# Nobita421/signature-Gan

Measured on AMD Instinct MI355X. Metric: signature images/sec (G+D train step, bs64 64x64 z=100), higher is better.
Workload: dtype f32; 1 GPU; configs[1]: reference conv G/D 64x64x1, z=100, batch 64 per GPU, f32, n_critic=1; global_batch=64, parallelism=dp1

## Files before the change

### signature-gan_amd/csrc/act.h

```cpp
#pragma once
#include <hip/hip_runtime.h>
#include <hip/hip_ext.h>
#include <stdint.h>

#define SIGGAN_LAUNCH_EV(ev, kernel, grid, block, shmem, stream, ...)                                            \
    do {                                                                                                         \
        if (ev) hipExtLaunchKernelGGL(kernel, grid, block, shmem, stream, nullptr, ev, 0, __VA_ARGS__);          \
        else hipLaunchKernelGGL(kernel, grid, block, shmem, stream, __VA_ARGS__);                                \
    } while (0)


namespace siggan {

typedef __bf16 bf16_t;
typedef _Float16 f16_t;
enum DType : int { DT_F32 = 0, DT_BF16 = 1, DT_F16 = 2 };
static inline size_t dt_size(int dt) { return dt == DT_F32 ? 4 : 2; }

typedef float f32x4 __attribute__((ext_vector_type(4)));
typedef float f32x16 __attribute__((ext_vector_type(16)));
typedef short s16x4 __attribute__((ext_vector_type(4)));
typedef short s16x8 __attribute__((ext_vector_type(8)));
typedef bf16_t bf16x4 __attribute__((ext_vector_type(4)));
typedef bf16_t bf16x8 __attribute__((ext_vector_type(8)));
typedef f16_t f16x4 __attribute__((ext_vector_type(4)));
typedef f16_t f16x8 __attribute__((ext_vector_type(8)));

template <class T> __device__ __forceinline__ f32x4 ld4(const T* p);
template <> __device__ __forceinline__ f32x4 ld4<float>(const float* p) { return *reinterpret_cast<const f32x4*>(p); }
template <> __device__ __forceinline__ f32x4 ld4<bf16_t>(const bf16_t* p) {
    const bf16x4 v = *reinterpret_cast<const bf16x4*>(p);
    return f32x4{(float)v[0], (float)v[1], (float)v[2], (float)v[3]};
}
template <> __device__ __forceinline__ f32x4 ld4<f16_t>(const f16_t* p) {
    const f16x4 v = *reinterpret_cast<const f16x4*>(p);
    return f32x4{(float)v[0], (float)v[1], (float)v[2], (float)v[3]};
}
template <class T> __device__ __forceinline__ void st4(T* p, f32x4 v);
template <> __device__ __forceinline__ void st4<float>(float* p, f32x4 v) { *reinterpret_cast<f32x4*>(p) = v; }
template <> __device__ __forceinline__ void st4<bf16_t>(bf16_t* p, f32x4 v) {
    *reinterpret_cast<bf16x4*>(p) = bf16x4{(bf16_t)v[0], (bf16_t)v[1], (bf16_t)v[2], (bf16_t)v[3]};
}
template <> __device__ __forceinline__ void st4<f16_t>(f16_t* p, f32x4 v) {
    *reinterpret_cast<f16x4*>(p) = f16x4{(f16_t)v[0], (f16_t)v[1], (f16_t)v[2], (f16_t)v[3]};
}
template <class T> __device__ __forceinline__ float ld1(const T* p) { return (float)*p; }
template <class T> __device__ __forceinline__ void st1(T* p, float v) { *p = (T)v; }

template <bool LK> __device__ __forceinline__ float g_act(float x, float gs) { return LK ? (x > 0.f ? x : x * gs) : fmaxf(x, 0.f); }
template <bool LK> __device__ __forceinline__ float g_dact(float x, float g, float gs) { return x > 0.f ? g : (LK ? g * gs : 0.f); }

#define SIGGAN_GS_SWITCH(GS, LK, ...)                                                   \
    do {                                                                         \
        if ((GS) != 0.f) { constexpr bool LK = true; __VA_ARGS__; }              \
        else { constexpr bool LK = false; __VA_ARGS__; }                         \
    } while (0)

#define SIGGAN_DT_SWITCH(DT, T, ...)                                     \
    do {                                                                 \
        if ((DT) == DT_F32) { using T = float; __VA_ARGS__; }            \
        else if ((DT) == DT_BF16) { using T = bf16_t; __VA_ARGS__; }     \
        else { using T = f16_t; __VA_ARGS__; }                           \
    } while (0)

}
```

### signature-gan_amd/csrc/gconv.h

```cpp
#pragma once
#include <hip/hip_runtime.h>
#include <stdint.h>
#include <vector>

#include "act.h"

namespace siggan {

enum Epilogue : int {
    EPI_RAW = 0,
    EPI_BIAS_LRELU_DROP,
    EPI_AFFINE_RELU,
    EPI_LRELU_BWD,
    EPI_BN_BWD_STATS,
};

struct GConvArgs {
    int dt;
    const void* in;
    const void* wp;
    void* out;
    int B, Hi, Wi, Ci, Co;
    int lgHr, lgWr;
    int Ho, Wo;
    int form;
    int M;
    int epi;
    const float* bias;
    const float* noise;
    const float* scale;
    const float* shift;
    const void* aref;
    const float* bnp;
    float* stat0;
    float* stat1;
    int64_t stat_cap;
    const float* cls_w;
    float* cls_part;
    float slope;
    float gslope;
    float* slab;
    int64_t slab_floats;
    size_t slab_stride;
    const float* zeros;
};

struct BnBwdParams { f32x4 sc, sf, mu, rs; };
__device__ __forceinline__ BnBwdParams bn_bwd_params(const float* __restrict__ bnp, int Co, int co) {
    BnBwdParams q;
    q.sc = *reinterpret_cast<const f32x4*>(bnp + co); q.sf = *reinterpret_cast<const f32x4*>(bnp + Co + co);
    q.mu = *reinterpret_cast<const f32x4*>(bnp + 2 * Co + co); q.rs = *reinterpret_cast<const f32x4*>(bnp + 3 * Co + co);
    return q;
}
template <class T, bool LK>
__device__ __forceinline__ void bn_bwd_stat_terms(const f32x4 v, const f32x4 y, const BnBwdParams& q, float gs, f32x4& s0, f32x4& s1) {
#pragma unroll
    for (int e = 0; e < 4; ++e) {
        const float vq = (float)(T)v[e];
        const float d = g_dact<LK>(fmaf(y[e], q.sc[e], q.sf[e]), vq, gs);
        s0[e] += d;
        s1[e] = fmaf(d, (y[e] - q.mu[e]) * q.rs[e], s1[e]);
    }
}
__host__ __device__ inline bool gen_lk(const GConvArgs& a) {
    return a.gslope != 0.f && (a.epi == EPI_AFFINE_RELU || a.epi == EPI_BN_BWD_STATS);
}

struct WgradArgs {
    int dt;
    const void* S;
    const void* L;
    float* slab;
    float* dw;
    float* db;
    int B, Cs, Cl;
    int lgHs, lgWs, lgCl;
    int K;
    int kchunk;
    const float* zeros;
};

struct Prof {
    struct Rec { int id; double flops, bytes; hipEvent_t e0, e1; };
    static constexpr int NID = 8;
    std::vector<Rec> recs;
    static const char* name(int id);
    void begin(int id, double flops, double bytes, hipStream_t st);
    void clear();
};
extern Prof* g_prof;

int launch_gconv(const GConvArgs& a, hipStream_t st);
void launch_gconv16(int cfg, const GConvArgs& a, dim3 grid, hipStream_t st, hipEvent_t e0, hipEvent_t e1, int kq = 1);
void launch_wgrad16(bool small, const WgradArgs& a, dim3 grid, hipStream_t st, hipEvent_t e0, hipEvent_t e1);
int launch_wgrad(WgradArgs a, int max_splits, hipStream_t st);

}
```

### signature-gan_amd/csrc/gconv.hip

```cpp
#include "gconv.h"
#include <hip/hip_ext.h>

namespace siggan {


static constexpr int BK = 32;
static constexpr int PAD = 4;

__device__ __forceinline__ int xcd_remap(int bid, int nwg) {
    const int q = nwg >> 3, r = nwg & 7, xcd = bid & 7, idx = bid >> 3;
    return (xcd < r ? xcd * (q + 1) : r * (q + 1) + (xcd - r) * q) + idx;
}

template <int BM, int BN, int WM, int WN, int BK = 32, int DEEP = 0, int KQ = 1, bool LK = false>
__global__ __launch_bounds__(256 * KQ) void k_gconv(const GConvArgs a) {
    constexpr int TM = BM / (32 * WM), TN = BN / (32 * WN);
    constexpr int PA = BM / 32, PB = BN / 32;
    constexpr int KC = BK / 32;
    constexpr int LD = BK + 4;
    __shared__ __attribute__((aligned(16))) float smem[KQ * 2 * LD * (BM + BN)];
    const int quad = KQ > 1 ? (int)(threadIdx.x >> 8) : 0;
    float* const sA = smem + quad * (2 * LD * (BM + BN));
    float* const sB = sA + 2 * LD * BM;

    const int tid = threadIdx.x & 255, lane = tid & 63, wave = tid >> 6;
    const int li = lane & 31, lh = lane >> 5;
    const int wm = wave / WN, wn = wave % WN;
    const float* const a_in = static_cast<const float*>(a.in);
    const float* const a_wp = static_cast<const float*>(a.wp);

    const int tiles_n = a.Co / BN;
    const int bid = xcd_remap(blockIdx.x, gridDim.x);
    const int m0 = (bid / tiles_n) * BM, n0 = (bid % tiles_n) * BN;
    const int cls = blockIdx.z, ph = cls >> 1, pw = cls & 1;
    const int Hr = 1 << a.lgHr, Wr = 1 << a.lgWr;
    const int ntaps = a.form == 0 ? 16 : 4;
    const int Ktot = ntaps * a.Ci;
    const int lgcpt = 31 - __builtin_clz(a.Ci / BK);
    const int nk_all = ntaps << lgcpt;
    const int kper = (nk_all + gridDim.y * KQ - 1) / (gridDim.y * KQ);
    const int k_lo = (blockIdx.y * KQ + quad) * kper;
    const int k_hi = min(nk_all, k_lo + kper);
    const int nk = k_hi - k_lo;

    const int kc = tid & 7, rloc = tid >> 3;
    const float* a_base[PA];
    int a_ih0[PA], a_iw0[PA];
#pragma unroll
    for (int p = 0; p < PA; ++p) {
        const int m = m0 + rloc + 32 * p;
        if (m < a.M) {
            const int n = m >> (a.lgHr + a.lgWr);
            const int rh = (m >> a.lgWr) & (Hr - 1), rw = m & (Wr - 1);
            a_base[p] = a_in + (size_t)n * a.Hi * a.Wi * a.Ci + kc * 4;
            if (a.form == 0) { a_ih0[p] = 2 * rh - 1; a_iw0[p] = 2 * rw - 1; }
            else             { a_ih0[p] = rh + ph;    a_iw0[p] = rw + pw; }
        } else {
            a_base[p] = a_in; a_ih0[p] = -(1 << 20); a_iw0[p] = -(1 << 20);
        }
    }
    const float* wcur = a_wp + ((size_t)cls * a.Co + n0 + rloc) * Ktot + kc * 4 + (size_t)k_lo * BK;

    const float* a_cur[PA];
    int a_step[PA];
    int l_tap = k_lo >> lgcpt, l_cc = k_lo & ((1 << lgcpt) - 1);
    auto set_tap = [&]() __attribute__((always_inline)) {
        int dh, dw;
        if (a.form == 0) { dh = l_tap >> 2; dw = l_tap & 3; } else { dh = -(l_tap >> 1); dw = -(l_tap & 1); }
#pragma unroll
        for (int p = 0; p < PA; ++p) {
            const int ih = a_ih0[p] + dh, iw = a_iw0[p] + dw;
            const bool ok = (unsigned)ih < (unsigned)a.Hi && (unsigned)iw < (unsigned)a.Wi;
            a_cur[p] = ok ? a_base[p] + ((size_t)(ih * a.Wi + iw) * a.Ci + l_cc * BK) : a.zeros;
            a_step[p] = ok ? BK : 0;
        }
    };
    constexpr int NSET = DEEP ? 2 : 1;
    f32x4 ra[NSET][PA][KC], rb[NSET][PB][KC];
    auto load_tile = [&](int set = 0) __attribute__((always_inline)) {
#pragma unroll
        for (int p = 0; p < PA; ++p) {
#pragma unroll
            for (int q = 0; q < KC; ++q) ra[set][p][q] = *reinterpret_cast<const f32x4*>(a_cur[p] + 32 * q);
            a_cur[p] += a_step[p];
        }
#pragma unroll
        for (int p = 0; p < PB; ++p)
#pragma unroll
            for (int q = 0; q < KC; ++q) rb[set][p][q] = *reinterpret_cast<const f32x4*>(wcur + (size_t)(32 * p) * Ktot + 32 * q);
        wcur += BK;
        if (++l_cc == (1 << lgcpt)) { l_cc = 0; ++l_tap; set_tap(); }
    };
    auto store_tile = [&](int buf, int set = 0) __attribute__((always_inline)) {
        float* dA = sA + buf * LD * BM + rloc * LD + kc * 4;
        float* dB = sB + buf * LD * BN + rloc * LD + kc * 4;
#pragma unroll
        for (int p = 0; p < PA; ++p)
#pragma unroll
            for (int q = 0; q < KC; ++q) *reinterpret_cast<f32x4*>(dA + 32 * p * LD + 32 * q) = ra[set][p][q];
#pragma unroll
        for (int p = 0; p < PB; ++p)
#pragma unroll
            for (int q = 0; q < KC; ++q) *reinterpret_cast<f32x4*>(dB + 32 * p * LD + 32 * q) = rb[set][p][q];
    };

    f32x16 acc[TM][TN];
#pragma unroll
    for (int i = 0; i < TM; ++i)
#pragma unroll
        for (int j = 0; j < TN; ++j)
#pragma unroll
            for (int r = 0; r < 16; ++r) acc[i][j][r] = 0.f;

    if (DEEP && nk >= 5) {
        auto tile = [&](const int h, const int kt, const bool st, const bool ld) __attribute__((always_inline)) {
            const float* pA = sA + h * LD * BM + (wm * (32 * TM) + li) * LD + 4 * lh;
            const float* pB = sB + h * LD * BN + (wn * (32 * TN) + li) * LD + 4 * lh;
            f32x4 fa[2][TM], fb[2][TN];
#pragma unroll
            for (int i = 0; i < TM; ++i) fa[0][i] = *reinterpret_cast<const f32x4*>(pA + 32 * i * LD);
#pragma unroll
            for (int j = 0; j < TN; ++j) fb[0][j] = *reinterpret_cast<const f32x4*>(pB + 32 * j * LD);
#pragma unroll
            for (int c = 0; c < BK / 8; ++c) {
                const int cur = c & 1, nxt = cur ^ 1;
                if (c + 1 < BK / 8) {
#pragma unroll
                    for (int i = 0; i < TM; ++i) fa[nxt][i] = *reinterpret_cast<const f32x4*>(pA + 32 * i * LD + 8 * (c + 1));
#pragma unroll
                    for (int j = 0; j < TN; ++j) fb[nxt][j] = *reinterpret_cast<const f32x4*>(pB + 32 * j * LD + 8 * (c + 1));
                }
                __builtin_amdgcn_sched_barrier(0);
#pragma unroll
                for (int t = 0; t < 4; ++t)
#pragma unroll
                    for (int i = 0; i < TM; ++i)
#pragma unroll
                        for (int j = 0; j < TN; ++j)
                            acc[i][j] = __builtin_amdgcn_mfma_f32_32x32x2f32(fa[cur][i][t], fb[cur][j][t], acc[i][j], 0, 0, 0);
                if (c == 0 && st) store_tile(h ^ 1, h ^ 1);
                if (c == 1 && ld) load_tile(h ^ 1);
            }
            __syncthreads();
        };
        set_tap();
        load_tile(0);
        load_tile(1);
        store_tile(0, 0);
        load_tile(0);
        __syncthreads();
        int kt = 0;
        for (; kt + 4 < nk; kt += 2) {
            tile(0, kt, true, true);
            tile(1, kt + 1, true, true);
        }
        for (; kt < nk; kt += 2) {
            tile(0, kt, kt + 1 < nk, kt + 3 < nk);
            if (kt + 1 < nk) tile(1, kt + 1, kt + 2 < nk, kt + 4 < nk);
        }
    } else {
    if (nk > 0) {
        set_tap();
        load_tile();
        store_tile(0);
        if (nk > 1) load_tile();
    }
    __syncthreads();

    for (int kt = 0; kt < nk; ++kt) {
        const int buf = kt & 1;
        const float* pA = sA + buf * LD * BM + (wm * (32 * TM) + li) * LD + 4 * lh;
        const float* pB = sB + buf * LD * BN + (wn * (32 * TN) + li) * LD + 4 * lh;
        f32x4 fa[2][TM], fb[2][TN];
#pragma unroll
        for (int i = 0; i < TM; ++i) fa[0][i] = *reinterpret_cast<const f32x4*>(pA + 32 * i * LD);
#pragma unroll
        for (int j = 0; j < TN; ++j) fb[0][j] = *reinterpret_cast<const f32x4*>(pB + 32 * j * LD);
#pragma unroll
        for (int c = 0; c < BK / 8; ++c) {
            const int cur = c & 1, nxt = cur ^ 1;
            if (c + 1 < BK / 8) {
#pragma unroll
                for (int i = 0; i < TM; ++i) fa[nxt][i] = *reinterpret_cast<const f32x4*>(pA + 32 * i * LD + 8 * (c + 1));
#pragma unroll
                for (int j = 0; j < TN; ++j) fb[nxt][j] = *reinterpret_cast<const f32x4*>(pB + 32 * j * LD + 8 * (c + 1));
            }
            __builtin_amdgcn_sched_barrier(0);
#pragma unroll
            for (int t = 0; t < 4; ++t)
#pragma unroll
                for (int i = 0; i < TM; ++i)
#pragma unroll
                    for (int j = 0; j < TN; ++j)
                        acc[i][j] = __builtin_amdgcn_mfma_f32_32x32x2f32(fa[cur][i][t], fb[cur][j][t], acc[i][j], 0, 0, 0);
            if (c == 0 && kt + 1 < nk) store_tile(buf ^ 1);
            if (c == 1 && kt + 2 < nk) load_tile();
        }
        __syncthreads();
    }
    }

    float* const outp = gridDim.y > 1 ? a.slab + (size_t)blockIdx.y * a.slab_stride : static_cast<float*>(a.out);
    const int epi = gridDim.y > 1 ? (int)EPI_RAW : a.epi;
    constexpr int LDT = BN + 4;
    static_assert(BM * LDT <= 2 * LD * (BM + BN), "output tile must fit the staging buffers");
    float* const sT = smem;
    if (KQ > 1) {
        float* const red = smem + 2 * LD * (BM + BN);
        if (quad == 1) {
#pragma unroll
            for (int i = 0; i < TM; ++i)
#pragma unroll
                for (int j = 0; j < TN; ++j)
#pragma unroll
                    for (int r = 0; r < 16; ++r) red[(((wave * TM + i) * TN + j) * 16 + r) * 64 + lane] = acc[i][j][r];
        }
        __syncthreads();
        if (quad == 0) {
#pragma unroll
            for (int i = 0; i < TM; ++i)
#pragma unroll
                for (int j = 0; j < TN; ++j)
#pragma unroll
                    for (int r = 0; r < 16; ++r) acc[i][j][r] += red[(((wave * TM + i) * TN + j) * 16 + r) * 64 + lane];
        }
    }
    if (quad == 0) {
#pragma unroll
        for (int i = 0; i < TM; ++i)
#pragma unroll
            for (int j = 0; j < TN; ++j)
#pragma unroll
                for (int r = 0; r < 16; ++r)
                    sT[(wm * (32 * TM) + 32 * i + (r & 3) + 8 * (r >> 2) + 4 * lh) * LDT + wn * (32 * TN) + 32 * j + li] = acc[i][j][r];
    }
    __syncthreads();
    if (quad != 0 && epi != EPI_BN_BWD_STATS) return;
    constexpr int C4 = BN / 4, RPP = 256 / C4;
    const int c4 = tid % C4, r0 = tid / C4;
    const int co = n0 + c4 * 4;
    BnBwdParams bq;
    f32x4 st0 = {0.f, 0.f, 0.f, 0.f}, st1 = st0;
    if (epi == EPI_BN_BWD_STATS) bq = bn_bwd_params(a.bnp, a.Co, co);
    const f32x4 bias4 = epi == EPI_BIAS_LRELU_DROP ? *reinterpret_cast<const f32x4*>(a.bias + co) : f32x4{0.f, 0.f, 0.f, 0.f};
    f32x4 sc4 = {1.f, 1.f, 1.f, 1.f}, sh4 = {0.f, 0.f, 0.f, 0.f};
    if (epi == EPI_AFFINE_RELU) { sc4 = *reinterpret_cast<const f32x4*>(a.scale + co); sh4 = *reinterpret_cast<const f32x4*>(a.shift + co); }
    const bool use_noise = (epi == EPI_BIAS_LRELU_DROP || epi == EPI_LRELU_BWD) && a.noise != nullptr;
#pragma unroll
    for (int p = 0; p < BM / RPP; ++p) {
        const int row = r0 + RPP * p, m = m0 + row;
        if (m >= a.M || quad != 0) continue;
        const int n = m >> (a.lgHr + a.lgWr);
        size_t opix;
        if (a.form == 0) {
            opix = (size_t)m;
        } else {
            const int rh = (m >> a.lgWr) & (Hr - 1), rw = m & (Wr - 1);
            opix = ((size_t)n * a.Ho + 2 * rh + ph) * a.Wo + 2 * rw + pw;
        }
        const size_t o = opix * a.Co + co;
        f32x4 v = *reinterpret_cast<const f32x4*>(sT + row * LDT + c4 * 4);
        if (epi == EPI_BN_BWD_STATS) {
            bn_bwd_stat_terms<float, LK>(v, *reinterpret_cast<const f32x4*>(static_cast<const float*>(a.aref) + o), bq, a.gslope, st0, st1);
        } else if (epi == EPI_BIAS_LRELU_DROP) {
#pragma unroll
            for (int e = 0; e < 4; ++e) { float t = v[e] + bias4[e]; v[e] = t > 0.f ? t : t * a.slope; }
            if (use_noise) {
                const f32x4 nz = *reinterpret_cast<const f32x4*>(a.noise + (size_t)n * a.Co + co);
#pragma unroll
                for (int e = 0; e < 4; ++e) v[e] *= nz[e];
            }
        } else if (epi == EPI_AFFINE_RELU) {
#pragma unroll
            for (int e = 0; e < 4; ++e) v[e] = g_act<LK>(fmaf(v[e], sc4[e], sh4[e]), a.gslope);
        } else if (epi == EPI_LRELU_BWD) {
            const f32x4 ar = *reinterpret_cast<const f32x4*>(static_cast<const float*>(a.aref) + o);
#pragma unroll
            for (int e = 0; e < 4; ++e) v[e] *= ar[e] > 0.f ? 1.f : a.slope;
            if (use_noise) {
                const f32x4 nz = *reinterpret_cast<const f32x4*>(a.noise + (size_t)n * a.Co + co);
#pragma unroll
                for (int e = 0; e < 4; ++e) v[e] *= nz[e];
            }
        }
        *reinterpret_cast<f32x4*>(outp + o) = v;
    }
    if (epi == EPI_BN_BWD_STATS) {
        __syncthreads();
        if (quad == 0) {
            *reinterpret_cast<f32x4*>(sT + (size_t)tid * 8) = st0;
            *reinterpret_cast<f32x4*>(sT + (size_t)tid * 8 + 4) = st1;
        }
        __syncthreads();
        if (quad == 0 && r0 == 0) {
#pragma unroll 4
            for (int k = 1; k < RPP; ++k) {
                st0 += *reinterpret_cast<const f32x4*>(sT + (size_t)(k * C4 + c4) * 8);
                st1 += *reinterpret_cast<const f32x4*>(sT + (size_t)(k * C4 + c4) * 8 + 4);
            }
            const size_t prow = (size_t)cls * (gridDim.x / tiles_n) + bid / tiles_n;
            *reinterpret_cast<f32x4*>(a.stat0 + prow * a.Co + co) = st0;
            *reinterpret_cast<f32x4*>(a.stat1 + prow * a.Co + co) = st1;
        }
    }
}

template <int CI, bool LK>
__global__ __launch_bounds__(256) void k_gconv_up4(const GConvArgs a) {
    constexpr int BM = 128, BN = 32, LD = BK + 4, LP = CI + 4, NCC = CI / BK;
    constexpr int PATCH_PIX = 264;
    constexpr int SMEM = (PATCH_PIX * LP + 2 * 4 * BN * LD) > (BM * 4 * BN) ? (PATCH_PIX * LP + 2 * 4 * BN * LD) : (BM * 4 * BN);
    __shared__ __attribute__((aligned(16))) float smem[SMEM];
    float* const sP = smem;
    float* const sB = smem + PATCH_PIX * LP;
    const int tid = threadIdx.x, lane = tid & 63, wave = tid >> 6;
    const int li = lane & 31, lh = lane >> 5;
    const int m0 = xcd_remap(blockIdx.x, gridDim.x) * BM;
    const int Hr = 1 << a.lgHr, Wr = 1 << a.lgWr, Wp = Wr + 2;
    const int Ktot = 4 * CI;
    const int n_img = m0 >> (a.lgHr + a.lgWr), rh0 = (m0 >> a.lgWr) & (Hr - 1), rows = BM >> a.lgWr;

    {
        const float* const img = static_cast<const float*>(a.in) + (size_t)n_img * a.Hi * a.Wi * CI;
        const int nchunk = (rows + 2) * Wp * (CI / 4);
        constexpr int NI = (PATCH_PIX * (CI / 4) + 255) / 256;
        f32x4 v[NI];
#pragma unroll
        for (int q = 0; q < NI; ++q) {
            const int i = tid + 256 * q;
            const int pix = i / (CI / 4), ch = i - pix * (CI / 4);
            const int pr = pix / Wp, pc = pix - pr * Wp;
            const int ih = rh0 - 1 + pr, iw = pc - 1;
            const bool ok = i < nchunk && (unsigned)ih < (unsigned)a.Hi && (unsigned)iw < (unsigned)a.Wi;
            const float* src = ok ? img + ((size_t)ih * a.Wi + iw) * CI + ch * 4 : a.zeros;
            v[q] = *reinterpret_cast<const f32x4*>(src);
        }
#pragma unroll
        for (int q = 0; q < NI; ++q) {
            const int i = tid + 256 * q;
            if (i < nchunk) {
                const int pix = i / (CI / 4), ch = i - pix * (CI / 4);
                *reinterpret_cast<f32x4*>(sP + pix * LP + ch * 4) = v[q];
            }
        }
    }
    const int kc = tid & 7, rloc = tid >> 3;
    const float* const w_row = static_cast<const float*>(a.wp) + (size_t)rloc * Ktot + kc * 4;
    f32x4 rb[4];
    int l_k = 0;
    auto load_tile = [&]() __attribute__((always_inline)) {
        const int cls = l_k / NCC, cc = l_k - cls * NCC;
#pragma unroll
        for (int t = 0; t < 4; ++t)
            rb[t] = *reinterpret_cast<const f32x4*>(w_row + (size_t)cls * a.Co * Ktot + t * CI + cc * BK);
        ++l_k;
    };
    auto store_tile = [&](int buf) __attribute__((always_inline)) {
#pragma unroll
        for (int t = 0; t < 4; ++t)
            *reinterpret_cast<f32x4*>(sB + ((buf * 4 + t) * BN + rloc) * LD + kc * 4) = rb[t];
    };

    f32x16 acc[4];
#pragma unroll
    for (int cls = 0; cls < 4; ++cls)
#pragma unroll
        for (int r = 0; r < 16; ++r) acc[cls][r] = 0.f;

    load_tile();
    store_tile(0);
    load_tile();
    __syncthreads();

    const int ml = wave * 32 + li;
    const float* const pP = sP + (((ml >> a.lgWr) + 1) * Wp + (ml & (Wr - 1)) + 1) * LP + 4 * lh;

#pragma unroll
    for (int cls = 0; cls < 4; ++cls) {
        const int ph = cls >> 1, pw = cls & 1;
        for (int cc = 0; cc < NCC; ++cc) {
            const int kt = cls * NCC + cc, buf = kt & 1;
            const float* pA[4];
#pragma unroll
            for (int t = 0; t < 4; ++t) pA[t] = pP + ((ph - (t >> 1)) * Wp + (pw - (t & 1))) * LP + cc * BK;
            const float* pB = sB + (buf * 4 * BN + li) * LD + 4 * lh;
            f32x4 fa[2][4], fb[2][4];
#pragma unroll
            for (int t = 0; t < 4; ++t) {
                fa[0][t] = *reinterpret_cast<const f32x4*>(pA[t]);
                fb[0][t] = *reinterpret_cast<const f32x4*>(pB + t * BN * LD);
            }
#pragma unroll
            for (int c = 0; c < BK / 8; ++c) {
                const int cur = c & 1, nxt = cur ^ 1;
                if (c + 1 < BK / 8) {
#pragma unroll
                    for (int t = 0; t < 4; ++t) {
                        fa[nxt][t] = *reinterpret_cast<const f32x4*>(pA[t] + 8 * (c + 1));
                        fb[nxt][t] = *reinterpret_cast<const f32x4*>(pB + t * BN * LD + 8 * (c + 1));
                    }
                }
                __builtin_amdgcn_sched_barrier(0);
#pragma unroll
                for (int t = 0; t < 4; ++t)
#pragma unroll
                    for (int u = 0; u < 4; ++u)
                        acc[cls] = __builtin_amdgcn_mfma_f32_32x32x2f32(fa[cur][t][u], fb[cur][t][u], acc[cls], 0, 0, 0);
                if (c == 0 && kt + 1 < 4 * NCC) store_tile(buf ^ 1);
                if (c == 1 && kt + 2 < 4 * NCC) load_tile();
            }
            __syncthreads();
        }
    }

    const float sc = a.epi == EPI_AFFINE_RELU ? a.scale[li] : 1.f, sf = a.epi == EPI_AFFINE_RELU ? a.shift[li] : 0.f;
    const int Wo = 2 * Wr;
    float* const so = smem;
#pragma unroll
    for (int r = 0; r < 16; ++r) {
        const int mr = wave * 32 + (r & 3) + 8 * (r >> 2) + 4 * lh;
        const int rl = mr >> a.lgWr, rw = mr & (Wr - 1);
#pragma unroll
        for (int cls = 0; cls < 4; ++cls) {
            float v = acc[cls][r];
            if (a.epi == EPI_AFFINE_RELU) v = g_act<LK>(fmaf(v, sc, sf), a.gslope);
            so[(((2 * rl + (cls >> 1)) * Wo) + 2 * rw + (cls & 1)) * BN + li] = v;
        }
    }
    __syncthreads();
    f32x4* const dst = reinterpret_cast<f32x4*>(static_cast<float*>(a.out) + ((size_t)n_img * a.Ho + 2 * rh0) * a.Wo * BN);
    const f32x4* const src = reinterpret_cast<const f32x4*>(so);
#pragma unroll
    for (int q = 0; q < (BM * 4 * BN / 4) / 256; ++q) dst[q * 256 + tid] = src[q * 256 + tid];
}

template <class T, bool LK>
__global__ __launch_bounds__(256) void k_splitk_epilogue(const GConvArgs a, int nsplit, int64_t total4) {
    const int64_t i = (int64_t)blockIdx.x * 256 + threadIdx.x;
    if (a.epi == EPI_BN_BWD_STATS) {
        __shared__ __attribute__((aligned(16))) float sh[256 * 8];
        const int C4 = a.Co / 4, c4 = threadIdx.x & (C4 - 1);
        f32x4 s0 = {0.f, 0.f, 0.f, 0.f}, s1 = s0;
        if (i < total4) {
            const f32x4* sl = reinterpret_cast<const f32x4*>(a.slab);
            const size_t stride4 = a.slab_stride / 4;
            f32x4 v = sl[i];
            for (int z = 1; z < nsplit; ++z) v += sl[(size_t)z * stride4 + i];
            bn_bwd_stat_terms<T, LK>(v, ld4<T>(static_cast<const T*>(a.aref) + i * 4), bn_bwd_params(a.bnp, a.Co, c4 * 4), a.gslope, s0, s1);
            st4<T>(static_cast<T*>(a.out) + i * 4, v);
        }
        *reinterpret_cast<f32x4*>(sh + threadIdx.x * 8) = s0;
        *reinterpret_cast<f32x4*>(sh + threadIdx.x * 8 + 4) = s1;
        __syncthreads();
        if ((int)threadIdx.x < C4) {
            for (int k = 1; k < 256 / C4; ++k) {
                s0 += *reinterpret_cast<const f32x4*>(sh + (k * C4 + c4) * 8);
                s1 += *reinterpret_cast<const f32x4*>(sh + (k * C4 + c4) * 8 + 4);
            }
            *reinterpret_cast<f32x4*>(a.stat0 + (size_t)blockIdx.x * a.Co + c4 * 4) = s0;
            *reinterpret_cast<f32x4*>(a.stat1 + (size_t)blockIdx.x * a.Co + c4 * 4) = s1;
        }
        return;
    }
    if (i >= total4) return;
    const float4* sl = reinterpret_cast<const float4*>(a.slab);
    const size_t stride4 = a.slab_stride / 4;
    float4 v = sl[i];
    for (int z = 1; z < nsplit; ++z) {
        const float4 w = sl[(size_t)z * stride4 + i];
        v.x += w.x; v.y += w.y; v.z += w.z; v.w += w.w;
    }
    const int C4 = a.Co / 4;
    const int64_t per_img = (int64_t)C4 * a.Ho * a.Wo;
    const bool p2 = (C4 & (C4 - 1)) == 0 && (per_img & (per_img - 1)) == 0;
    const int c = (p2 ? (int)(i & (C4 - 1)) : (int)(i % C4)) * 4;
    const int64_t n = p2 ? i >> (63 - __builtin_clzll(per_img)) : i / per_img;
    float* e = reinterpret_cast<float*>(&v);
    if (a.epi == EPI_BIAS_LRELU_DROP) {
#pragma unroll
        for (int k = 0; k < 4; ++k) {
            float x = e[k] + a.bias[c + k];
            x = x > 0.f ? x : x * a.slope;
            if (a.noise) x *= a.noise[n * a.Co + c + k];
            e[k] = x;
        }
    } else if (a.epi == EPI_AFFINE_RELU) {
#pragma unroll
        for (int k = 0; k < 4; ++k) e[k] = g_act<LK>(fmaf(e[k], a.scale[c + k], a.shift[c + k]), a.gslope);
    } else if (a.epi == EPI_LRELU_BWD) {
        const f32x4 ar = ld4<T>(static_cast<const T*>(a.aref) + i * 4);
        const float* r = reinterpret_cast<const float*>(&ar);
#pragma unroll
        for (int k = 0; k < 4; ++k) {
            float x = e[k] * (r[k] > 0.f ? 1.f : a.slope);
            if (a.noise) x *= a.noise[n * a.Co + c + k];
            e[k] = x;
        }
    }
    st4<T>(static_cast<T*>(a.out) + i * 4, f32x4{v.x, v.y, v.z, v.w});
    if (a.cls_w) {
        __shared__ float shc[4];
        const f32x4 w4 = *reinterpret_cast<const f32x4*>(a.cls_w + (size_t)(p2 ? (i & (per_img - 1)) : (i % per_img)) * 4);
        float d = (float)(T)v.x * w4[0];
        d = fmaf((float)(T)v.y, w4[1], d); d = fmaf((float)(T)v.z, w4[2], d); d = fmaf((float)(T)v.w, w4[3], d);
#pragma unroll
        for (int o = 32; o > 0; o >>= 1) d += __shfl_down(d, o, 64);
        if ((threadIdx.x & 63) == 0) shc[threadIdx.x >> 6] = d;
        __syncthreads();
        if (threadIdx.x == 0) a.cls_part[blockIdx.x] = ((shc[0] + shc[1]) + shc[2]) + shc[3];
    }
}

Prof* g_prof = nullptr;

const char* Prof::name(int id) {
    static const char* n[NID] = {"k_gconv<128,128>", "k_gconv<128,64>", "k_gconv<64,64>", "k_gconv<128,32>",
                                 "k_wgrad<64,64>", "k_gconv_up4", "k_wgrad<32,128>", "?"};
    return n[id < 0 || id >= NID ? NID - 1 : id];
}
void Prof::begin(int id, double flops, double bytes, hipStream_t) {
    Rec r; r.id = id; r.flops = flops; r.bytes = bytes;
    (void)hipEventCreate(&r.e0); (void)hipEventCreate(&r.e1);
    recs.push_back(r);
}
void Prof::clear() {
    for (auto& r : recs) { (void)hipEventDestroy(r.e0); (void)hipEventDestroy(r.e1); }
    recs.clear();
}

static double gconv_bytes(const GConvArgs& a) {
    const double es = (double)dt_size(a.dt);
    const double in = (double)a.B * a.Hi * a.Wi * a.Ci, out = (double)a.B * a.Ho * a.Wo * a.Co, w = 16.0 * a.Ci * a.Co;
    return es * (in + w + out * (a.epi == EPI_LRELU_BWD ? 2.0 : 1.0));
}
static double wgrad_bytes(const WgradArgs& a) {
    const double es = (double)dt_size(a.dt);
    return es * ((double)a.K * a.Cs + 4.0 * a.K * a.Cl) + 4.0 * 16.0 * a.Cs * a.Cl;
}

template <int BM, int BN, int WM, int WN, int BKT = 32, int DEEP = 0, int KQ = 1>
static int launch_cfg(const GConvArgs& a_in, hipStream_t st, int id, int nsplit) {
    GConvArgs a = a_in;
    const int tiles = ((a.M + BM - 1) / BM) * (a.Co / BN);
    const int ncls = a.form == 0 ? 1 : 4;
    const int64_t total4 = (int64_t)a.B * a.Ho * a.Wo * a.Co / 4;
    int rows = 0;
    if (a.epi == EPI_BN_BWD_STATS) {
        if (nsplit > 1 && (256 % (a.Co / 4)) != 0) nsplit = 1;
        rows = nsplit > 1 ? (int)((total4 + 255) / 256) : ((a.M + BM - 1) / BM) * ncls;
        if ((int64_t)2 * rows * a.Co > a.stat_cap) { a.epi = EPI_RAW; rows = 0; }
        else a.stat1 = a.stat0 + (size_t)rows * a.Co;
    }
    if (a.cls_w) {
        const int64_t per_img4 = (int64_t)a.Ho * a.Wo * a.Co / 4;
        if (nsplit > 1 && a.epi != EPI_BN_BWD_STATS && total4 % 256 == 0 && per_img4 % 256 == 0) rows = (int)(per_img4 / 256);
        else a.cls_w = nullptr;
    }
    dim3 grid(tiles, nsplit, ncls);
    if (g_prof) g_prof->begin(id, 2.0 * a.M * a.Co * (double)((a.form == 0 ? 16 : 4) * a.Ci) * ncls, gconv_bytes(a), st);
    hipEvent_t e0 = g_prof ? g_prof->recs.back().e0 : nullptr, e1 = g_prof ? g_prof->recs.back().e1 : nullptr;
    if (a.dt != DT_F32) {
        launch_gconv16(id, a, grid, st, e0, e1, KQ);
    } else if (gen_lk(a)) {
        hipExtLaunchKernelGGL((k_gconv<BM, BN, WM, WN, BKT, DEEP, KQ, true>), grid, dim3(256 * KQ), 0, st, e0, e1, 0, a);
    } else if (g_prof) {
        hipExtLaunchKernelGGL((k_gconv<BM, BN, WM, WN, BKT, DEEP, KQ>), grid, dim3(256 * KQ), 0, st, e0, e1, 0, a);
    } else {
        hipLaunchKernelGGL((k_gconv<BM, BN, WM, WN, BKT, DEEP, KQ>), grid, dim3(256 * KQ), 0, st, a);
    }
    if (nsplit > 1)
        SIGGAN_GS_SWITCH(gen_lk(a) ? 1.f : 0.f, LK, SIGGAN_DT_SWITCH(a.dt, T, hipLaunchKernelGGL((k_splitk_epilogue<T, LK>),
            dim3((unsigned)((total4 + 255) / 256)), dim3(256), 0, st, a, nsplit, total4)));
    return rows;
}

int launch_gconv(const GConvArgs& a_in, hipStream_t st) {
    GConvArgs a = a_in;
    const int ncls = a.form == 0 ? 1 : 4;
    auto blocks = [&](int bm, int bn) { return ((a.M + bm - 1) / bm) * (a.Co / bn) * ncls; };
    const int nk = (a.form == 0 ? 16 : 4) * (a.Ci / BK);
    auto splits = [&](int nblk) {
        int ns = 1;
        if (a.slab && nblk < 384) {
            ns = (512 + nblk - 1) / nblk;
            if (ns > nk / 4) ns = nk / 4;
            if (ns > 8) ns = 8;
            const int64_t out_floats = (int64_t)a.B * a.Ho * a.Wo * a.Co;
            if (ns > 1 && (int64_t)ns * out_floats > a.slab_floats) ns = (int)(a.slab_floats / out_floats);
            if (ns < 1) ns = 1;
        }
        a.slab_stride = (size_t)a.B * a.Ho * a.Wo * a.Co;
        return ns;
    };
    if (a.Co >= 64) {
        if (a.Co >= 128 && blocks(128, 128) >= 512) return launch_cfg<128, 128, 2, 2, 32, 1>(a, st, 0, 1);
        const int ns = splits(blocks(64, 64));
        if (ns == 2 && (nk & 1) == 0) return launch_cfg<64, 64, 2, 2, 32, 1, 2>(a, st, 2, 1);
        if (ns == 4 && !a.cls_w && a.dt != DT_F32 && (nk & 1) == 0) return launch_cfg<64, 64, 2, 2, 32, 1, 2>(a, st, 2, 1);
        return launch_cfg<64, 64, 2, 2, 32, 1>(a, st, 2, ns);
    }
    if (a.dt == DT_F32 && a.form == 1 && a.Co == 32 && (a.epi == EPI_RAW || a.epi == EPI_AFFINE_RELU) && (a.Ci == 32 || a.Ci == 64) &&
        a.M / 128 >= (a.Ci == 32 ? 384 : 768) && a.M % 128 == 0 &&
        ((1 << (a.lgHr + a.lgWr)) % 128) == 0 && a.lgWr >= 4 && a.lgWr <= 6) {
        dim3 grid(a.M / 128);
        if (g_prof) g_prof->begin(5, 2.0 * a.M * a.Co * (double)(4 * a.Ci) * 4, gconv_bytes(a), st);
        hipEvent_t e0 = g_prof ? g_prof->recs.back().e0 : nullptr, e1 = g_prof ? g_prof->recs.back().e1 : nullptr;
        if (gen_lk(a)) {
            if (a.Ci == 32) hipExtLaunchKernelGGL((k_gconv_up4<32, true>), grid, dim3(256), 0, st, e0, e1, 0, a);
            else hipExtLaunchKernelGGL((k_gconv_up4<64, true>), grid, dim3(256), 0, st, e0, e1, 0, a);
        } else {
            if (a.Ci == 32) hipExtLaunchKernelGGL((k_gconv_up4<32, false>), grid, dim3(256), 0, st, e0, e1, 0, a);
            else hipExtLaunchKernelGGL((k_gconv_up4<64, false>), grid, dim3(256), 0, st, e0, e1, 0, a);
        }
        return 0;
    }
    const int ns = splits(blocks(128, 32));
    return launch_cfg<128, 32, 4, 1, 32, 1>(a, st, 3, ns);
}

template <int BM, int BN, int WM, int WN>
__global__ __launch_bounds__(256) void k_wgrad(const WgradArgs a) {
    constexpr int TM = BM / (32 * WM), TN = BN / (32 * WN);
    constexpr int LDA = BM + PAD, LDB = BN + PAD;
    constexpr int CA = BM / 4, RA = 256 / CA, PA = BK / RA;
    constexpr int CB = BN / 4, RB = 256 / CB, PB = BK / RB;
    __shared__ __attribute__((aligned(16))) float smem[2 * BK * (LDA + LDB)];
    float* const sA = smem;
    float* const sB = smem + 2 * BK * LDA;

    const int tid = threadIdx.x, lane = tid & 63, wave = tid >> 6;
    const int li = lane & 31, lh = lane >> 5;
    const int wm = wave / WN, wn = wave % WN;
    const int N = 16 << a.lgCl;
    const int tiles_n = N / BN;
    const int lin = blockIdx.z * gridDim.x + blockIdx.x;
    const int lid = xcd_remap(lin, gridDim.x * gridDim.z);
    const int bx = lid % gridDim.x, bz = lid / gridDim.x;
    const int i0 = (bx / tiles_n) * BM, j0 = (bx % tiles_n) * BN;
    const int kbeg = bz * a.kchunk;
    const int kend = min(a.K, kbeg + a.kchunk);
    const int nk = (kend - kbeg + BK - 1) / BK;
    const int Hs = 1 << a.lgHs, Ws = 1 << a.lgWs, Hl = 2 * Hs, Wl = 2 * Ws, Cl = 1 << a.lgCl;

    const int ca = tid % CA, ka = tid / CA;
    const int cb = tid % CB, kb = tid / CB;
    const float* const a_S = static_cast<const float*>(a.S);
    const float* const a_L = static_cast<const float*>(a.L);
    const int jj = j0 + cb * 4, tap = jj >> a.lgCl, lch = jj & (Cl - 1);
    const int kh = tap >> 2, kw = tap & 3;

    f32x4 ra[2][PA], rb[2][PB];
    size_t a_off[PA];
    int a_pix[PA], b_pix[PB];
#pragma unroll
    for (int p = 0; p < PA; ++p) { a_pix[p] = kbeg + ka + RA * p; a_off[p] = (size_t)a_pix[p] * a.Cs + i0 + ca * 4; }
#pragma unroll
    for (int p = 0; p < PB; ++p) b_pix[p] = kbeg + kb + RB * p;
    const int a_adv = BK * a.Cs;
    const int lgWl = a.lgWs + 1;
#define WG_LOAD_TILE(KT, SET)                                                                         \
    {                                                                                                 \
        _Pragma("unroll") for (int p = 0; p < PA; ++p) {                                              \
            const float* src = a_pix[p] < kend ? a_S + a_off[p] : a.zeros;                            \
            ra[SET][p] = *reinterpret_cast<const f32x4*>(src);                                       \
            a_off[p] += a_adv; a_pix[p] += BK;                                                        \
        }                                                                                             \
        _Pragma("unroll") for (int p = 0; p < PB; ++p) {                                              \
            const int pix = b_pix[p];                                                                 \
            const int y = pix >> a.lgWs;                                              \
            const int ih = 2 * (y & (Hs - 1)) - 1 + kh, iw = 2 * (pix & (Ws - 1)) - 1 + kw;           \
            const bool ok = pix < kend && (unsigned)ih < (unsigned)Hl && (unsigned)iw < (unsigned)Wl; \
                          \
            const unsigned off = (((unsigned)(2 * y - 1 + kh) << lgWl) + (unsigned)iw) << a.lgCl;     \
            const float* src = ok ? a_L + ((size_t)off + lch) : a.zeros;                              \
            rb[SET][p] = *reinterpret_cast<const f32x4*>(src);                                       \
            b_pix[p] += BK;                                                                           \
        }                                                                                             \
    }
#define WG_STORE_TILE(BUF, SET)                                                                       \
    {                                                                                                 \
        _Pragma("unroll") for (int p = 0; p < PA; ++p)                                                \
            *reinterpret_cast<f32x4*>(sA + (BUF) * BK * LDA + (ka + RA * p) * LDA + ca * 4) = ra[SET][p]; \
        _Pragma("unroll") for (int p = 0; p < PB; ++p)                                                \
            *reinterpret_cast<f32x4*>(sB + (BUF) * BK * LDB + (kb + RB * p) * LDB + cb * 4) = rb[SET][p]; \
    }

    f32x16 acc[TM][TN];
#pragma unroll
    for (int i = 0; i < TM; ++i)
#pragma unroll
        for (int j = 0; j < TN; ++j)
#pragma unroll
            for (int r = 0; r < 16; ++r) acc[i][j][r] = 0.f;

    constexpr int NQ = 256 / BM, KQ = BK / NQ;
    const bool bias_blk = a.db != nullptr && j0 == 0;
    const int bcol = tid % BM, kq = tid / BM;
    float bsum = 0.f;
#define WG_TILE(BUF, ST, LD)                                                                          \
    {                                                                                                 \
        if (bias_blk) {                                                                               \
            const float* col = sA + (BUF) * BK * LDA + kq * KQ * LDA + bcol;                          \
            _Pragma("unroll") for (int k = 0; k < KQ; ++k) bsum += col[k * LDA];                      \
        }                                                                                             \
        const float* pA = sA + (BUF) * BK * LDA + lh * LDA + wm * (32 * TM) + li;                     \
        const float* pB = sB + (BUF) * BK * LDB + lh * LDB + wn * (32 * TN) + li;                     \
                          \
        float fa[2][4][TM], fb[2][4][TN];                                                             \
        _Pragma("unroll") for (int q = 0; q < 4; ++q) {                                               \
            _Pragma("unroll") for (int i = 0; i < TM; ++i) fa[0][q][i] = pA[(2 * q) * LDA + 32 * i];  \
            _Pragma("unroll") for (int j = 0; j < TN; ++j) fb[0][q][j] = pB[(2 * q) * LDB + 32 * j];  \
        }                                                                                             \
        _Pragma("unroll") for (int c = 0; c < BK / 8; ++c) {                                          \
            const int cur = c & 1, nxt = cur ^ 1;                                                     \
            if (c + 1 < BK / 8) {                                                                     \
                _Pragma("unroll") for (int q = 0; q < 4; ++q) {                                       \
                    _Pragma("unroll") for (int i = 0; i < TM; ++i) fa[nxt][q][i] = pA[(8 * c + 8 + 2 * q) * LDA + 32 * i]; \
                    _Pragma("unroll") for (int j = 0; j < TN; ++j) fb[nxt][q][j] = pB[(8 * c + 8 + 2 * q) * LDB + 32 * j]; \
                }                                                                                     \
            }                                                                                         \
            __builtin_amdgcn_sched_barrier(0);                                                        \
            _Pragma("unroll") for (int q = 0; q < 4; ++q)                                             \
                _Pragma("unroll") for (int i = 0; i < TM; ++i)                                        \
                    _Pragma("unroll") for (int j = 0; j < TN; ++j)                                    \
                        acc[i][j] = __builtin_amdgcn_mfma_f32_32x32x2f32(fa[cur][q][i], fb[cur][q][j], acc[i][j], 0, 0, 0); \
            if (c == 0) { ST }                                                                        \
            if (c == 1) { LD }                                                                        \
        }                                                                                             \
        __syncthreads();                                                                              \
    }
    if (nk >= 5) {
        WG_LOAD_TILE(0, 0)
        WG_LOAD_TILE(1, 1)
        WG_STORE_TILE(0, 0)
        WG_LOAD_TILE(2, 0)
        __syncthreads();
        int kt = 0;
        for (; kt + 4 < nk; kt += 2) {
            WG_TILE(0, WG_STORE_TILE(1, 1), WG_LOAD_TILE(kt + 3, 1))
            WG_TILE(1, WG_STORE_TILE(0, 0), WG_LOAD_TILE(kt + 4, 0))
        }
        for (; kt < nk; kt += 2) {
            WG_TILE(0, if (kt + 1 < nk) WG_STORE_TILE(1, 1), if (kt + 3 < nk) WG_LOAD_TILE(kt + 3, 1))
            if (kt + 1 < nk) WG_TILE(1, if (kt + 2 < nk) WG_STORE_TILE(0, 0), if (kt + 4 < nk) WG_LOAD_TILE(kt + 4, 0))
        }
    } else {
        if (nk > 0) {
            WG_LOAD_TILE(0, 0)
            WG_STORE_TILE(0, 0)
            if (nk > 1) WG_LOAD_TILE(1, 0)
        }
        __syncthreads();
        for (int kt = 0; kt < nk; ++kt) {
            if (kt & 1) WG_TILE(1, if (kt + 1 < nk) WG_STORE_TILE(0, 0), if (kt + 2 < nk) WG_LOAD_TILE(kt + 2, 0))
            else WG_TILE(0, if (kt + 1 < nk) WG_STORE_TILE(1, 0), if (kt + 2 < nk) WG_LOAD_TILE(kt + 2, 0))
        }
    }
#undef WG_TILE

#undef WG_LOAD_TILE
#undef WG_STORE_TILE
    if (bias_blk) {
        smem[kq * BM + bcol] = bsum;
        __syncthreads();
        if (tid < BM) {
            float t = smem[tid];
#pragma unroll
            for (int q = 1; q < NQ; ++q) t += smem[q * BM + tid];
            if (gridDim.z == 1) a.db[i0 + tid] = t;
            else a.slab[(size_t)gridDim.z * a.Cs * N + (size_t)bz * a.Cs + i0 + tid] = t;
        }
    }
    if (gridDim.z == 1 && a.dw) {
#pragma unroll
        for (int i = 0; i < TM; ++i)
#pragma unroll
            for (int r = 0; r < 16; ++r) {
                const int row = i0 + wm * (32 * TM) + 32 * i + (r & 3) + 8 * (r >> 2) + 4 * lh;
#pragma unroll
                for (int j = 0; j < TN; ++j) {
                    const int col = j0 + wn * (32 * TN) + 32 * j + li;
                    a.dw[((size_t)row * Cl + (col & (Cl - 1))) * 16 + (col >> a.lgCl)] = acc[i][j][r];
                }
            }
        return;
    }
    float* const out = a.slab + (size_t)bz * a.Cs * N;
#pragma unroll
    for (int i = 0; i < TM; ++i)
#pragma unroll
        for (int r = 0; r < 16; ++r) {
            const int row = i0 + wm * (32 * TM) + 32 * i + (r & 3) + 8 * (r >> 2) + 4 * lh;
#pragma unroll
            for (int j = 0; j < TN; ++j)
                out[(size_t)row * N + j0 + wn * (32 * TN) + 32 * j + li] = acc[i][j][r];
        }
}

static void launch_wgrad_reduce(const float* slab, float* dw, float* db, int nsplit, int Cs, int Cl, hipStream_t st);

int launch_wgrad(WgradArgs a, int max_splits, hipStream_t st) {
    const int N = 16 << a.lgCl;
    const bool small = a.Cs < 64;
    const int tiles = small ? (N / 128) : (a.Cs / 64) * (N / 64);
    int ktiles = (a.K + BK - 1) / BK;
    int nsplit = (512 + tiles - 1) / tiles;
    if (nsplit > ktiles / 4) nsplit = ktiles / 4;
    if (nsplit > max_splits) nsplit = max_splits;
    if (nsplit < 1) nsplit = 1;
    int per = (ktiles + nsplit - 1) / nsplit;
    a.kchunk = per * BK;
    nsplit = (ktiles + per - 1) / per;
    dim3 grid(tiles, 1, nsplit);
    if (g_prof) g_prof->begin(small ? 6 : 4, 2.0 * a.Cs * (double)N * a.K, wgrad_bytes(a), st);
    hipEvent_t e0 = g_prof ? g_prof->recs.back().e0 : nullptr, e1 = g_prof ? g_prof->recs.back().e1 : nullptr;
    if (a.dt != DT_F32) {
        launch_wgrad16(small, a, grid, st, e0, e1);
    } else if (g_prof) {
        if (small) hipExtLaunchKernelGGL((k_wgrad<32, 128, 1, 4>), grid, dim3(256), 0, st, e0, e1, 0, a);
        else hipExtLaunchKernelGGL((k_wgrad<64, 64, 2, 2>), grid, dim3(256), 0, st, e0, e1, 0, a);
    } else if (small) {
        hipLaunchKernelGGL((k_wgrad<32, 128, 1, 4>), grid, dim3(256), 0, st, a);
    } else {
        hipLaunchKernelGGL((k_wgrad<64, 64, 2, 2>), grid, dim3(256), 0, st, a);
    }
    if (nsplit > 1) launch_wgrad_reduce(a.slab, a.dw, a.db, nsplit, a.Cs, 1 << a.lgCl, st);
    return nsplit;
}

__global__ __launch_bounds__(1024) void k_wgrad_reduce(const float* __restrict__ slab, float* __restrict__ dw, float* __restrict__ db,
                                                       int nsplit, int Cs, int lgCl) {
    __shared__ float sh[16][64];
    const int N = 16 << lgCl, Cl = 1 << lgCl;
    const size_t total = (size_t)Cs * N;
    const int cl = threadIdx.x & 63, zl = threadIdx.x >> 6, SL = blockDim.x >> 6;
    const size_t wblocks = total / 64;
    const bool bias = blockIdx.x >= wblocks;
    const size_t idx = bias ? (size_t)(blockIdx.x - wblocks) * 64 + cl : (size_t)blockIdx.x * 64 + cl;
    const float* src = bias ? slab + (size_t)nsplit * total : slab;
    const size_t zstride = bias ? (size_t)Cs : total;
    const bool live = !bias || idx < (size_t)Cs;
    float acc = 0.f;
    if (live) {
#pragma unroll 8
        for (int z = zl; z < nsplit; z += SL) acc += src[(size_t)z * zstride + idx];
    }
    if (SL > 1) {
        sh[zl][cl] = acc;
        __syncthreads();
        if (zl != 0) return;
        for (int k = 1; k < SL; ++k) acc += sh[k][cl];
    }
    if (!live) return;
    if (bias) { db[idx] = acc; return; }
    const int j = (int)(idx & (size_t)(N - 1)), s_ = (int)(idx >> (4 + lgCl));
    const int tap = j >> lgCl, l = j & (Cl - 1);
    dw[((size_t)s_ * Cl + l) * 16 + tap] = acc;
}

static int ilog2(int v) { int l = 0; while ((1 << l) < v) ++l; return l; }

static void launch_wgrad_reduce(const float* slab, float* dw, float* db, int nsplit, int Cs, int Cl, hipStream_t st) {
    const size_t total = (size_t)Cs * 16 * Cl;
    int SL = 1;
    while (SL < 16 && SL < nsplit) SL *= 2;
    const unsigned blocks = (unsigned)(total / 64) + (db ? (unsigned)((Cs + 63) / 64) : 0u);
    hipLaunchKernelGGL(k_wgrad_reduce, dim3(blocks), dim3(64 * SL), 0, st, slab, dw, db, nsplit, Cs, ilog2(Cl));
}

}
```

### signature-gan_amd/csrc/ops.h

```cpp
#pragma once
#include <hip/hip_runtime.h>
#include <stdint.h>

#include "act.h"

namespace siggan {

struct DevState {
    unsigned long long seed;
    unsigned long long rng_ctr;
    float step_size;
    float bc2_sqrt;
    float grad_mul;
    float grad_norm;
    float sumsq;
    int skip;
    float pad[2];
};

void launch_randn(float* out, int64_t n, const DevState* st, uint32_t stream_id, hipStream_t s);
void launch_dropnoise_multi(int nt, float* const* out, const int64_t* n, const int64_t* elem0, const uint32_t* sid, float keep,
                            const DevState* st, hipStream_t s, uint32_t ctr_add = 0);
void launch_mask_to_noise(const float* mask, float* out, int64_t n, float keep, hipStream_t s);
void launch_tick(DevState* st, hipStream_t s);

enum PrepType : int { PREP_PACK_DOWN = 0, PREP_PACK_UP, PREP_FC_T, PREP_CLS, PREP_BN_EVAL, PREP_SCALE, PREP_TAPS };
struct PrepJob {
    int type, O, I, perm;
    int dt;
    const float* mul;
    const float* src;
    const float* src2;
    const float* src3;
    const float* src4;
    float* dst;
};
struct PrepTable {
    static constexpr int MAXJ = 32;
    int njobs;
    int overflow;
    long long prefix[MAXJ + 1];
    PrepJob job[MAXJ];
};
void prep_add(PrepTable& t, const PrepJob& j, long long count);
bool launch_prepare(const PrepTable& t, float bn_eps, hipStream_t s);
bool launch_prepare_conv1(const PrepTable& t, float bn_eps, int dt, const float* x, const float* W, const float* b, float slope,
                          void* out, int B, int S, hipStream_t s);

void launch_fc_fwd(int dt, const float* z, const float* Wt, const float* b, void* y, int B, int K, int C0, float gslope,
                   hipStream_t s, const float* bn_affine_relu = nullptr, const DevState* st = nullptr, uint32_t stream_id = 0,
                   float* z_out = nullptr);
bool launch_fc_fwd_fused(int dt, const float* z, const float* W, const float* bias, void* y, void* a, const float* gamma,
                         const float* beta, float* rmean, float* rvar, int64_t* batches, float* bn, const float* bne,
                         float* z_out, const DevState* st, uint32_t sid, int B, int K, int C0, float momentum, float eps,
                         float gslope, hipStream_t s);
bool launch_fc_bwd_fused(int dt, const void* da, const void* y, const float* z, float* bn, float* dW, float* db, float* dgamma,
                         float* dbeta, int B, int K, int C0, float gslope, hipStream_t s);
void launch_fc_wgrad(int dt, const void* dy, const float* z, float* dW, float* db, int B, int K, int C0, hipStream_t s);

void launch_bn_train_stats(int dt, const void* y, int64_t R, int C, const float* gamma, const float* beta,
                           float* rmean, float* rvar, int64_t* batches, float* bn, float* partial,
                           int perm_c0, float momentum, float eps, hipStream_t s);
void launch_bn_relu(int dt, const void* y, void* a, int64_t R, int C, const float* bn, float gslope, hipStream_t s);
void launch_bn_bwd(int dt, void* da, const void* y, int64_t R, int C, float* bn, float* partial,
                   float* dgamma, float* dbeta, int perm_c0, float gslope, hipStream_t s, int pre_rows = 0, hipEvent_t done = nullptr);

void launch_final_fwd(int dt, const void* act, const float* Wt, const float* b, float* img, int B, int S, int C, float gslope,
                      hipStream_t s, const float* bn = nullptr, hipEvent_t done = nullptr);
void launch_final_bwd_reduce(int dt, const float* dpre, const float* Wt, const void* y, int B, int S, int C, const float* bn,
                             float* partial, float* partial_w, float gslope, hipStream_t s);
void launch_final_bn_bwd_apply(int dt, const float* dpre, const float* Wt, const void* y, void* dy, int B, int S, int C, float* bn,
                               const float* partial, const float* partial_w, float* dW, float* db, float* dgamma, float* dbeta,
                               float gslope, hipStream_t s, hipEvent_t done = nullptr);

void launch_conv1_fwd(int dt, const float* x0, int n0, const float* x1, const float* W, const float* b,
                      const float* noise, float slope, void* out, int B, int S, int C, hipStream_t s);
void launch_conv1_wgrad(int dt, const void* dv, const float* x0, int n0, const float* x1, float* dW, float* db,
                        float* partial, int B, int S, int C, hipStream_t s);
void launch_conv1_dgrad_tanh(int dt, const void* dv, const float* Wt, const float* img, float* dpre, int B, int S,
                             int C, hipStream_t s);
void launch_cls_fwd(int dt, const void* act, const float* wcp, const float* bc, float* logits, int B, int F, hipStream_t s);
void launch_cls_features(int dt, const void* act, float* feat, int B, int C, hipStream_t s);
void launch_bce(const float* logits, int B, int n0, float y0, float y1, float* probs, float* dlogit,
                float* metrics, int is_g_step, hipStream_t s, float gscale = 1.0f, const float* parts = nullptr, int P = 0,
                const float* bc = nullptr);
void launch_cls_bwd(int dt, const float* logits, int n0, float y0, float y1, const float* wcp, const void* act, const float* noise,
                    float slope, void* dv, int B, int C, hipStream_t s, float gscale = 1.0f, float* bce_probs = nullptr,
                    float* bce_dlogit = nullptr, float* bce_metrics = nullptr, int bce_is_g = 0, bool with_bce = false,
                    const float* parts = nullptr, int P = 0, const float* bc = nullptr);
void launch_cls_wgrad(int dt, const float* dlogit, const void* act, float* dWc, float* dbc, int B, int C, hipStream_t s);
void launch_to_f32(int dt, const void* src, float* dst, int64_t n, hipStream_t s);

struct SnLayer {
    const float* W;
    int rows, K;
    int u_off, v_off;
    int64_t w_off;
};
struct SnTable {
    static constexpr int MAXS = 8;
    int n;
    SnLayer layer[MAXS];
    int pre_k[MAXS + 1], pre_r[MAXS + 1];
    float *u, *v;
    float *tbuf, *wbuf;
    float* sig;
    float *u_saved, *v_saved;
    float* dots;
    int u_total, v_total;
    int slot[2];
};
void launch_sn_sigma(const SnTable& t, int training, int slot, float eps, hipStream_t s);
void launch_sn_combine(const SnTable& t, const float* g0, const float* g1, float* out, int64_t total, int npass, hipStream_t s);

void launch_grad_sumsq(const float* g, int64_t n, DevState* st, float* partial, hipStream_t s);
void launch_adam_prepare(DevState* st, float* steps, int ntensors, double lr, double beta1, double beta2,
                         float grad_scale, float clip_max_norm, float* metric_norm, hipStream_t s,
                         int check_finite = 0, float* metric_skipped = nullptr, const float* sumsq_partial = nullptr);
__host__ __device__ inline double pow_step(double b, double t) {
    unsigned long long n = (unsigned long long)t;
    double r = 1.0;
    while (n) { if (n & 1) r *= b; b *= b; n >>= 1; }
    return r;
}
void launch_adam_fused(float* p, float* g, float* m, float* v, int64_t n, DevState* st, float* steps, int ntensors, double t,
                       double lr, double beta1, double beta2, double eps, float grad_scale, float clip_max_norm,
                       float* metric_norm, const float* sumsq_partial, hipStream_t s, float* metric_skipped = nullptr);
void launch_adam(float* p, float* g, float* m, float* v, int64_t n, const DevState* st, double beta1,
                 double beta2, double eps, int write_back_grad, hipStream_t s);

enum ApType : int { AP_FLAT = 0, AP_CONV, AP_T16, AP_TAPS, AP_BN };
struct ApJob {
    int type;
    int A, Bc;
    int dt;
    long long off, n;
    long long off2, n2;
    float* dst;
    float* dst2;
    const float* rmean;
    const float* rvar;
    int wait;
};
struct ApTable {
    static constexpr int MAXJ = 24;
    int njobs, overflow;
    long long prefix[MAXJ + 1];
    ApJob job[MAXJ];
};
void ap_add(ApTable& t, const ApJob& j);
struct ApRide { const float* x; void* out; int B, S, dt; float slope; long long w_off, b_off; unsigned* counter; unsigned* late; };
bool launch_adam_pack(const ApTable& t, float* p, float* g, float* m, float* v, DevState* st, float* steps, int ntensors,
                      double tstep, double lr, double beta1, double beta2, double eps, float grad_scale, float clip_max_norm,
                      float* metric_norm, const float* sumsq_partial, float* metric_skipped, float bn_eps,
                      const ApRide* ride, hipStream_t s);

void launch_augment(const uint8_t* cache, int64_t n_images, const int32_t* index, const int32_t* prm, const int16_t* tabs,
                    const float* lut, float* out, int B, int S, int augment, int fill, hipStream_t s);

}
```

### signature-gan_amd/csrc/ops.hip

```cpp
#include "ops.h"
#include "rng.h"

namespace siggan {

static inline int cdiv(int64_t a, int64_t b) { return (int)((a + b - 1) / b); }

__device__ __forceinline__ uint4 draw(const DevState* st, uint64_t idx, uint32_t stream_id, uint32_t ctr_add = 0) {
    return draw_raw(st->seed, st->rng_ctr + ctr_add, idx, stream_id);
}

__global__ void k_randn(float* __restrict__ out, int64_t n, const DevState* __restrict__ st, uint32_t sid) {
    const int64_t t = (int64_t)blockIdx.x * blockDim.x + threadIdx.x;
    if (t * 4 >= n) return;
    const f32x4 v = normal4(draw(st, (uint64_t)t, sid));
    for (int j = 0; j < 4 && t * 4 + j < n; ++j) out[t * 4 + j] = v[j];
}
__global__ void k_mask_to_noise(const float* __restrict__ m, float* __restrict__ out, int64_t n, float inv) {
    const int64_t i = (int64_t)blockIdx.x * blockDim.x + threadIdx.x;
    if (i < n) out[i] = m[i] * inv;
}
__global__ void k_tick(DevState* st) { st->rng_ctr += 1; }

void launch_randn(float* out, int64_t n, const DevState* st, uint32_t sid, hipStream_t s) {
    hipLaunchKernelGGL(k_randn, dim3(cdiv((n + 3) / 4, 256)), dim3(256), 0, s, out, n, st, sid);
}
struct NoiseTable { float* out[8]; int64_t n[8]; int64_t elem0[8]; uint32_t sid[8]; int64_t pre[9]; int nt; };
__global__ void k_dropnoise_multi(const NoiseTable tb, float keep, float inv, const DevState* __restrict__ st, uint32_t ctr_add) {
    const int64_t g = (int64_t)blockIdx.x * blockDim.x + threadIdx.x;
    if (g >= tb.pre[tb.nt]) return;
    int t = 0;
    while (g >= tb.pre[t + 1]) ++t;
    const int64_t q = g - tb.pre[t];
    const uint4 r = draw(st, (uint64_t)(tb.elem0[t] / 4 + q), tb.sid[t], ctr_add);
    const uint32_t x[4] = {r.x, r.y, r.z, r.w};
    float* o = tb.out[t];
    for (int j = 0; j < 4 && q * 4 + j < tb.n[t]; ++j) o[q * 4 + j] = u01(x[j]) < keep ? inv : 0.f;
}
void launch_dropnoise_multi(int nt, float* const* out, const int64_t* n, const int64_t* elem0, const uint32_t* sid, float keep,
                            const DevState* st, hipStream_t s, uint32_t ctr_add) {
    NoiseTable tb; tb.nt = nt; tb.pre[0] = 0;
    for (int t = 0; t < nt; ++t) { tb.out[t] = out[t]; tb.n[t] = n[t]; tb.elem0[t] = elem0[t]; tb.sid[t] = sid[t]; tb.pre[t + 1] = tb.pre[t] + (n[t] + 3) / 4; }
    hipLaunchKernelGGL(k_dropnoise_multi, dim3(cdiv(tb.pre[nt], 256)), dim3(256), 0, s, tb, keep, 1.0f / keep, st, ctr_add);
}
void launch_mask_to_noise(const float* mask, float* out, int64_t n, float keep, hipStream_t s) {
    hipLaunchKernelGGL(k_mask_to_noise, dim3(cdiv(n, 256)), dim3(256), 0, s, mask, out, n, 1.0f / keep);
}
void launch_tick(DevState* st, hipStream_t s) { hipLaunchKernelGGL(k_tick, dim3(1), dim3(1), 0, s, st); }

__device__ __forceinline__ int perm16(int c, int perm_c0) { return perm_c0 > 0 ? (c % perm_c0) * 16 + c / perm_c0 : c; }

struct AdamK { float mul, ss, bc2, w1, beta2, w2, eps; };
__device__ __forceinline__ void adam_upd(const AdamK& k, float& pp, float& gg, float& mm, float& vv) {
    const float gr = gg * k.mul;
    gg = gr;
    mm = k.w1 < 0.5f ? mm + k.w1 * (gr - mm) : gr - (gr - mm) * (1.0f - k.w1);
    vv = vv * k.beta2 + k.w2 * gr * gr;
    const float denom = sqrtf(vv) / k.bc2 + k.eps;
    pp = pp + (k.ss * mm) / denom;
}

static long long prep_units(const PrepJob& j) {
    switch (j.type) {
        case PREP_PACK_DOWN: case PREP_CLS: return j.type == PREP_CLS ? 1 : j.O;
        case PREP_PACK_UP: return j.O;
        case PREP_FC_T: return (long long)(j.I * 16 / 64) * ((j.O + 127) / 128);
        case PREP_SCALE: return (j.O + 1023) / 1024;
        case PREP_TAPS: return (j.O * j.I + 255) / 256;
        default: return (j.O + 255) / 256;
    }
}
void prep_add(PrepTable& t, const PrepJob& j, long long ) {
    if (t.njobs >= PrepTable::MAXJ) { t.overflow = 1; return; }
    if (t.njobs == 0) t.prefix[0] = 0;
    t.job[t.njobs] = j;
    t.prefix[t.njobs + 1] = t.prefix[t.njobs] + prep_units(j);
    ++t.njobs;
}
__device__ __forceinline__ void put_w(const PrepJob& q, size_t idx, float v) {
    if (q.mul) v *= q.mul[0];
    if (q.dt == DT_F32) q.dst[idx] = v;
    else if (q.dt == DT_BF16) reinterpret_cast<bf16_t*>(q.dst)[idx] = (bf16_t)v;
    else reinterpret_cast<f16_t*>(q.dst)[idx] = (f16_t)v;
}
__device__ __forceinline__ void prepare_unit(const PrepTable& t, float eps, unsigned bid) {
    extern __shared__ float tile[];
    int j = 0;
    while ((long long)bid >= t.prefix[j + 1]) ++j;
    const PrepJob& q = t.job[j];
    const int u = (int)(bid - t.prefix[j]);
    const int tid = threadIdx.x;
    if (q.type == PREP_PACK_DOWN || q.type == PREP_CLS) {
        const int I = q.type == PREP_CLS ? q.O : q.I;
        const float* src = q.src + (size_t)u * I * 16;
#pragma unroll 4
        for (int e = tid; e < I * 16; e += 256) tile[(e >> 4) * 17 + (e & 15)] = src[e];
        __syncthreads();
        const size_t d0 = (size_t)u * I * 16;
        if ((I & (I - 1)) == 0) {
            const int lgI = 31 - __builtin_clz(I);
#pragma unroll 4
            for (int e = tid; e < I * 16; e += 256) { const int tap = e >> lgI, i = e & (I - 1); put_w(q, d0 + e, tile[i * 17 + tap]); }
        } else {
            for (int e = tid; e < I * 16; e += 256) { const int tap = e / I, i = e - tap * I; put_w(q, d0 + e, tile[i * 17 + tap]); }
        }
    } else if (q.type == PREP_PACK_UP) {
        const int I = q.I, O = q.O;
#pragma unroll 4
        for (int e = tid; e < I * 16; e += 256) tile[(e >> 4) * 17 + (e & 15)] = q.src[((size_t)(e >> 4) * O + u) * 16 + (e & 15)];
        __syncthreads();
        if ((I & (I - 1)) == 0) {
            const int lgI = 31 - __builtin_clz(I);
#pragma unroll 4
            for (int e = tid; e < I * 16; e += 256) {
                const int i = e & (I - 1), tt = (e >> lgI) & 3, cls = e >> (lgI + 2);
                const int kh = 1 - (cls >> 1) + 2 * (tt >> 1), kw = 1 - (cls & 1) + 2 * (tt & 1);
                put_w(q, ((size_t)cls * O + u) * 4 * I + tt * I + i, tile[i * 17 + kh * 4 + kw]);
            }
        } else {
            for (int e = tid; e < I * 16; e += 256) {
                const int i = e % I, tt = (e / I) & 3, cls = e / (4 * I);
                const int kh = 1 - (cls >> 1) + 2 * (tt >> 1), kw = 1 - (cls & 1) + 2 * (tt & 1);
                put_w(q, ((size_t)cls * O + u) * 4 * I + tt * I + i, tile[i * 17 + kh * 4 + kw]);
            }
        }
    } else if (q.type == PREP_FC_T) {
        const int K = q.O, C0 = q.I, F = C0 * 16, kchunks = (K + 127) / 128;
        const int f0 = (u / kchunks) * 64, k0 = (u % kchunks) * 128, kn = min(128, K - k0);
        for (int e = tid; e < 64 * kn; e += 256) {
            const int r = e / kn, k = e - r * kn, fp = f0 + r;
            tile[r * 129 + k] = q.src[(size_t)((fp % C0) * 16 + fp / C0) * K + k0 + k];
        }
        __syncthreads();
        for (int e = tid; e < 64 * kn; e += 256) { const int k = e >> 6, r = e & 63; q.dst[(size_t)(k0 + k) * F + f0 + r] = tile[r * 129 + k]; }
    } else if (q.type == PREP_TAPS) {
        const int e = u * 256 + tid;
        if (e < q.O * q.I) q.dst[(e % q.I) * q.O + e / q.I] = q.mul ? q.src[e] * q.mul[0] : q.src[e];
    } else if (q.type == PREP_SCALE) {
        const float m = q.mul ? q.mul[0] : 1.0f;
        for (int e = u * 1024 + tid; e < min(q.O, (u + 1) * 1024); e += 256) q.dst[e] = q.src[e] * m;
    } else {
        const int C = q.O, c = u * 256 + tid;
        if (c < C) {
            const int tix = perm16(c, q.perm);
            const float rstd = 1.0f / sqrtf(q.src4[tix] + eps);
            const float sc = q.src[tix] * rstd;
            q.dst[c] = sc; q.dst[C + c] = q.src2[tix] - q.src3[tix] * sc; q.dst[2 * C + c] = q.src3[tix]; q.dst[3 * C + c] = rstd;
        }
    }
}
__global__ __launch_bounds__(256) void k_prepare(const PrepTable t, float eps) { prepare_unit(t, eps, blockIdx.x); }
bool launch_prepare(const PrepTable& t, float bn_eps, hipStream_t s) {
    if (t.overflow) return false;
    if (t.njobs == 0) return true;
    hipLaunchKernelGGL(k_prepare, dim3((unsigned)t.prefix[t.njobs]), dim3(256), 512 * 17 * sizeof(float), s, t, bn_eps);
    return true;
}

struct ColPlan { int cg, cbx, nch, rows; };
static ColPlan col_plan(int64_t R, int C) {
    const int C4 = C / 4;
    ColPlan p;
    p.cg = C4 < 64 ? C4 : 64;
    p.cbx = cdiv(C4, p.cg);
    const int rl = 256 / p.cg;
    int nch = 1024 / p.cbx;
    if (nch > 256) nch = 256;
    const int64_t max_ch = (R + 2 * rl - 1) / (2 * rl);
    if (nch > max_ch) nch = (int)max_ch;
    if (nch < 1) nch = 1;
    int rows = (int)((R + nch - 1) / nch);
    rows = ((rows + rl - 1) / rl) * rl;
    p.nch = (int)((R + rows - 1) / rows);
    p.rows = rows;
    return p;
}

__device__ __forceinline__ void add4(float4& a, const float4 b) { a.x += b.x; a.y += b.y; a.z += b.z; a.w += b.w; }

template <class F>
__global__ __launch_bounds__(256) void k_colreduce(F f, int64_t R, int C, int cg, int rows, float* __restrict__ p0,
                                                   float* __restrict__ p1) {
    __shared__ float4 sh[2][256];
    const int C4 = C / 4, rl = 256 / cg;
    const int cl = threadIdx.x % cg, lane = threadIdx.x / cg;
    const int c4 = blockIdx.x * cg + cl;
    const int64_t r0 = (int64_t)blockIdx.y * rows;
    const int64_t r1 = r0 + rows < R ? r0 + rows : R;
    float4 s0 = make_float4(0.f, 0.f, 0.f, 0.f), s1 = s0;
    if (c4 < C4) {
#pragma unroll 8
        for (int64_t r = r0 + lane; r < r1; r += rl) f(r, c4, C4, s0, s1);
    }
    sh[0][threadIdx.x] = s0; sh[1][threadIdx.x] = s1;
    __syncthreads();
    if (lane == 0 && c4 < C4) {
        for (int k = 1; k < rl; ++k) { add4(s0, sh[0][k * cg + cl]); add4(s1, sh[1][k * cg + cl]); }
        reinterpret_cast<float4*>(p0 + (size_t)blockIdx.y * C)[c4] = s0;
        reinterpret_cast<float4*>(p1 + (size_t)blockIdx.y * C)[c4] = s1;
    }
}

template <int W = 64>
__device__ __forceinline__ void gather2(const float* __restrict__ p0, const float* __restrict__ p1, int nch, int C,
                                        float& s, float& q, float (*sh)[16][64], int bx = -1) {
    const int cl = threadIdx.x & (W - 1), rl = threadIdx.x / W, nl = blockDim.x / W;
    const int c = (bx < 0 ? (int)blockIdx.x : bx) * W + cl;
    float* const s0 = &sh[0][0][0];
    float* const s1 = &sh[1][0][0];
    float a = 0.f, b = 0.f;
    if (c < C) {
        if (p1) {
#pragma unroll 8
            for (int k = rl; k < nch; k += nl) { a += p0[(size_t)k * C + c]; b += p1[(size_t)k * C + c]; }
        } else {
#pragma unroll 8
            for (int k = rl; k < nch; k += nl) a += p0[(size_t)k * C + c];
        }
    }
    s0[rl * W + cl] = a; s1[rl * W + cl] = b;
    __syncthreads();
    s = 0.f; q = 0.f;
    for (int k = 0; k < nl; ++k) { s += s0[k * W + cl]; q += s1[k * W + cl]; }
}

__device__ __forceinline__ float4 f4(const f32x4 v) { return make_float4(v[0], v[1], v[2], v[3]); }
template <class T>
struct FStats {
    const T* y;
    __device__ void operator()(int64_t r, int c4, int C4, float4& s0, float4& s1) const {
        const float4 v = f4(ld4<T>(y + (r * C4 + c4) * 4)), p = f4(ld4<T>(y + c4 * 4));
        const float4 d = make_float4(v.x - p.x, v.y - p.y, v.z - p.z, v.w - p.w);
        add4(s0, d);
        s1.x = fmaf(d.x, d.x, s1.x); s1.y = fmaf(d.y, d.y, s1.y); s1.z = fmaf(d.z, d.z, s1.z); s1.w = fmaf(d.w, d.w, s1.w);
    }
};
template <class T, bool LK>
struct FBnBwd {
    const T* da; const T* y; const float4* bn; float gs;
    __device__ void operator()(int64_t r, int c4, int C4, float4& s0, float4& s1) const {
        const size_t i = (size_t)r * C4 + c4;
        const float4 g = f4(ld4<T>(da + i * 4)), yy = f4(ld4<T>(y + i * 4)), sc = bn[c4], sf = bn[C4 + c4], mu = bn[2 * C4 + c4], rs = bn[3 * C4 + c4];
        const float4 d = make_float4(g_dact<LK>(fmaf(yy.x, sc.x, sf.x), g.x, gs), g_dact<LK>(fmaf(yy.y, sc.y, sf.y), g.y, gs),
                                     g_dact<LK>(fmaf(yy.z, sc.z, sf.z), g.z, gs), g_dact<LK>(fmaf(yy.w, sc.w, sf.w), g.w, gs));
        add4(s0, d);
        s1.x = fmaf(d.x, (yy.x - mu.x) * rs.x, s1.x); s1.y = fmaf(d.y, (yy.y - mu.y) * rs.y, s1.y);
        s1.z = fmaf(d.z, (yy.z - mu.z) * rs.z, s1.z); s1.w = fmaf(d.w, (yy.w - mu.w) * rs.w, s1.w);
    }
};


template <int W, class T>
__global__ __launch_bounds__(1024) void k_bn_train_fin(const float* __restrict__ p0, const float* __restrict__ p1, int nch, int64_t R, int C,
                               const T* __restrict__ y, const float* __restrict__ gamma,
                               const float* __restrict__ beta, float* __restrict__ rmean, float* __restrict__ rvar,
                               int64_t* __restrict__ batches, float* __restrict__ bn, int perm_c0, float momentum,
                               float eps) {
    __shared__ float sh[2][16][64];
    float s, q;
    gather2<W>(p0, p1, nch, C, s, q, sh);
    const int c = blockIdx.x * W + (threadIdx.x & (W - 1));
    if (blockIdx.x == 0 && threadIdx.x == 0 && batches) batches[0] += 1;
    if (threadIdx.x >= W || c >= C) return;
    const float invR = 1.0f / (float)R;
    const float d = s * invR;
    const float mean = ld1<T>(y + c) + d;
    float var = q * invR - d * d;
    var = var > 0.f ? var : 0.f;
    const float rstd = 1.0f / sqrtf(var + eps);
    const int t = perm16(c, perm_c0);
    const float sc = gamma[t] * rstd;
    bn[c] = sc; bn[C + c] = beta[t] - mean * sc; bn[2 * C + c] = mean; bn[3 * C + c] = rstd;
    const float unb = R > 1 ? var * ((float)R / (float)(R - 1)) : var;
    rmean[t] = momentum * mean + (1.0f - momentum) * rmean[t];
    rvar[t] = momentum * unb + (1.0f - momentum) * rvar[t];
}
void launch_bn_train_stats(int dt, const void* yv, int64_t R, int C, const float* gamma, const float* beta, float* rmean,
                           float* rvar, int64_t* batches, float* bn, float* partial, int perm_c0, float momentum,
                           float eps, hipStream_t s) {
    const ColPlan pl = col_plan(R, C);
    float* p0 = partial; float* p1 = partial + (size_t)pl.nch * C;
    SIGGAN_DT_SWITCH(dt, T, {
        const T* y = (const T*)yv;
        hipLaunchKernelGGL((k_colreduce<FStats<T>>), dim3(pl.cbx, pl.nch), dim3(256), 0, s, FStats<T>{y}, R, C, pl.cg, pl.rows, p0, p1);
        if (C <= 32)
            hipLaunchKernelGGL((k_bn_train_fin<32, T>), dim3(cdiv(C, 32)), dim3(1024), 0, s, p0, p1, pl.nch, R, C, y, gamma, beta, rmean,
                               rvar, batches, bn, perm_c0, momentum, eps);
        else
            hipLaunchKernelGGL((k_bn_train_fin<64, T>), dim3(cdiv(C, 64)), dim3(1024), 0, s, p0, p1, pl.nch, R, C, y, gamma, beta, rmean,
                               rvar, batches, bn, perm_c0, momentum, eps);
    });
}

template <class T, bool LK>
__global__ void k_bn_relu(const T* __restrict__ y, T* __restrict__ a, int64_t n4, int C4,
                          const float4* __restrict__ bn, float gs) {
    const int64_t i = (int64_t)blockIdx.x * blockDim.x + threadIdx.x;
    if (i >= n4) return;
    const int c = (C4 & (C4 - 1)) == 0 ? (int)(i & (C4 - 1)) : (int)(i % C4);
    const float4 v = f4(ld4<T>(y + i * 4)), sc = bn[c], sh = bn[C4 + c];
    st4<T>(a + i * 4, f32x4{g_act<LK>(fmaf(v.x, sc.x, sh.x), gs), g_act<LK>(fmaf(v.y, sc.y, sh.y), gs),
                            g_act<LK>(fmaf(v.z, sc.z, sh.z), gs), g_act<LK>(fmaf(v.w, sc.w, sh.w), gs)});
}
void launch_bn_relu(int dt, const void* y, void* a, int64_t R, int C, const float* bn, float gslope, hipStream_t s) {
    const int64_t n4 = R * C / 4;
    SIGGAN_DT_SWITCH(dt, T, {
        if (gslope != 0.f) hipLaunchKernelGGL((k_bn_relu<T, true>), dim3(cdiv(n4, 256)), dim3(256), 0, s, (const T*)y, (T*)a, n4, C / 4,
                                               (const float4*)bn, gslope);
        else hipLaunchKernelGGL((k_bn_relu<T, false>), dim3(cdiv(n4, 256)), dim3(256), 0, s, (const T*)y, (T*)a, n4, C / 4,
                                (const float4*)bn, gslope);
    });
}

template <int W>
__global__ __launch_bounds__(1024) void k_bn_bwd_fin(const float* __restrict__ p0, const float* __restrict__ p1, int nch, int64_t R, int C,
                             float* __restrict__ bn, float* __restrict__ dgamma, float* __restrict__ dbeta, int perm_c0) {
    __shared__ float sh[2][16][64];
    float s, q;
    gather2<W>(p0, p1, nch, C, s, q, sh);
    const int c = blockIdx.x * W + (threadIdx.x & (W - 1));
    if (threadIdx.x >= W || c >= C) return;
    const int t = perm16(c, perm_c0);
    dbeta[t] = s; dgamma[t] = q;
    const float invR = 1.0f / (float)R;
    bn[4 * C + c] = s * invR; bn[5 * C + c] = q * invR;
}
static void launch_bn_bwd_fin(const float* p0, const float* p1, int nch, int64_t R, int C, float* bn, float* dgamma,
                              float* dbeta, int perm_c0, hipStream_t s) {
    if (C <= 32) hipLaunchKernelGGL(k_bn_bwd_fin<32>, dim3(cdiv(C, 32)), dim3(1024), 0, s, p0, p1, nch, R, C, bn, dgamma, dbeta, perm_c0);
    else hipLaunchKernelGGL(k_bn_bwd_fin<64>, dim3(cdiv(C, 64)), dim3(1024), 0, s, p0, p1, nch, R, C, bn, dgamma, dbeta, perm_c0);
}
template <class T, bool LK>
__global__ void k_bn_bwd_apply(T* __restrict__ da, const T* __restrict__ y, int64_t n4, int C4,
                               const float4* __restrict__ bn, float gs) {
    const int64_t i = (int64_t)blockIdx.x * blockDim.x + threadIdx.x;
    if (i >= n4) return;
    const int c = (C4 & (C4 - 1)) == 0 ? (int)(i & (C4 - 1)) : (int)(i % C4);
    const float4 g = f4(ld4<T>(da + i * 4)), yy = f4(ld4<T>(y + i * 4));
    const float4 sc = bn[c], sf = bn[C4 + c], mu = bn[2 * C4 + c], rs = bn[3 * C4 + c], c1 = bn[4 * C4 + c], c2 = bn[5 * C4 + c];
    float4 o;
    o.x = sc.x * (g_dact<LK>(fmaf(yy.x, sc.x, sf.x), g.x, gs) - c1.x - (yy.x - mu.x) * rs.x * c2.x);
    o.y = sc.y * (g_dact<LK>(fmaf(yy.y, sc.y, sf.y), g.y, gs) - c1.y - (yy.y - mu.y) * rs.y * c2.y);
    o.z = sc.z * (g_dact<LK>(fmaf(yy.z, sc.z, sf.z), g.z, gs) - c1.z - (yy.z - mu.z) * rs.z * c2.z);
    o.w = sc.w * (g_dact<LK>(fmaf(yy.w, sc.w, sf.w), g.w, gs) - c1.w - (yy.w - mu.w) * rs.w * c2.w);
    st4<T>(da + i * 4, f32x4{o.x, o.y, o.z, o.w});
}
template <class T, bool LK>
__global__ __launch_bounds__(256) void k_bn_bwd_fin_apply(T* __restrict__ da, const T* __restrict__ y, int64_t R, int C, float* __restrict__ bn,
                                                          const float* __restrict__ p0, const float* __restrict__ p1, int nrows,
                                                          float* __restrict__ dgamma, float* __restrict__ dbeta, int rows_per_chunk,
                                                          float gs) {
    __shared__ f32x4 sh[2][32][8];
    const int c4 = threadIdx.x & 7, rl = threadIdx.x >> 3;
    const int ch = blockIdx.x * 32 + c4 * 4;
    f32x4 s = {0.f, 0.f, 0.f, 0.f}, q = s;
#pragma unroll 4
    for (int k = rl; k < nrows; k += 32) {
        s += *reinterpret_cast<const f32x4*>(p0 + (size_t)k * C + ch);
        q += *reinterpret_cast<const f32x4*>(p1 + (size_t)k * C + ch);
    }
    sh[0][rl][c4] = s; sh[1][rl][c4] = q;
    __syncthreads();
    s = sh[0][0][c4]; q = sh[1][0][c4];
#pragma unroll
    for (int k = 1; k < 32; ++k) { s += sh[0][k][c4]; q += sh[1][k][c4]; }
    const float invR = 1.0f / (float)R;
    const f32x4 c1 = s * invR, c2 = q * invR;
    if (blockIdx.y == 0 && rl == 0) {
        *reinterpret_cast<f32x4*>(dbeta + ch) = s; *reinterpret_cast<f32x4*>(dgamma + ch) = q;
        *reinterpret_cast<f32x4*>(bn + 4 * C + ch) = c1; *reinterpret_cast<f32x4*>(bn + 5 * C + ch) = c2;
    }
    const f32x4 sc = *reinterpret_cast<const f32x4*>(bn + ch), sf = *reinterpret_cast<const f32x4*>(bn + C + ch);
    const f32x4 mu = *reinterpret_cast<const f32x4*>(bn + 2 * C + ch), rs = *reinterpret_cast<const f32x4*>(bn + 3 * C + ch);
    const int64_t r0 = (int64_t)blockIdx.y * rows_per_chunk, r1 = r0 + rows_per_chunk < R ? r0 + rows_per_chunk : R;
#pragma unroll 4
    for (int64_t r = r0 + rl; r < r1; r += 32) {
        const size_t i = (size_t)r * C + ch;
        const f32x4 g = ld4<T>(da + i), yy = ld4<T>(y + i);
        f32x4 o;
#pragma unroll
        for (int e = 0; e < 4; ++e)
            o[e] = sc[e] * (g_dact<LK>(fmaf(yy[e], sc[e], sf[e]), g[e], gs) - c1[e] - (yy[e] - mu[e]) * rs[e] * c2[e]);
        st4<T>(da + i, o);
    }
}
void launch_bn_bwd(int dt, void* dav, const void* yv, int64_t R, int C, float* bn, float* partial,
                   float* dgamma, float* dbeta, int perm_c0, float gslope, hipStream_t s, int pre_rows, hipEvent_t done) {
    const ColPlan pl = col_plan(R, C);
    const int nch = pre_rows > 0 ? pre_rows : pl.nch;
    float* p0 = partial; float* p1 = partial + (size_t)nch * C;
    const int64_t n4 = R * C / 4;
    if (pre_rows > 0 && perm_c0 == 0 && (C % 32) == 0) {
        const int slices = C / 32;
        int64_t chunks = 256 / slices; if (chunks < 1) chunks = 1;
        if (chunks > (R + 63) / 64) chunks = (R + 63) / 64;
        int rpc = (int)((R + chunks - 1) / chunks); rpc = ((rpc + 31) / 32) * 32;
        chunks = (R + rpc - 1) / rpc;
        SIGGAN_GS_SWITCH(gslope, LK, SIGGAN_DT_SWITCH(dt, T, SIGGAN_LAUNCH_EV(done, (k_bn_bwd_fin_apply<T, LK>), dim3(slices, (unsigned)chunks),
                                                                      dim3(256), 0, s, (T*)dav, (const T*)yv, R, C, bn, p0, p1, nch,
                                                                      dgamma, dbeta, rpc, gslope)));
        return;
    }
    SIGGAN_GS_SWITCH(gslope, LK, SIGGAN_DT_SWITCH(dt, T, {
        T* da = (T*)dav; const T* y = (const T*)yv;
        if (pre_rows <= 0)
            hipLaunchKernelGGL((k_colreduce<FBnBwd<T, LK>>), dim3(pl.cbx, pl.nch), dim3(256), 0, s,
                               FBnBwd<T, LK>{da, y, (const float4*)bn, gslope}, R, C, pl.cg, pl.rows, p0, p1);
        launch_bn_bwd_fin(p0, p1, nch, R, C, bn, dgamma, dbeta, perm_c0, s);
        SIGGAN_LAUNCH_EV(done, (k_bn_bwd_apply<T, LK>), dim3(cdiv(n4, 256)), dim3(256), 0, s, da, y, n4, C / 4, (const float4*)bn, gslope);
    }));
}

template <class T, bool LK>
__global__ __launch_bounds__(256) void k_fc_fwd(const float* __restrict__ z, const float* __restrict__ Wt,
                                                const float* __restrict__ b, T* __restrict__ y, int B, int K, int C0,
                                                const float* __restrict__ bn, const DevState* __restrict__ st, uint32_t sid,
                                                float* __restrict__ z_out, float gs) {
    extern __shared__ float sz[];
    const int F = C0 * 16;
    const int fp = blockIdx.x * 256 + threadIdx.x, nb = blockIdx.y * 8;
    if (z) {
        for (int i = threadIdx.x; i < 8 * K; i += 256) {
            const int n = nb + i / K;
            sz[i] = n < B ? z[(size_t)n * K + i % K] : 0.f;
        }
    } else {
        const int64_t e0 = (int64_t)nb * K;
        const int rows = B - nb < 8 ? B - nb : 8, cnt = rows * K;
        for (int i = threadIdx.x; i < 2 * K; i += 256) {
            const int q = i * 4;
            float v[4] = {0.f, 0.f, 0.f, 0.f};
            if (q < cnt) {
                const f32x4 nv = normal4(draw(st, (uint64_t)(e0 / 4 + i), sid));
                v[0] = nv[0]; v[1] = nv[1]; v[2] = nv[2]; v[3] = nv[3];
            }
#pragma unroll
            for (int j = 0; j < 4; ++j) {
                const bool in = q + j < cnt;
                sz[q + j] = in ? v[j] : 0.f;
                if (in && z_out && blockIdx.x == 0) z_out[e0 + q + j] = v[j];
            }
        }
    }
    __syncthreads();
    if (fp >= F) return;
    float acc[8];
#pragma unroll
    for (int j = 0; j < 8; ++j) acc[j] = 0.f;
    const float* wp = Wt + fp;
    int k = 0;
    for (; k + 50 <= K; k += 50) {
        float w[50];
#pragma unroll
        for (int u = 0; u < 50; ++u) w[u] = wp[(size_t)(k + u) * F];
#pragma unroll
        for (int u = 0; u < 50; ++u)
#pragma unroll
            for (int j = 0; j < 8; ++j) acc[j] = fmaf(sz[j * K + k + u], w[u], acc[j]);
    }
    for (; k + 14 <= K; k += 14) {
        float w[14];
#pragma unroll
        for (int u = 0; u < 14; ++u) w[u] = wp[(size_t)(k + u) * F];
#pragma unroll
        for (int u = 0; u < 14; ++u)
#pragma unroll
            for (int j = 0; j < 8; ++j) acc[j] = fmaf(sz[j * K + k + u], w[u], acc[j]);
    }
    for (; k < K; ++k) {
        const float w = wp[(size_t)k * F];
#pragma unroll
        for (int j = 0; j < 8; ++j) acc[j] = fmaf(sz[j * K + k], w, acc[j]);
    }
    const float bias = b[(fp % C0) * 16 + fp / C0];
    if (bn) {
        const float sc = bn[fp], sf = bn[F + fp];
#pragma unroll
        for (int j = 0; j < 8; ++j)
            if (nb + j < B) st1<T>(y + (size_t)(nb + j) * F + fp, g_act<LK>(fmaf(acc[j] + bias, sc, sf), gs));
        return;
    }
#pragma unroll
    for (int j = 0; j < 8; ++j)
        if (nb + j < B) st1<T>(y + (size_t)(nb + j) * F + fp, acc[j] + bias);
}
void launch_fc_fwd(int dt, const float* z, const float* Wt, const float* b, void* y, int B, int K, int C0, float gslope,
                   hipStream_t s, const float* bn_affine_relu, const DevState* st, uint32_t stream_id, float* z_out) {
    SIGGAN_GS_SWITCH(gslope, LK, SIGGAN_DT_SWITCH(dt, T, hipLaunchKernelGGL((k_fc_fwd<T, LK>), dim3(cdiv(C0 * 16, 256), cdiv(B, 8)), dim3(256),
                                                                     8 * K * sizeof(float), s, z, Wt, b, (T*)y, B, K, C0, bn_affine_relu,
                                                                     st, stream_id, z_out, gslope)));
}
static constexpr int FK = 8;
template <class T>
__global__ __launch_bounds__(256) void k_fc_wgrad(const T* __restrict__ dy, const float* __restrict__ z, float* __restrict__ dW,
                           float* __restrict__ db, int B, int K, int C0) {
    __shared__ float sz[64][FK];
    const int F = C0 * 16;
    const int fp = blockIdx.x * 256 + threadIdx.x, k0 = blockIdx.y * FK;
    float acc[FK], sb = 0.f;
#pragma unroll
    for (int u = 0; u < FK; ++u) acc[u] = 0.f;
    for (int n0 = 0; n0 < B; n0 += 64) {
        __syncthreads();
        for (int i = threadIdx.x; i < 64 * FK; i += 256) {
            const int n = n0 + i / FK, k = k0 + i % FK;
            sz[i / FK][i % FK] = (n < B && k < K) ? z[(size_t)n * K + k] : 0.f;
        }
        __syncthreads();
        if (fp < F) {
            const int nn = B - n0 < 64 ? B - n0 : 64;
            int n = 0;
            for (; n + 8 <= nn; n += 8) {
                float g[8];
#pragma unroll
                for (int v = 0; v < 8; ++v) g[v] = ld1<T>(dy + (size_t)(n0 + n + v) * F + fp);
#pragma unroll
                for (int v = 0; v < 8; ++v) {
                    sb += g[v];
#pragma unroll
                    for (int u = 0; u < FK; ++u) acc[u] = fmaf(g[v], sz[n + v][u], acc[u]);
                }
            }
            for (; n < nn; ++n) {
                const float g = ld1<T>(dy + (size_t)(n0 + n) * F + fp);
                sb += g;
#pragma unroll
                for (int u = 0; u < FK; ++u) acc[u] = fmaf(g, sz[n][u], acc[u]);
            }
        }
    }
    if (fp >= F) return;
    const int f = (fp % C0) * 16 + fp / C0;
#pragma unroll
    for (int u = 0; u < FK; ++u)
        if (k0 + u < K) dW[(size_t)f * K + k0 + u] = acc[u];
    if (blockIdx.y == 0) db[f] = sb;
}
void launch_fc_wgrad(int dt, const void* dy, const float* z, float* dW, float* db, int B, int K, int C0, hipStream_t s) {
    SIGGAN_DT_SWITCH(dt, T, hipLaunchKernelGGL(k_fc_wgrad<T>, dim3(cdiv(C0 * 16, 256), cdiv(K, FK)), dim3(256), 0, s, (const T*)dy, z, dW, db,
                                                B, K, C0));
}

typedef f32x4 f4v;
__device__ __forceinline__ f4v ldg4(const float* p) { return *reinterpret_cast<const f4v*>(p); }
__device__ __forceinline__ int clampi(int v, int hi) { return v < 0 ? 0 : (v > hi ? hi : v); }

struct StripId { int n, y0, x; };
template <int RY>
__device__ __forceinline__ StripId strip_of(int sid, int S, int xi) {
    const int nbx = S >> 5, nby = S / RY;
    StripId r;
    r.x = (sid % nbx) * 32 + xi; sid /= nbx;
    r.y0 = (sid % nby) * RY; r.n = sid / nby;
    return r;
}

template <class T, bool BN, bool LK>
__global__ __launch_bounds__(256) void k_final_fwd(const T* __restrict__ act, const float* __restrict__ Wt,
                                                   const float* __restrict__ b, float* __restrict__ img, int S,
                                                   const float* __restrict__ bn, float gs) {
    constexpr int RY = 4, C = 32;
    const int c4 = threadIdx.x & 7;
    const StripId t = strip_of<RY>(blockIdx.x, S, threadIdx.x >> 3);
    f4v w[9];
#pragma unroll
    for (int k = 0; k < 9; ++k) w[k] = ldg4(Wt + k * 32 + c4 * 4);
    const float bias = b[0];
    f4v sc = {1.f, 1.f, 1.f, 1.f}, sf = {0.f, 0.f, 0.f, 0.f};
    if (BN) { sc = ldg4(bn + c4 * 4); sf = ldg4(bn + C + c4 * 4); }
    const T* base = act + (size_t)t.n * S * S * C + c4 * 4;
    f4v v[RY + 2][3];
#pragma unroll
    for (int r = 0; r < RY + 2; ++r) {
        const int yy = t.y0 + r - 1, yc = clampi(yy, S - 1);
#pragma unroll
        for (int d = 0; d < 3; ++d) {
            const int xx = t.x + d - 1, xc = clampi(xx, S - 1);
            f4v q = ld4<T>(base + ((size_t)yc * S + xc) * C);
            if (BN) q = f4v{g_act<LK>(fmaf(q.x, sc.x, sf.x), gs), g_act<LK>(fmaf(q.y, sc.y, sf.y), gs),
                            g_act<LK>(fmaf(q.z, sc.z, sf.z), gs), g_act<LK>(fmaf(q.w, sc.w, sf.w), gs)};
            v[r][d] = (yy == yc && xx == xc) ? q : f4v{0.f, 0.f, 0.f, 0.f};
        }
    }
#pragma unroll
    for (int r = 0; r < RY; ++r) {
        float acc = 0.f;
#pragma unroll
        for (int kh = 0; kh < 3; ++kh)
#pragma unroll
            for (int kw = 0; kw < 3; ++kw) {
                const f4v a = v[r + kh][kw], ww = w[kh * 3 + kw];
                acc = fmaf(a.x, ww.x, acc); acc = fmaf(a.y, ww.y, acc); acc = fmaf(a.z, ww.z, acc); acc = fmaf(a.w, ww.w, acc);
            }
        acc += __shfl_xor(acc, 4, 8); acc += __shfl_xor(acc, 2, 8); acc += __shfl_xor(acc, 1, 8);
        if (c4 == 0) img[((size_t)t.n * S + t.y0 + r) * S + t.x] = tanhf(acc + bias);
    }
}
void launch_final_fwd(int dt, const void* act, const float* Wt, const float* b, float* img, int B, int S, int C, float gslope,
                      hipStream_t s, const float* bn, hipEvent_t done) {
    (void)C;
    const dim3 grid(B * (S / 4) * (S / 32));
    SIGGAN_DT_SWITCH(dt, T, {
        if (bn && gslope != 0.f) SIGGAN_LAUNCH_EV(done, (k_final_fwd<T, true, true>), grid, dim3(256), 0, s, (const T*)act, Wt, b, img, S, bn, gslope);
        else if (bn) SIGGAN_LAUNCH_EV(done, (k_final_fwd<T, true, false>), grid, dim3(256), 0, s, (const T*)act, Wt, b, img, S, bn, gslope);
        else SIGGAN_LAUNCH_EV(done, (k_final_fwd<T, false, false>), grid, dim3(256), 0, s, (const T*)act, Wt, b, img, S, bn, gslope);
    });
}

template <int RY>
__device__ __forceinline__ float dpre_patch_elem(const float* __restrict__ dpre, int n, int y0, int xb, int S, int idx) {
    constexpr int PW = 34;
    const int r = idx / PW, k = idx - r * PW;
    const int yy = y0 + r - 1, xx = xb + k - 1, yc = clampi(yy, S - 1), xc = clampi(xx, S - 1);
    const float q = dpre[((size_t)n * S + yc) * S + xc];
    return (yy == yc && xx == xc && idx < (RY + 2) * PW) ? q : 0.f;
}
template <int RY>
__device__ __forceinline__ void read_dpre_patch(const float* sp, int xi, float (&d)[RY + 2][3]) {
#pragma unroll
    for (int r = 0; r < RY + 2; ++r)
#pragma unroll
        for (int k = 0; k < 3; ++k) d[r][k] = sp[r * 34 + xi + k];
}
template <int RY>
__device__ __forceinline__ f4v final_dact(const float (&d)[RY + 2][3], const f4v (&w)[9], int r) {
    f4v acc = {0.f, 0.f, 0.f, 0.f};
#pragma unroll
    for (int kh = 0; kh < 3; ++kh)
#pragma unroll
        for (int kw = 0; kw < 3; ++kw) {
            const float g = d[r + 2 - kh][2 - kw];
            const f4v ww = w[kh * 3 + kw];
            acc.x = fmaf(g, ww.x, acc.x); acc.y = fmaf(g, ww.y, acc.y); acc.z = fmaf(g, ww.z, acc.z); acc.w = fmaf(g, ww.w, acc.w);
        }
    return acc;
}

template <class T, int RY, bool LK>
__global__ __launch_bounds__(256) void k_final_bwd_reduce(const float* __restrict__ dpre, const float* __restrict__ Wt,
                                                          const T* __restrict__ y, const float* __restrict__ bn,
                                                          float* __restrict__ p0, float* __restrict__ p1,
                                                          float* __restrict__ pw, int S, int nstrips, float gs) {
    constexpr int C = 32;
    __shared__ f4v sh[2][4][8];
    __shared__ float shw[4][8][37];
    const int c4 = threadIdx.x & 7, wave = threadIdx.x >> 6;
    f4v w[9];
#pragma unroll
    for (int k = 0; k < 9; ++k) w[k] = ldg4(Wt + k * 32 + c4 * 4);
    const f4v sc = ldg4(bn + c4 * 4), sf = ldg4(bn + C + c4 * 4), mu = ldg4(bn + 2 * C + c4 * 4), rs = ldg4(bn + 3 * C + c4 * 4);
    f4v s0 = {0.f, 0.f, 0.f, 0.f}, s1 = s0;
    f4v acc[9];
#pragma unroll
    for (int k = 0; k < 9; ++k) acc[k] = f4v{0.f, 0.f, 0.f, 0.f};
    float sdb = 0.f;
    __shared__ float sp[2][(RY + 2) * 34];
    const int xi = threadIdx.x >> 3;
    f4v yn[RY];
    float pn;
    {
        const StripId t0 = strip_of<RY>(blockIdx.x < (unsigned)nstrips ? blockIdx.x : 0, S, xi);
        const T* yb = y + (((size_t)t0.n * S + t0.y0) * S + t0.x) * C + c4 * 4;
#pragma unroll
        for (int r = 0; r < RY; ++r) yn[r] = ld4<T>(yb + (size_t)r * S * C);
        pn = dpre_patch_elem<RY>(dpre, t0.n, t0.y0, t0.x - xi, S, threadIdx.x);
    }
    int it = 0;
    for (int sid = blockIdx.x; sid < nstrips; sid += gridDim.x, it ^= 1) {
        if (threadIdx.x < (RY + 2) * 34) sp[it][threadIdx.x] = pn;
        __syncthreads();
        f4v yv[RY];
#pragma unroll
        for (int r = 0; r < RY; ++r) yv[r] = yn[r];
        {
            const int nx = sid + gridDim.x < nstrips ? sid + gridDim.x : sid;
            const StripId tn = strip_of<RY>(nx, S, xi);
            const T* yb = y + (((size_t)tn.n * S + tn.y0) * S + tn.x) * C + c4 * 4;
#pragma unroll
            for (int r = 0; r < RY; ++r) yn[r] = ld4<T>(yb + (size_t)r * S * C);
            pn = dpre_patch_elem<RY>(dpre, tn.n, tn.y0, tn.x - xi, S, threadIdx.x);
        }
        float d[RY + 2][3];
        read_dpre_patch<RY>(sp[it], xi, d);
#pragma unroll
        for (int r = 0; r < RY; ++r) {
            const f4v g = final_dact<RY>(d, w, r);
            const f4v v = yv[r];
            const f4v pre = {fmaf(v.x, sc.x, sf.x), fmaf(v.y, sc.y, sf.y), fmaf(v.z, sc.z, sf.z), fmaf(v.w, sc.w, sf.w)};
            const f4v m = {g_dact<LK>(pre.x, g.x, gs), g_dact<LK>(pre.y, g.y, gs), g_dact<LK>(pre.z, g.z, gs), g_dact<LK>(pre.w, g.w, gs)};
            s0 += m;
            s1.x = fmaf(m.x, (v.x - mu.x) * rs.x, s1.x); s1.y = fmaf(m.y, (v.y - mu.y) * rs.y, s1.y);
            s1.z = fmaf(m.z, (v.z - mu.z) * rs.z, s1.z); s1.w = fmaf(m.w, (v.w - mu.w) * rs.w, s1.w);
            const f4v a = {g_act<LK>(pre.x, gs), g_act<LK>(pre.y, gs), g_act<LK>(pre.z, gs), g_act<LK>(pre.w, gs)};
            sdb += d[r + 1][1];
#pragma unroll
            for (int kh = 0; kh < 3; ++kh)
#pragma unroll
                for (int kw = 0; kw < 3; ++kw) {
                    const float gg = d[r + 2 - kh][2 - kw];
                    f4v& q = acc[kh * 3 + kw];
                    q.x = fmaf(a.x, gg, q.x); q.y = fmaf(a.y, gg, q.y); q.z = fmaf(a.z, gg, q.z); q.w = fmaf(a.w, gg, q.w);
                }
        }
    }
#pragma unroll
    for (int o = 8; o < 64; o <<= 1) {
        s0.x += __shfl_xor(s0.x, o); s0.y += __shfl_xor(s0.y, o); s0.z += __shfl_xor(s0.z, o); s0.w += __shfl_xor(s0.w, o);
        s1.x += __shfl_xor(s1.x, o); s1.y += __shfl_xor(s1.y, o); s1.z += __shfl_xor(s1.z, o); s1.w += __shfl_xor(s1.w, o);
#pragma unroll
        for (int k = 0; k < 9; ++k) {
            acc[k].x += __shfl_xor(acc[k].x, o); acc[k].y += __shfl_xor(acc[k].y, o);
            acc[k].z += __shfl_xor(acc[k].z, o); acc[k].w += __shfl_xor(acc[k].w, o);
        }
// ... 871 lines not shown
```

### signature-gan_amd/csrc/siggan.hip

```cpp
#include <hip/hip_runtime.h>
#include <dlfcn.h>
#include <math.h>
#include <stdarg.h>
#include <stdio.h>
#include <stdlib.h>
#include <string.h>
#include <new>
#include <vector>

#include "../../include/siggan.h"
#include "gconv.h"
#include "ops.h"

using namespace siggan;

static thread_local char g_err[512] = "";
static int fail(int code, const char* fmt, ...) {
    va_list ap;
    va_start(ap, fmt);
    vsnprintf(g_err, sizeof g_err, fmt, ap);
    va_end(ap);
    return code;
}
int siggan_set_error(int code, const char* fmt, ...) {
// ... 360 lines not shown

extern "C" int siggan_destroy(siggan_ctx* c) {
    if (!c) return SIGGAN_OK;
    DevGuard dg(c->cfg.device);
    (void)hipDeviceSynchronize();
    if (c->comm) { (void)rccl()->CommDestroy(c->comm); c->comm = nullptr; }
    for (auto& e : c->graphs) (void)hipGraphExecDestroy(e.second);
    for (int i = 0; i < siggan_ctx::NEV; ++i) if (c->ev[i]) (void)hipEventDestroy(c->ev[i]);
    for (int i = 0; i < siggan_ctx::NEV; ++i) if (c->ev_fenced[i]) (void)hipEventDestroy(c->ev_fenced[i]);
    for (int i = 0; i < 2; ++i) if (c->ev_bridge[i]) (void)hipEventDestroy(c->ev_bridge[i]);
    if (c->s_m) (void)hipStreamDestroy(c->s_m);
    if (c->s_a) (void)hipStreamDestroy(c->s_a);
    if (c->s_b) (void)hipStreamDestroy(c->s_b);
    if (c->s_c) (void)hipStreamDestroy(c->s_c);
    if (c->s_n) (void)hipStreamDestroy(c->s_n);
    if (c->ev_ar) (void)hipEventDestroy(c->ev_ar);
    for (int i = 0; i < 2; ++i) if (c->ev_sys[i]) (void)hipEventDestroy(c->ev_sys[i]);
    if (c->ev_gfwd) (void)hipEventDestroy(c->ev_gfwd);
    if (c->ev_dreal) (void)hipEventDestroy(c->ev_dreal);
    if (c->ws) (void)hipFree(c->ws);
    if (c->ride_late) (void)hipHostFree(c->ride_late);
    delete c;
    return SIGGAN_OK;
}

extern "C" int64_t siggan_param_count(const siggan_ctx* c, int which) { return !c ? -1 : (which == 0 ? c->g_total : c->d_total); }
extern "C" int32_t siggan_param_tensors(const siggan_ctx* c, int which) {
    return !c ? -1 : (int32_t)(which == 0 ? c->g_off.size() : c->d_off.size());
}
extern "C" int siggan_param_span(const siggan_ctx* c, int which, int32_t idx, int64_t* offset, int64_t* numel) {
    if (!c || !offset || !numel) return fail(SIGGAN_E_INVALID, "null argument");
    const auto& o = which == 0 ? c->g_off : c->d_off;
    const auto& n = which == 0 ? c->g_num : c->d_num;
    if (idx < 0 || idx >= (int32_t)o.size()) return fail(SIGGAN_E_INVALID, "tensor index %d out of range", idx);
    *offset = o[idx]; *numel = n[idx];
    return SIGGAN_OK;
}
extern "C" int64_t siggan_bn_count(const siggan_ctx* c) { return c ? c->bn_total : -1; }
extern "C" int64_t siggan_sn_count(const siggan_ctx* c, int which) {
    if (!c) return -1;
    int64_t ut = 1, vt = (int64_t)c->dC[c->Ld] * 16;
    for (int l = 1; l <= c->Ld; ++l) { ut += c->dC[l]; vt += (int64_t)c->dC[l - 1] * 16; }
    return which == 0 ? ut : vt;
}
extern "C" int32_t siggan_bn_layers(const siggan_ctx* c) { return c ? c->Lg + 1 : -1; }
extern "C" int64_t siggan_workspace_bytes(const siggan_ctx* c) { return c ? (int64_t)c->ws_bytes : -1; }

static void drop_dreal(siggan_ctx* c) {
    if (c->dreal_B) { c->dreal_orphan = true; c->dreal_B = 0; }
}
static int settle(siggan_ctx* c, hipStream_t s) {
    if (c->dreal_orphan) {
        HIPCHK(hipStreamWaitEvent(s, c->ev_dreal, 0));
        c->dreal_orphan = false;
    }
    return SIGGAN_OK;
}

extern "C" int siggan_bind(siggan_ctx* c, const siggan_storage* st) {
    if (!c || !st) return fail(SIGGAN_E_INVALID, "null argument");
    const void* need[] = {st->g_params, st->g_bn_running_mean, st->g_bn_running_var, st->d_params};
    for (const void* p : need)
        if (!p) return fail(SIGGAN_E_INVALID, "siggan_bind: parameters and BatchNorm buffers are required");
    const void* all[] = {st->g_params, st->g_grads, st->g_exp_avg, st->g_exp_avg_sq, st->d_params, st->d_grads,
                         st->d_exp_avg, st->d_exp_avg_sq};
    for (const void* p : all)
        if (((uintptr_t)p & 15) != 0) return fail(SIGGAN_E_INVALID, "siggan_bind: arenas must be 16-byte aligned");
    c->st = *st;
    if (c->sn) {
        if (!st->d_sn_u || !st->d_sn_v) return fail(SIGGAN_E_INVALID, "siggan_bind: a spectral-norm context needs d_sn_u / d_sn_v");
        SnTable& t = c->snt; memset(&t, 0, sizeof t);
        t.n = c->Ld + 1;
        int uo = 0, vo = 0;
        t.pre_k[0] = t.pre_r[0] = 0;
        for (int i = 0; i < t.n; ++i) {
            SnLayer& L = t.layer[i];
            const bool cls = i == c->Ld;
            const int pi = cls ? di_cls_w(c) : di_w(i + 1);
            L.W = st->d_params + c->d_off[pi]; L.w_off = c->d_off[pi];
            L.rows = cls ? 1 : c->dC[i + 1]; L.K = cls ? c->dC[c->Ld] * 16 : c->dC[i] * 16;
            L.u_off = uo; L.v_off = vo; uo += L.rows; vo += L.K;
            t.pre_k[i + 1] = t.pre_k[i] + (L.K + 255) / 256;
            t.pre_r[i + 1] = t.pre_r[i] + (L.rows + 3) / 4;
        }
        t.u = st->d_sn_u; t.v = st->d_sn_v; t.tbuf = c->sn_tbuf; t.wbuf = c->sn_wbuf; t.sig = c->sn_sig;
        t.u_saved = c->sn_us; t.v_saved = c->sn_vs; t.dots = c->sn_dots; t.u_total = uo; t.v_total = vo;
    }
    c->bound = true; c->g_dirty = c->d_dirty = true; c->pending = 0; c->staged_B = 0; c->conv1_rode = 0;
    c->adam_t_known[0] = c->adam_t_known[1] = false;
    c->early_ar = false;
    drop_dreal(c);
    return SIGGAN_OK;
}
extern "C" int siggan_params_changed(siggan_ctx* c) {
    if (!c) return fail(SIGGAN_E_INVALID, "null context");
    c->g_dirty = c->d_dirty = true;
    c->conv1_rode = 0;
    c->adam_t_known[0] = c->adam_t_known[1] = false;
    c->early_ar = false;
    drop_dreal(c);
    return SIGGAN_OK;
}
extern "C" int siggan_seed(siggan_ctx* c, uint64_t seed, uint64_t offset) {
    if (!c) return fail(SIGGAN_E_INVALID, "null context");
    DevGuard dg_(c->cfg.device); HIPCHK(dg_.err);
    unsigned long long v[2] = {seed, offset};
    HIPCHK(hipMemcpy(c->dev, v, sizeof v, hipMemcpyHostToDevice));
    drop_dreal(c);
    return SIGGAN_OK;
}

extern "C" int siggan_rng_state(siggan_ctx* c, uint64_t* seed, uint64_t* offset) {
    ENTER(c);
    if (!seed || !offset) return fail(SIGGAN_E_INVALID, "null argument");
    HIPCHK(hipDeviceSynchronize());
    unsigned long long v[2];
    HIPCHK(hipMemcpy(v, c->dev, sizeof v, hipMemcpyDeviceToHost));
    *seed = v[0]; *offset = v[1];
    return SIGGAN_OK;
}

static int check_bn_batch(const siggan_ctx* c, int batch) {
    if (batch == 1)
        return fail(SIGGAN_E_INVALID, "Expected more than 1 value per channel when training, got input size torch.Size([1, %d])", c->F);
    return SIGGAN_OK;
}
static int check_call(siggan_ctx* c, int batch, bool need_bound = true) {
    if (!c) return fail(SIGGAN_E_INVALID, "null context");
    if (need_bound && !c->bound) return fail(SIGGAN_E_STATE, "siggan_bind has not been called");
    if (batch < 1 || batch > c->Bm) return fail(SIGGAN_E_INVALID, "batch %d outside [1, max_batch=%d]", batch, c->Bm);
    return SIGGAN_OK;
}

static void repack(siggan_ctx* c, hipStream_t sg, hipStream_t sd, bool do_g, bool do_d, int sn_slot = 0, const float* conv1_x = nullptr,
                   int conv1_r0 = 0, int conv1_B = 0) {
    if (do_g) {
        PrepTable t; t.njobs = 0; t.overflow = 0;
        PrepJob j; memset(&j, 0, sizeof j);
        if (!c->fc_fused) {
            j.type = PREP_FC_T; j.O = c->latent; j.I = c->gC[0]; j.src = GP(c, gi_fc_w()); j.dst = c->wfc_t;
            prep_add(t, j, (long long)c->latent * c->F);
        }
        for (int l = 1; l <= c->Lg; ++l) {
            const long long n = (long long)c->gC[l - 1] * c->gC[l] * 16;
            memset(&j, 0, sizeof j);
            j.src = GP(c, gi_up_w(l)); j.dt = c->dt;
            j.type = PREP_PACK_UP; j.I = c->gC[l - 1]; j.O = c->gC[l]; j.dst = (float*)c->g_up[l];
            prep_add(t, j, n);
            j.type = PREP_PACK_DOWN; j.O = c->gC[l - 1]; j.I = c->gC[l]; j.dst = (float*)c->g_dn[l];
            prep_add(t, j, n);
        }
        for (int l = 0; l <= c->Lg; ++l) {
            const int C = l == 0 ? c->F : c->gC[l];
            memset(&j, 0, sizeof j);
            j.type = PREP_BN_EVAL; j.O = C; j.perm = l == 0 ? c->gC[0] : 0;
            j.src = GP(c, gi_bn_w(l)); j.src2 = GP(c, gi_bn_b(l));
            j.src3 = c->st.g_bn_running_mean + c->g_bn_off[l]; j.src4 = c->st.g_bn_running_var + c->g_bn_off[l];
            j.dst = c->g_bne[l];
            prep_add(t, j, C);
        }
        memset(&j, 0, sizeof j);
        j.type = PREP_TAPS; j.I = 9; j.O = c->gC[c->Lg]; j.src = GP(c, gi_fin_w(c)); j.dst = c->wfin_t;
        prep_add(t, j, 9 * j.O);
        if (!launch_prepare(t, BN_EPS, sg)) c->lane_err = hipErrorInvalidValue;
    }
    if (do_d) {
        PrepTable t; t.njobs = 0; t.overflow = 0;
        PrepJob j;
        for (int l = 2; l <= c->Ld; ++l) {
            const long long n = (long long)c->dC[l - 1] * c->dC[l] * 16;
            memset(&j, 0, sizeof j);
            j.src = DP(c, di_w(l)); j.dt = c->dt;
            if (c->sn) j.mul = c->sn_sig + (sn_slot * 2 + 1) * SnTable::MAXS + (l - 1);
            j.type = PREP_PACK_DOWN; j.O = c->dC[l]; j.I = c->dC[l - 1]; j.dst = (float*)c->d_dn[l];
            prep_add(t, j, n);
            j.type = PREP_PACK_UP; j.I = c->dC[l]; j.O = c->dC[l - 1]; j.dst = (float*)c->d_up[l];
            prep_add(t, j, n);
        }
        memset(&j, 0, sizeof j);
        j.type = PREP_CLS; j.O = c->dC[c->Ld]; j.src = DP(c, di_cls_w(c)); j.dst = c->wcp;
        if (c->sn) j.mul = c->sn_sig + (sn_slot * 2 + 1) * SnTable::MAXS + c->Ld;
        prep_add(t, j, (long long)c->dC[c->Ld] * 16);
        if (c->sn) {
            memset(&j, 0, sizeof j);
            j.type = PREP_SCALE; j.O = c->dC[1] * 16; j.src = DP(c, di_w(1)); j.dst = c->d_w1s;
            j.mul = c->sn_sig + (sn_slot * 2 + 1) * SnTable::MAXS;
            prep_add(t, j, j.O);
        }
        memset(&j, 0, sizeof j);
        j.type = PREP_TAPS; j.I = 16; j.O = c->dC[1]; j.src = DP(c, di_w(1)); j.dst = c->d_w1t;
        if (c->sn) j.mul = c->sn_sig + (sn_slot * 2 + 1) * SnTable::MAXS;
        prep_add(t, j, j.O * 16);
        bool ok;
        if (conv1_x && !c->sn) {
            const int64_t H = c->S >> 1;
            char* out = c->d_a[1] + (size_t)((int64_t)conv1_r0 * H * H * c->dC[1]) * c->es;
            ok = launch_prepare_conv1(t, BN_EPS, c->dt, conv1_x, DP(c, di_w(1)), DP(c, di_b(1)), c->cfg.leaky_slope, out, conv1_B, c->S, sd);
        } else {
            ok = launch_prepare(t, BN_EPS, sd);
        }
        if (!ok) c->lane_err = hipErrorInvalidValue;
    }
}

static bool ap_table_g(siggan_ctx* c, ApTable& t) {
    if (!c->fc_fused || c->gC[c->Lg] * 9 > 1024) return false;
    for (int l = 0; l <= c->Lg; ++l) if (c->gC[l] % 16) return false;
    t.njobs = 0; t.overflow = 0;
    ApJob j;
    memset(&j, 0, sizeof j);
    j.type = AP_FLAT; j.off = c->g_off[gi_fc_w()]; j.n = c->g_num[gi_fc_w()] + c->g_num[gi_fc_b()];
    ap_add(t, j);
    for (int l = 0; l <= c->Lg; ++l) {
        if (l > 0) {
            memset(&j, 0, sizeof j);
            j.type = AP_CONV; j.A = c->gC[l - 1]; j.Bc = c->gC[l]; j.dt = c->dt; j.off = c->g_off[gi_up_w(l)];
            j.dst = (float*)c->g_dn[l]; j.dst2 = (float*)c->g_up[l];
            ap_add(t, j);
        }
        memset(&j, 0, sizeof j);
        j.type = AP_BN; j.A = l == 0 ? c->F : c->gC[l]; j.Bc = l == 0 ? c->gC[0] : 0;
        j.off = c->g_off[gi_bn_w(l)]; j.off2 = c->g_off[gi_bn_b(l)];
        j.rmean = c->st.g_bn_running_mean + c->g_bn_off[l]; j.rvar = c->st.g_bn_running_var + c->g_bn_off[l];
        j.dst = c->g_bne[l];
        ap_add(t, j);
    }
    memset(&j, 0, sizeof j);
    j.type = AP_TAPS; j.A = c->gC[c->Lg]; j.Bc = 9; j.off = c->g_off[gi_fin_w(c)]; j.n = 9 * c->gC[c->Lg];
    j.off2 = c->g_off[gi_fin_b(c)]; j.n2 = 1; j.dst = c->wfin_t;
    ap_add(t, j);
    return !t.overflow;
}
static bool ap_table_d(siggan_ctx* c, ApTable& t, int nride) {
    if (c->sn || c->dC[1] * 16 > 1024 || c->dC[1] > 256) return false;
    for (int l = 1; l <= c->Ld; ++l) if (c->dC[l] % 16) return false;
    t.njobs = 0; t.overflow = 0;
    ApJob j;
    memset(&j, 0, sizeof j);
    j.type = AP_TAPS; j.A = c->dC[1]; j.Bc = 16; j.off = c->d_off[di_w(1)]; j.n = 16 * c->dC[1];
    j.off2 = c->d_off[di_b(1)]; j.n2 = c->dC[1]; j.dst = c->d_w1t; j.wait = nride;
    ap_add(t, j);
    for (int l = 2; l <= c->Ld; ++l) {
        memset(&j, 0, sizeof j);
        j.type = AP_CONV; j.A = c->dC[l]; j.Bc = c->dC[l - 1]; j.dt = c->dt; j.off = c->d_off[di_w(l)];
        j.dst = (float*)c->d_dn[l]; j.dst2 = (float*)c->d_up[l];
        ap_add(t, j);
        memset(&j, 0, sizeof j);
        j.type = AP_FLAT; j.off = c->d_off[di_b(l)]; j.n = c->dC[l];
        ap_add(t, j);
    }
    memset(&j, 0, sizeof j);
    j.type = AP_T16; j.A = c->dC[c->Ld]; j.off = c->d_off[di_cls_w(c)]; j.dst = c->wcp;
    ap_add(t, j);
    memset(&j, 0, sizeof j);
    j.type = AP_FLAT; j.off = c->d_off[di_cls_b(c)]; j.n = 1;
    ap_add(t, j);
    return !t.overflow;
}

static int lane_check(siggan_ctx* c) {
    if (c->comm_err)
        return fail(SIGGAN_E_HIP, "ncclAllReduce of the gradient bucket failed (the optimiser update was skipped): %s",
                    rccl()->GetErrorString(c->comm_err));
    if (c->ride_late && __atomic_load_n(c->ride_late, __ATOMIC_ACQUIRE))
        return fail(SIGGAN_E_STATE, "riders did not report: the optimiser update's owner of the first Discriminator block stopped "
                                    "waiting for them (a G step's first block may have used twice-updated weights)");
    if (c->lane_err == hipSuccess) return SIGGAN_OK;
    const hipError_t e = c->lane_err; c->lane_err = hipSuccess;
    return fail(SIGGAN_E_HIP, "an event record / stream wait / prepare table of the step failed: %s", hipGetErrorString(e));
}
struct Lanes {
    siggan_ctx* c;
    hipStream_t m, a, b;
    bool ext;
    hipEvent_t tail_wait;
    hipEvent_t fork_event(hipStream_t to) { return (ext && to != m) ? next() : nullptr; }
    void fork_after(hipStream_t to, hipEvent_t done) {
        if (to == m) return;
        if (done) note(hipStreamWaitEvent(to, done, 0)); else fork(to);
    }
    hipEvent_t next() { hipEvent_t e = (c->comm ? c->ev_fenced : c->ev)[c->evi]; c->evi = (c->evi + 1) % siggan_ctx::NEV; return e; }
    void fork(hipStream_t to) {
        if (to == m) return;
        hipEvent_t e = next();
        note(hipEventRecord(e, m)); note(hipStreamWaitEvent(to, e, 0));
    }
    void join(hipStream_t from) {
        if (from == m) return;
        hipEvent_t e = next();
        note(hipEventRecord(e, from)); note(hipStreamWaitEvent(m, e, 0));
    }
    void note(hipError_t e) { if (e != hipSuccess && c->lane_err == hipSuccess) c->lane_err = e; }
    void record(hipEvent_t e, hipStream_t s) { note(hipEventRecord(e, s)); }
    void wait(hipStream_t s, hipEvent_t e) { note(hipStreamWaitEvent(s, e, 0)); }
};

static GConvArgs gconv_args(siggan_ctx* c) {
    GConvArgs a; memset(&a, 0, sizeof a);
    a.dt = c->dt; a.gslope = c->cfg.g_leaky_slope;
    a.slab = c->slab_k; a.slab_floats = c->slab_k_floats; a.zeros = c->zeros;
    return a;
}

static void g_forward_pass(siggan_ctx* c, const float* z, int B, bool training, float* img, hipStream_t s,
                           float* partial = nullptr, float* slab_k = nullptr, uint32_t rng_sid = 0, float* z_out = nullptr,
                           hipEvent_t done = nullptr) {
    if (!partial) partial = c->partial;
    char* const* const A = training ? c->g_a : c->g_ae;
    const float gs = c->cfg.g_leaky_slope;
    if (c->fc_fused && launch_fc_fwd_fused(c->dt, z, GP(c, gi_fc_w()), GP(c, gi_fc_b()), c->fc_y, A[0], GP(c, gi_bn0_w()),
                                          GP(c, gi_bn0_b()), c->st.g_bn_running_mean, c->st.g_bn_running_var, c->st.g_bn_batches,
                                          c->g_bn[0], training ? nullptr : c->g_bne[0], z_out, c->dev, rng_sid, B, c->latent,
                                          c->gC[0], BN_MOMENTUM, BN_EPS, gs, s)) {
    } else if (!training) {
        launch_fc_fwd(c->dt, z, c->wfc_t, GP(c, gi_fc_b()), A[0], B, c->latent, c->gC[0], gs, s, c->g_bne[0], c->dev, rng_sid, z_out);
    } else {
        launch_fc_fwd(c->dt, z, c->wfc_t, GP(c, gi_fc_b()), c->fc_y, B, c->latent, c->gC[0], gs, s, nullptr, c->dev, rng_sid, z_out);
        launch_bn_train_stats(c->dt, c->fc_y, B, c->F, GP(c, gi_bn0_w()), GP(c, gi_bn0_b()), c->st.g_bn_running_mean,
                              c->st.g_bn_running_var, c->st.g_bn_batches, c->g_bn[0], partial, c->gC[0], BN_MOMENTUM,
                              BN_EPS, s);
        launch_bn_relu(c->dt, c->fc_y, A[0], B, c->F, c->g_bn[0], gs, s);
    }
    for (int l = 1; l <= c->Lg; ++l) {
        const int Hi = 4 << (l - 1), Ci = c->gC[l - 1], Co = c->gC[l];
        GConvArgs a = gconv_args(c);
        if (slab_k) a.slab = slab_k;
        a.in = A[l - 1]; a.wp = c->g_up[l]; a.B = B; a.Hi = Hi; a.Wi = Hi; a.Ci = Ci; a.Co = Co;
        a.lgHr = ilog2i(Hi); a.lgWr = a.lgHr; a.Ho = 2 * Hi; a.Wo = 2 * Hi; a.form = 1; a.M = B * Hi * Hi;
        const int C = Co;
        const int64_t off = c->g_bn_off[l];
        if (training) {
            a.out = c->g_y[l]; a.epi = EPI_RAW;
            launch_gconv(a, s);
            const int64_t R = (int64_t)B * 4 * Hi * Hi;
            launch_bn_train_stats(c->dt, c->g_y[l], R, C, GP(c, gi_bn_w(l)), GP(c, gi_bn_b(l)), c->st.g_bn_running_mean + off,
                                  c->st.g_bn_running_var + off, c->st.g_bn_batches + l, c->g_bn[l], partial, 0,
                                  BN_MOMENTUM, BN_EPS, s);
            if (l < c->Lg) launch_bn_relu(c->dt, c->g_y[l], A[l], R, C, c->g_bn[l], gs, s);
        } else {
            a.out = A[l]; a.epi = EPI_AFFINE_RELU; a.scale = c->g_bne[l]; a.shift = c->g_bne[l] + C;
            launch_gconv(a, s);
        }
    }
    if (training)
        launch_final_fwd(c->dt, c->g_y[c->Lg], c->wfin_t, GP(c, gi_fin_b(c)), img, B, c->S, c->gC[c->Lg], gs, s, c->g_bn[c->Lg], done);
    else
        launch_final_fwd(c->dt, A[c->Lg], c->wfin_t, GP(c, gi_fin_b(c)), img, B, c->S, c->gC[c->Lg], gs, s, nullptr, done);
    c->ga_last_B = training ? B : 0;
}

static void d_forward_rows(siggan_ctx* c, const float* x, int r0, int nB, bool dropout, hipStream_t s, float* slab_k,
                           bool fuse_cls = false, bool conv1_done = false) {
    const float slope = c->cfg.leaky_slope;
    auto act = [&](int l) { const int64_t H = c->S >> l; return c->d_a[l] + (size_t)((int64_t)r0 * H * H * c->dC[l]) * c->es; };
    auto nz = [&](int l) { return dropout ? c->d_noise[l] + (int64_t)r0 * c->dC[l] : nullptr; };
    if (!conv1_done)
        launch_conv1_fwd(c->dt, x, nB, x, c->sn ? c->d_w1s : DP(c, di_w(1)), DP(c, di_b(1)), nz(1), slope, act(1), nB, c->S, c->dC[1], s);
    for (int l = 2; l <= c->Ld; ++l) {
        const int Hi = c->S >> (l - 1), Ho = Hi / 2;
        GConvArgs a = gconv_args(c);
        a.slab = slab_k;
        a.in = act(l - 1); a.wp = c->d_dn[l]; a.out = act(l);
        a.B = nB; a.Hi = Hi; a.Wi = Hi; a.Ci = c->dC[l - 1]; a.Co = c->dC[l];
        a.lgHr = ilog2i(Ho); a.lgWr = a.lgHr; a.Ho = Ho; a.Wo = Ho; a.form = 0; a.M = nB * Ho * Ho;
        a.epi = EPI_BIAS_LRELU_DROP; a.bias = DP(c, di_b(l)); a.noise = nz(l); a.slope = slope;
        const int P_max = c->dC[c->Ld] * 16 / 1024;
        if (l == c->Ld && fuse_cls && P_max >= 1 && P_max <= 16) { a.cls_w = c->wcp; a.cls_part = c->lparts + (size_t)r0 * P_max; }
        const int P = launch_gconv(a, s);
        if (l == c->Ld) c->lP[r0 == 0 ? 0 : 1] = a.cls_w ? P : 0;
    }
    if (c->lP[r0 == 0 ? 0 : 1] == 0)
        launch_cls_fwd(c->dt, act(c->Ld), c->wcp, DP(c, di_cls_b(c)), c->logits + r0, nB, c->dC[c->Ld] * 16, s);
}

struct BceSpec { int n0; float y0, y1; float* mt; int is_g; };

static void d_backward_pass(siggan_ctx* c, Lanes& L, const float* x0, int n0, const float* x1, int Bd, bool dropout,
                            bool want_wgrad, bool want_dimage, const BceSpec& bce, int r0 = 0, float* garena = nullptr,
                            bool early_allreduce = false) {
    const float slope = c->cfg.leaky_slope;
    const int Ld = c->Ld;
    float* const ga = garena ? garena : c->st.d_grads;
    auto G_ = [&](int i) { return ga + c->d_off[i]; };
    auto act = [&](int l) { const int64_t H = c->S >> l; return c->d_a[l] + (size_t)((int64_t)r0 * H * H * c->dC[l]) * c->es; };
    auto dvp = [&](int l) { const int64_t H = c->S >> l; return c->d_dv[l] + (size_t)((int64_t)r0 * H * H * c->dC[l]) * c->es; };
    auto nz = [&](int l) { return dropout ? c->d_noise[l] + (int64_t)r0 * c->dC[l] : nullptr; };
    hipStream_t const sb = want_wgrad ? L.b : L.m;
    const int hP = c->lP[r0 == 0 ? 0 : 1];
    const int P = (r0 == 0 && Bd > bce.n0 && bce.n0 > 0 && c->lP[1] != hP) ? -1 : hP;
    if (P < 0) { c->lane_err = hipErrorInvalidValue; return; }
    const float* const parts = P ? c->lparts + (size_t)r0 * P : nullptr;
    const float* const bc = DP(c, di_cls_b(c));
    if (sb != L.m) {
        L.fork(L.b);
        launch_bce(c->logits + r0, Bd, bce.n0, bce.y0, bce.y1, c->probs + r0, c->dlogit + r0, bce.mt, bce.is_g, sb, c->gscale, parts, P, bc);
    }
    launch_cls_bwd(c->dt, c->logits + r0, bce.n0, bce.y0, bce.y1, c->wcp, act(Ld), nz(Ld), slope, dvp(Ld), Bd,
                   c->dC[Ld], L.m, c->gscale, c->probs + r0, c->dlogit + r0, bce.mt, bce.is_g, sb == L.m, parts, P, bc);
    if (want_wgrad)
        launch_cls_wgrad(c->dt, c->dlogit + r0, act(Ld), G_(di_cls_w(c)), G_(di_cls_b(c)), Bd, c->dC[Ld], sb);
    for (int l = Ld; l >= 2; --l) {
        const int Ho = c->S >> l, Hi = 2 * Ho, Co = c->dC[l], Ci = c->dC[l - 1];
        const bool w_main = want_wgrad && l == 2 && c->dt != DT_F32 && garena == nullptr;
        auto wgrad_l = [&](hipStream_t st, float* slab) {
            WgradArgs w; memset(&w, 0, sizeof w); w.zeros = c->zeros; w.dt = c->dt;
            w.S = dvp(l); w.L = act(l - 1); w.slab = slab; w.dw = G_(di_w(l)); w.B = Bd; w.Cs = Co; w.Cl = Ci;
            w.lgHs = ilog2i(Ho); w.lgWs = w.lgHs; w.lgCl = ilog2i(Ci); w.K = Bd * Ho * Ho;
            w.db = G_(di_b(l));
            const int max_splits = (int)(c->slab_floats / ((int64_t)Co * (16 * Ci + 1)));
            launch_wgrad(w, max_splits, st);
        };
        if (want_wgrad && !w_main) {
            L.fork(L.a);
            wgrad_l(L.a, c->slab);
            if (early_allreduce && l == Ld && c->comm && !c->comm_err && garena == nullptr) {
                hipEvent_t ea = c->ev_sys[0], eb = c->ev_sys[1];
                L.record(ea, L.a); L.record(eb, sb);
                L.wait(c->s_n, ea); L.wait(c->s_n, eb);
                const int64_t o = c->d_off[di_w(l)];
                const int rc = rccl()->AllReduce(ga + o, ga + o, (size_t)(c->d_total - o), NCCL_FLOAT32, NCCL_SUM, c->comm, c->s_n);
                if (rc != NCCL_SUCCESS) c->comm_err = rc;
                else { L.record(c->ev_ar, c->s_n); c->early_ar = true; }
            }
        }
        GConvArgs a = gconv_args(c);
        a.in = dvp(l); a.wp = c->d_up[l]; a.out = dvp(l - 1);
        a.B = Bd; a.Hi = Ho; a.Wi = Ho; a.Ci = Co; a.Co = Ci;
        a.lgHr = ilog2i(Ho); a.lgWr = a.lgHr; a.Ho = Hi; a.Wo = Hi; a.form = 1; a.M = Bd * Ho * Ho;
        a.epi = EPI_LRELU_BWD; a.aref = act(l - 1); a.noise = nz(l - 1); a.slope = slope;
        launch_gconv(a, L.m);
        if (w_main) {
            L.fork(L.b);
            launch_conv1_wgrad(c->dt, dvp(1), x0, n0, x1, G_(di_w(1)), G_(di_b(1)), c->partial_b, Bd, c->S, c->dC[1], L.b);
            wgrad_l(L.m, c->slab_b);
        }
    }
    if (want_wgrad && c->dt != DT_F32 && garena == nullptr) {
        L.join(L.a);
        L.join(L.b);
    } else if (want_wgrad) {
        launch_conv1_wgrad(c->dt, dvp(1), x0, n0, x1, G_(di_w(1)), G_(di_b(1)), c->partial_b, Bd, c->S, c->dC[1], L.m);
        L.join(L.b);
        if (L.tail_wait) L.wait(L.m, L.tail_wait);
        L.join(L.a);
    }
    if (want_dimage)
        launch_conv1_dgrad_tanh(c->dt, dvp(1), c->d_w1t, x0, c->dpre, Bd, c->S, c->dC[1], L.m);
}

static void g_backward_pass(siggan_ctx* c, Lanes& L, const float* z, int B) {
    const float gs = c->cfg.g_leaky_slope;
    const int Lg = c->Lg, S = c->S;
    int pre_rows = 0;
    for (int l = Lg; l >= 1; --l) {
        const int Hi = 4 << (l - 1), Ho = 2 * Hi, Ci = c->gC[l - 1], Co = c->gC[l];
        const int64_t R = (int64_t)B * Ho * Ho;
        hipEvent_t const ef = L.fork_event(L.a);
        if (l == Lg) {
            launch_final_bwd_reduce(c->dt, c->dpre, c->wfin_t, c->g_y[l], B, S, Co, c->g_bn[l], c->partial, c->partial_b, gs, L.m);
            launch_final_bn_bwd_apply(c->dt, c->dpre, c->wfin_t, c->g_y[l], c->g_da[l], B, S, Co, c->g_bn[l], c->partial, c->partial_b,
                                      GG(c, gi_fin_w(c)), GG(c, gi_fin_b(c)), GG(c, gi_bn_w(l)), GG(c, gi_bn_b(l)), gs, L.m, ef);
        } else
            launch_bn_bwd(c->dt, c->g_da[l], c->g_y[l], R, Co, c->g_bn[l], c->partial, GG(c, gi_bn_w(l)), GG(c, gi_bn_b(l)), 0, gs, L.m, pre_rows, ef);
        L.fork_after(L.a, ef);
        WgradArgs w; memset(&w, 0, sizeof w); w.zeros = c->zeros; w.dt = c->dt;
        w.S = c->g_a[l - 1]; w.L = c->g_da[l]; w.slab = c->slab; w.dw = GG(c, gi_up_w(l)); w.B = B; w.Cs = Ci; w.Cl = Co;
        w.lgHs = ilog2i(Hi); w.lgWs = w.lgHs; w.lgCl = ilog2i(Co); w.K = B * Hi * Hi;
        const int max_splits = (int)(c->slab_floats / ((int64_t)Ci * (16 * Co + 1)));
        launch_wgrad(w, max_splits, L.a);
        GConvArgs a = gconv_args(c);
        a.in = c->g_da[l]; a.wp = c->g_dn[l]; a.out = c->g_da[l - 1];
        a.B = B; a.Hi = Ho; a.Wi = Ho; a.Ci = Co; a.Co = Ci;
        a.lgHr = ilog2i(Hi); a.lgWr = a.lgHr; a.Ho = Hi; a.Wo = Hi; a.form = 0; a.M = B * Hi * Hi; a.epi = EPI_RAW;
        if (l >= 2) {
            a.epi = EPI_BN_BWD_STATS; a.aref = c->g_y[l - 1]; a.bnp = c->g_bn[l - 1]; a.stat0 = c->partial; a.stat_cap = PARTIAL_FLOATS;
        }
        pre_rows = launch_gconv(a, L.m);
    }
    if (!(c->fc_fused && launch_fc_bwd_fused(c->dt, c->g_da[0], c->fc_y, z, c->g_bn[0], GG(c, gi_fc_w()), GG(c, gi_fc_b()),
                                             GG(c, gi_bn0_w()), GG(c, gi_bn0_b()), B, c->latent, c->gC[0], gs, L.m))) {
        launch_bn_bwd(c->dt, c->g_da[0], c->fc_y, B, c->F, c->g_bn[0], c->partial, GG(c, gi_bn0_w()), GG(c, gi_bn0_b()),
                      c->gC[0], gs, L.m);
        launch_fc_wgrad(c->dt, c->g_da[0], z, GG(c, gi_fc_w()), GG(c, gi_fc_b()), B, c->latent, c->gC[0], L.m);
    }
    L.join(L.a);
}

static void make_noise(siggan_ctx* c, const float* masks, int B, int p0, int p1, hipStream_t s, uint32_t ctr_add = 0) {
    const float keep = 1.0f - c->cfg.dropout;
    int64_t sumC = 0;
    for (int l = 1; l <= c->Ld; ++l) sumC += c->dC[l];
    if (!masks) {
        float* out[8]; int64_t n[8], e0[8]; uint32_t sid[8];
        for (int l = 1; l <= c->Ld; ++l) {
            const int64_t nl = (int64_t)B * c->dC[l];
            out[l - 1] = c->d_noise[l] + p0 * nl; n[l - 1] = nl * (p1 - p0); e0[l - 1] = p0 * nl; sid[l - 1] = 16 + l;
        }
        launch_dropnoise_multi(c->Ld, out, n, e0, sid, keep, c->dev, s, ctr_add);
        return;
    }
    int64_t pre = 0;
    for (int l = 1; l <= c->Ld; ++l) {
        const int64_t n = (int64_t)B * c->dC[l];
        for (int p = p0; p < p1; ++p)
            launch_mask_to_noise(masks + (int64_t)p * B * sumC + (int64_t)B * pre, c->d_noise[l] + p * n, n, keep, s);
        pre += c->dC[l];
    }
}

static int check_hyper(const siggan_hyper* hp) {
    if (!hp) return fail(SIGGAN_E_INVALID, "null hyper-parameters");
    if (!(hp->lr >= 0.0) || !(hp->beta1 >= 0.0 && hp->beta1 < 1.0) || !(hp->beta2 >= 0.0 && hp->beta2 < 1.0) || !(hp->eps >= 0.0))
        return fail(SIGGAN_E_INVALID, "invalid Adam hyper-parameters");
    return SIGGAN_OK;
}

static const float SN_EPS = 1e-12f;

static void phase_d_grads_sn(siggan_ctx* c, Lanes& L, const PhaseKey& k) {
    const int B = k.B;
    const bool drop = c->cfg.dropout > 0.f;
    repack(c, L.m, L.m, k.g_dirty != 0, false);
    if (k.pre_real)
        L.note(hipMemcpyAsync(c->real_stage, c->staged_src, (size_t)B * c->S * c->S * sizeof(float), hipMemcpyDeviceToDevice, L.m));
    if (drop) make_noise(c, k.has_masks ? c->mask_stage : nullptr, B, 0, 2, L.m);
    const float* fake = c->img;
    if (k.variant == SIGGAN_STEP_ABLATION) {
        g_forward_pass(c, k.has_zg ? c->z_g : nullptr, B, true, c->img_g, L.m, nullptr, nullptr, 2, c->z_g);
        L.record(c->ev_gfwd, L.m);
        fake = c->img_g;
    } else {
        g_forward_pass(c, k.has_z ? c->z : nullptr, B, false, c->img, L.m, nullptr, nullptr, 1, c->z);
    }
    launch_sn_sigma(c->snt, 1, 0, SN_EPS, L.m);
    repack(c, L.m, L.m, false, true, 0);
    d_forward_rows(c, c->real_stage, 0, B, drop, L.m, c->slab_k);
    launch_sn_sigma(c->snt, 1, 1, SN_EPS, L.m);
    repack(c, L.m, L.m, false, true, 1);
    d_forward_rows(c, fake, B, B, drop, L.m, c->slab_k);
    launch_bce(c->logits, 2 * B, B, k.ls, 0.f, c->probs, c->dlogit, k.mt, 0, L.m, c->gscale);
    d_backward_pass(c, L, fake, B, fake, B, drop, true, false, BceSpec{B, 0.f, 0.f, nullptr, 0}, B, c->sn_g[1]);
    repack(c, L.m, L.m, false, true, 0);
    d_backward_pass(c, L, c->real_stage, B, c->real_stage, B, drop, true, false, BceSpec{B, k.ls, k.ls, nullptr, 0}, 0, c->sn_g[0]);
    c->snt.slot[0] = 0; c->snt.slot[1] = 1;
    launch_sn_combine(c->snt, c->sn_g[0], c->sn_g[1], c->st.d_grads, c->d_total, 2, L.m);
}

static void phase_d_grads(siggan_ctx* c, Lanes& L, const PhaseKey& k) {
    c->early_ar = false;
    if (c->sn) return phase_d_grads_sn(c, L, k);
    const int B = k.B;
    const bool drop = c->cfg.dropout > 0.f;
    const bool nolane = k.pre_real == 2 && !k.d_dirty && (!drop || c->dreal_noise2);
    const float* xreal = c->real_stage;
    if (nolane) {
        repack(c, L.m, L.m, k.g_dirty != 0, false);
        xreal = c->staged_src;
    } else {
    L.fork(L.a);
    repack(c, L.m, L.a, k.g_dirty != 0, k.d_dirty != 0);
    if (k.pre_real)
        L.note(hipMemcpyAsync(c->real_stage, c->staged_src, (size_t)B * c->S * c->S * sizeof(float), hipMemcpyDeviceToDevice, L.a));
    if (drop && !(k.pre_real == 2 && c->dreal_noise2))
        make_noise(c, k.has_masks ? c->mask_stage : nullptr, B, k.pre_real == 2 ? 1 : 0, 2, L.a);
    if (k.pre_real != 2) d_forward_rows(c, c->real_stage, 0, B, drop, L.a, c->slab_k2, true);
    }
    const float* fake = c->img;
    const bool spec_fwd = k.spec_g && k.variant != SIGGAN_STEP_ABLATION;
    const bool spec_early = spec_fwd && c->dt != DT_F32;
    hipEvent_t e_early = nullptr, e_eval = nullptr;
    if (spec_early) { e_early = L.next(); L.record(e_early, L.m); }
    if (k.variant == SIGGAN_STEP_ABLATION) {
        g_forward_pass(c, k.has_zg ? c->z_g : nullptr, B, true, c->img_g, L.m, nullptr, nullptr, 2, c->z_g);
        L.record(c->ev_gfwd, L.m);
        fake = c->img_g;
    } else {
        if (spec_fwd && !spec_early && nolane) e_eval = L.fork_event(c->s_c);
        g_forward_pass(c, k.has_z ? c->z : nullptr, B, false, c->img, L.m, nullptr, nullptr, 1, c->z, e_eval);
    }
    if (spec_early) {
        L.wait(c->s_c, e_early);
        g_forward_pass(c, k.has_zg ? c->z_g : nullptr, B, true, c->img_g, c->s_c, c->partial_c, c->slab_k3, 2, c->z_g);
        L.record(c->ev_gfwd, c->s_c);
    }
    if (!nolane) L.join(L.a);
    hipEvent_t e_spec = nullptr;
    if (spec_fwd && !spec_early) { e_spec = e_eval; if (!e_spec) { e_spec = L.next(); L.record(e_spec, L.m); } }
    const bool join_early = k.pre_real == 2 && !c->dreal_joined && drop && c->dreal_noise2;
    if (join_early) L.wait(L.m, c->ev_dreal);
    d_forward_rows(c, fake, B, B, drop, L.m, c->slab_k, true);
    if (k.pre_real == 2 && !c->dreal_joined && !join_early) L.wait(L.m, c->ev_dreal);
    c->dreal_joined = c->dreal_noise2 = false;
    if (spec_fwd && !spec_early) {
        L.wait(c->s_c, e_spec);
        g_forward_pass(c, k.has_zg ? c->z_g : nullptr, B, true, c->img_g, c->s_c, c->partial_c, c->slab_k2, 2, c->z_g);
        L.record(c->ev_gfwd, c->s_c);
    }
    c->gfwd_joined = false;
    if (spec_fwd && c->dt == DT_F32) { L.tail_wait = c->ev_gfwd; c->gfwd_joined = true; }
    d_backward_pass(c, L, xreal, B, fake, 2 * B, drop, true, false, BceSpec{B, k.ls, 0.f, k.mt, 0}, 0, nullptr, k.coll != 0);
    L.tail_wait = nullptr;
    if (spec_fwd && c->dt != DT_F32) { L.wait(L.m, c->ev_gfwd); c->gfwd_joined = true; }
}

static void phase_g_grads(siggan_ctx* c, Lanes& L, const PhaseKey& k) {
    const int B = k.B;
    const float* zg; float* img;
    const bool d_pack = !c->sn && k.d_dirty != 0;
    bool conv1_done = false;
    if (k.spec_g) {
        if (!c->gfwd_joined) L.wait(L.m, c->ev_gfwd);
        c->gfwd_joined = false;
        conv1_done = k.rode || (d_pack && k.variant != SIGGAN_STEP_ABLATION);
        repack(c, L.m, L.m, false, d_pack, 0, (conv1_done && !k.rode) ? c->img_g : nullptr, B, B);
        zg = c->z_g; img = c->img_g;
    } else {
        L.fork(L.a);
        repack(c, L.m, L.a, k.g_dirty != 0, d_pack);
        g_forward_pass(c, k.has_z ? c->z : nullptr, B, true, c->img, L.m, nullptr, nullptr, 2, c->z);
        L.join(L.a);
        zg = c->z; img = c->img;
    }
    const bool abl = k.variant == SIGGAN_STEP_ABLATION;
    const bool gdrop = abl && c->cfg.dropout > 0.f;
    if (c->sn) {
        launch_sn_sigma(c->snt, abl ? 1 : 0, 2, SN_EPS, L.m);
        repack(c, L.m, L.m, false, true, 2);
    }
    if (gdrop) {
        int64_t sumC = 0;
        for (int l = 1; l <= c->Ld; ++l) sumC += c->dC[l];
        make_noise(c, k.has_masks ? c->mask_stage + (int64_t)2 * B * sumC : nullptr, B, 0, 1, L.m);
    }
    const float gy = abl ? k.ls : 1.0f;
    const int r0g = (!abl && !c->sn) ? B : 0;
    c->g_r0 = r0g;
    const bool real_early = k.pre_real && r0g != 0;
    if (real_early) {
        const bool drop = c->cfg.dropout > 0.f;
        L.fork(c->s_c);
        if (drop) make_noise(c, nullptr, B, 0, 2, c->s_c, 1);
        c->dreal_noise2 = drop;
        d_forward_rows(c, c->staged_src, 0, B, drop, c->s_c, c->slab_k2, true);
        L.record(c->ev_dreal, c->s_c);
    }
    d_forward_rows(c, img, r0g, B, gdrop, L.m, c->slab_k, true, conv1_done);
    d_backward_pass(c, L, img, B, img, B, gdrop, false, true, BceSpec{B, gy, gy, k.mt, 1}, r0g);
    if (k.pre_real && !real_early) {
        const bool drop = c->cfg.dropout > 0.f;
        L.fork(c->s_c);
        if (drop) make_noise(c, nullptr, B, 0, 1, c->s_c, 1);
        d_forward_rows(c, c->staged_src, 0, B, drop, c->s_c, c->slab_k2, true);
        L.record(c->ev_dreal, c->s_c);
    }
    g_backward_pass(c, L, zg, B);
    if (real_early && c->dt != DT_F32) { L.wait(L.m, c->ev_dreal); c->dreal_joined = true; }
}

static void phase_apply(siggan_ctx* c, Lanes& L, const PhaseKey& k) {
    const int which = k.phase == 2 ? 1 : 0;
    float* p = which == 0 ? c->st.g_params : c->st.d_params;
    float* g = which == 0 ? c->st.g_grads : c->st.d_grads;
    float* m = which == 0 ? c->st.g_exp_avg : c->st.d_exp_avg;
    float* v = which == 0 ? c->st.g_exp_avg_sq : c->st.d_exp_avg_sq;
    float* steps = which == 0 ? c->st.g_adam_steps : c->st.d_adam_steps;
    const int64_t n = which == 0 ? c->g_total : c->d_total;
    const int nt = (int)(which == 0 ? c->g_off.size() : c->d_off.size());
    const bool clip = k.clip > 0.f;
    float gs = k.gs / c->gscale;
    if (c->comm) {
        if (c->comm_err) return;
        if (which == 1 && c->early_ar) {
            const int64_t o = c->d_off[di_w(c->Ld)];
            const int e = rccl()->AllReduce(g, g, (size_t)o, NCCL_FLOAT32, NCCL_SUM, c->comm, L.m);
            c->early_ar = false;
            if (e != NCCL_SUCCESS) { c->comm_err = e; return; }
            L.wait(L.m, c->ev_ar);
        } else {
        const int e = rccl()->AllReduce(g, g, (size_t)n, NCCL_FLOAT32, NCCL_SUM, c->comm, L.m);
        if (e != NCCL_SUCCESS) { c->comm_err = e; return; }
        }
        gs *= 1.0f / (float)c->comm_world;
    }
    const bool guard = c->dt == DT_F16;
    if (clip || guard) launch_grad_sumsq(g, n, c->dev, c->partial, L.m);
    if (k.fused_t > 0.0 && k.pack) {
        ApTable t;
        ApRide rd; memset(&rd, 0, sizeof rd);
        if (k.ride) {
            if (!c->gfwd_joined) { L.wait(L.m, c->ev_gfwd); c->gfwd_joined = true; }
            const int64_t H = c->S >> 1;
            rd.x = c->img_g; rd.out = c->d_a[1] + (size_t)((int64_t)k.ride * H * H * c->dC[1]) * c->es; rd.B = k.ride; rd.S = c->S;
            rd.dt = c->dt; rd.slope = c->cfg.leaky_slope; rd.w_off = c->d_off[di_w(1)]; rd.b_off = c->d_off[di_b(1)];
            rd.counter = (unsigned*)c->ride_ctr; rd.late = c->ride_late_dev;
        }
        const bool ok = (which == 0 ? ap_table_g(c, t) : ap_table_d(c, t, k.ride ? k.ride * (c->S / 4) : 0)) &&
            launch_adam_pack(t, p, g, m, v, c->dev, steps, nt, k.fused_t, k.lr, k.beta1, k.beta2, k.eps, gs, k.clip,
                             k.mt + (which == 0 ? SIGGAN_M_G_GRAD_NORM : SIGGAN_M_D_GRAD_NORM), clip ? c->partial : nullptr,
                             k.mt + (which == 0 ? SIGGAN_M_G_SKIPPED : SIGGAN_M_D_SKIPPED), BN_EPS, k.ride ? &rd : nullptr, L.m);
        if (!ok) c->lane_err = hipErrorInvalidValue;
        return;
    }
    if (k.fused_t > 0.0) {
        launch_adam_fused(p, g, m, v, n, c->dev, steps, nt, k.fused_t, k.lr, k.beta1, k.beta2, k.eps, gs, k.clip,
                          k.mt + (which == 0 ? SIGGAN_M_G_GRAD_NORM : SIGGAN_M_D_GRAD_NORM), clip ? c->partial : nullptr, L.m,
                          k.mt + (which == 0 ? SIGGAN_M_G_SKIPPED : SIGGAN_M_D_SKIPPED));
        return;
    }
    launch_adam_prepare(c->dev, steps, nt, k.lr, k.beta1, k.beta2, gs, k.clip,
                        k.mt + (which == 0 ? SIGGAN_M_G_GRAD_NORM : SIGGAN_M_D_GRAD_NORM), L.m, guard ? 1 : 0,
                        k.mt + (which == 0 ? SIGGAN_M_G_SKIPPED : SIGGAN_M_D_SKIPPED), (clip || guard) ? c->partial : nullptr);
    launch_adam(p, g, m, v, n, c->dev, k.beta1, k.beta2, k.eps, (clip || gs != 1.0f) ? 1 : 0, L.m);
}

static void run_phase_body(siggan_ctx* c, Lanes& L, const PhaseKey& k) {
    if (k.phase == 0) phase_d_grads(c, L, k);
    else if (k.phase == 1) phase_g_grads(c, L, k);
    else phase_apply(c, L, k);
}

static int run_phase(siggan_ctx* c, const PhaseKey& k, hipStream_t u) {
    const bool overlap = (c->mode & SIGGAN_MODE_OVERLAP) != 0;
    const bool graph = (c->mode & SIGGAN_MODE_GRAPH) != 0 && g_prof == nullptr;
    if (graph && c->comm && k.phase >= 2) return fail(SIGGAN_E_STATE, "SIGGAN_MODE_GRAPH is not available with a communicator");
    if (graph && c->sn) return fail(SIGGAN_E_STATE, "SIGGAN_MODE_GRAPH is not available with spectral normalisation");
    if (!graph) {
        const bool ext = overlap && g_prof == nullptr;
        Lanes L{c, u, overlap ? c->s_a : u, overlap ? c->s_b : u, ext, nullptr};
        run_phase_body(c, L, k);
        LAUNCHCHK();
        return lane_check(c);
    }
    hipGraphExec_t exec = nullptr;
    for (auto& e : c->graphs)
        if (e.first == k) { exec = e.second; break; }
    if (!exec) {
        Lanes L{c, c->s_m, overlap ? c->s_a : c->s_m, overlap ? c->s_b : c->s_m, false, nullptr};
        hipGraph_t g = nullptr;
        HIPCHK(hipStreamBeginCapture(c->s_m, hipStreamCaptureModeRelaxed));
        run_phase_body(c, L, k);
        hipError_t e1 = hipStreamEndCapture(c->s_m, &g);
        if (e1 != hipSuccess || !g) return fail(SIGGAN_E_HIP, "stream capture failed: %s", hipGetErrorString(e1));
        hipError_t e2 = hipGraphInstantiate(&exec, g, nullptr, nullptr, 0);
        (void)hipGraphDestroy(g);
        if (e2 != hipSuccess) return fail(SIGGAN_E_HIP, "hipGraphInstantiate: %s", hipGetErrorString(e2));
        if (c->graphs.size() >= 64) { (void)hipGraphExecDestroy(c->graphs.front().second); c->graphs.erase(c->graphs.begin()); }
        c->graphs.emplace_back(k, exec);
    }
    hipEvent_t e_in = c->ev_bridge[0], e_out = c->ev_bridge[1];
    HIPCHK(hipEventRecord(e_in, u));
    HIPCHK(hipStreamWaitEvent(c->s_m, e_in, 0));
    HIPCHK(hipGraphLaunch(exec, c->s_m));
    HIPCHK(hipEventRecord(e_out, c->s_m));
    HIPCHK(hipStreamWaitEvent(u, e_out, 0));
    return SIGGAN_OK;
}

static PhaseKey make_key(siggan_ctx* c, int phase, int B, bool has_z, bool has_masks, const siggan_hyper* hp,
                         float* metrics_dev) {
    PhaseKey k; memset(&k, 0, sizeof k);
    k.phase = phase; k.B = B; k.has_z = has_z; k.has_masks = has_masks;
    k.mt = metrics_dev ? metrics_dev : c->metrics;
    if (phase <= 1) { k.g_dirty = c->g_dirty; k.d_dirty = c->d_dirty; k.ls = hp->label_smoothing; }
    else {
        k.lr = hp->lr; k.beta1 = hp->beta1; k.beta2 = hp->beta2; k.eps = hp->eps;
        k.clip = hp->clip_max_norm > 0.f ? hp->clip_max_norm : 0.f;
        k.gs = hp->grad_scale > 0.f ? hp->grad_scale : 1.0f;
    }
    return k;
}

static int finish_metrics(siggan_ctx* c, float* metrics_dev, float* metrics_host, hipStream_t s) {
    if (metrics_host) {
        HIPCHK(hipMemcpyAsync(metrics_host, metrics_dev ? metrics_dev : c->metrics, SIGGAN_M_COUNT * sizeof(float),
                              hipMemcpyDeviceToHost, s));
        HIPCHK(hipStreamSynchronize(s));
// ... 106 lines not shown
    ENTER(c);
    int rc = check_call(c, batch);
    if (rc) return rc;
    if (!real_dev) return fail(SIGGAN_E_INVALID, "null real batch");
    drop_dreal(c);
    if ((rc = settle(c, (hipStream_t)stream))) return rc;
    c->staged_src = real_dev;
    c->staged_B = batch;
    return SIGGAN_OK;
}

extern "C" int siggan_d_grads(siggan_ctx* c, const float* real_dev, int32_t batch, const float* z_dev, const float* masks_dev,
                              const siggan_hyper* hp, float* metrics_dev, void* stream) {
    return d_grads_common(c, real_dev, batch, z_dev, masks_dev, hp, metrics_dev, stream, false, nullptr);
}

extern "C" int siggan_step_begin(siggan_ctx* c, const float* real_dev, int32_t batch, const float* z_dev, const float* masks_dev,
                                 const float* zg_dev, const siggan_hyper* hp, float* metrics_dev, void* stream) {
    return d_grads_common(c, real_dev, batch, z_dev, masks_dev, hp, metrics_dev, stream, true, zg_dev, true);
}

static int apply_common(siggan_ctx* c, int which, const siggan_hyper* hp, float* metrics_dev, float* metrics_host, void* stream) {
    ENTER(c);
    int rc = check_call(c, 1);
    if (rc) return rc;
    if ((rc = check_hyper(hp))) return rc;
    if (c->pending != (which == 1 ? 1 : 2))
        return fail(SIGGAN_E_STATE, "siggan_%c_apply without a preceding siggan_%c_grads", which ? 'd' : 'g', which ? 'd' : 'g');
    const float* need[] = {which ? c->st.d_grads : c->st.g_grads, which ? c->st.d_exp_avg : c->st.g_exp_avg,
                           which ? c->st.d_exp_avg_sq : c->st.g_exp_avg_sq, which ? c->st.d_adam_steps : c->st.g_adam_steps};
    for (const float* p : need)
        if (!p) return fail(SIGGAN_E_STATE, "gradient / Adam arenas were not bound");
    hipStream_t s = (hipStream_t)stream;
    if ((rc = settle(c, s))) return rc;
    if (!metrics_dev) metrics_dev = c->metrics_last != c->metrics ? c->metrics_last : nullptr;
    else if (c->metrics_last && metrics_dev != c->metrics_last)
        HIPCHK(hipMemcpyAsync(metrics_dev, c->metrics_last, SIGGAN_M_COUNT * sizeof(float), hipMemcpyDeviceToDevice, (hipStream_t)stream));
    PhaseKey k = make_key(c, which == 1 ? 2 : 3, 0, false, false, hp, metrics_dev);
    const int wi = which == 1 ? 1 : 0;
    if ((c->mode & SIGGAN_MODE_GRAPH) == 0 && c->dt != DT_F16) {
        if (!c->adam_t_known[wi]) {
            float t0 = 0.f;
            HIPCHK(hipStreamSynchronize(s));
            HIPCHK(hipMemcpy(&t0, which == 1 ? c->st.d_adam_steps : c->st.g_adam_steps, sizeof t0, hipMemcpyDeviceToHost));
            c->adam_t[wi] = (double)t0; c->adam_t_known[wi] = true;
        }
        k.fused_t = c->adam_t[wi] + 1.0;
        ApTable probe;
        k.pack = (which == 0 ? ap_table_g(c, probe) : ap_table_d(c, probe, 0)) ? 1 : 0;
        if (which == 1 && k.pack && c->g_fwd_pending && c->variant != SIGGAN_STEP_ABLATION && g_prof == nullptr && c->dt == DT_F32)
            k.ride = c->g_fwd_pending;
    } else {
        c->adam_t_known[wi] = false;
    }
    if ((rc = run_phase(c, k, s))) return rc;
    if (k.fused_t > 0.0) c->adam_t[wi] = k.fused_t;
    if (which == 0) c->g_dirty = !k.pack; else c->d_dirty = !k.pack;
    if (which == 1) c->conv1_rode = k.ride;
    c->pending = 0;
    return finish_metrics(c, metrics_dev, metrics_host, s);
}

extern "C" int siggan_d_apply(siggan_ctx* c, const siggan_hyper* hp, float* metrics_dev, float* metrics_host, void* stream) {
    return apply_common(c, 1, hp, metrics_dev, metrics_host, stream);
}

extern "C" int siggan_d_step(siggan_ctx* c, const float* real_dev, int32_t batch, const float* z_dev, const float* masks_dev,
                             const siggan_hyper* hp, float* metrics_dev, float* metrics_host, void* stream) {
    int rc = d_grads_common(c, real_dev, batch, z_dev, masks_dev, hp, metrics_dev, stream, false, nullptr, true);
    if (rc) return rc;
    return siggan_d_apply(c, hp, metrics_dev, metrics_host, stream);
}

extern "C" int siggan_g_grads(siggan_ctx* c, int32_t batch, const float* z_dev, const siggan_hyper* hp, float* metrics_dev,
                              void* stream) {
    ENTER(c);
    int rc = check_call(c, batch);
    if (rc) return rc;
    if ((rc = check_bn_batch(c, batch))) return rc;
    if ((rc = check_hyper(hp))) return rc;
    if (!c->st.g_grads) return fail(SIGGAN_E_STATE, "gradient arena was not bound");
    hipStream_t s = (hipStream_t)stream;
    if ((rc = settle(c, s))) return rc;
    const int B = batch;
    const bool spec = c->g_fwd_pending != 0;
    if (c->variant == SIGGAN_STEP_ABLATION && !spec)
        return fail(SIGGAN_E_STATE, "ablation step: siggan_g_grads follows the siggan_d_grads / siggan_d_apply of the same iteration");
    if (spec && (c->g_fwd_pending != B || z_dev))
        return fail(SIGGAN_E_STATE, "siggan_g_grads after siggan_step_begin must use the same batch and no explicit z (pass it to step_begin)");
    if (!spec && !z_dev && c->zg_stash == B) z_dev = c->z_g;
    c->zg_stash = 0;
    if (!spec && z_dev && z_dev != c->z) HIPCHK(hipMemcpyAsync(c->z, z_dev, (size_t)B * c->latent * sizeof(float), hipMemcpyDeviceToDevice, s));
    PhaseKey k = make_key(c, 1, B, z_dev != nullptr, false, hp, metrics_dev);
    c->metrics_last = k.mt;
    k.spec_g = spec; k.variant = c->variant; k.has_masks = c->abl_masks;
    k.rode = (spec && c->conv1_rode == B && !c->d_dirty) ? 1 : 0;
    c->conv1_rode = 0;
    c->abl_masks = false;
    k.pre_real = c->staged_B == B && c->dreal_B == 0 && (c->mode & SIGGAN_MODE_OVERLAP) != 0 && (c->mode & SIGGAN_MODE_GRAPH) == 0 &&
                 g_prof == nullptr && c->pending == 0 && !c->sn;
    if ((rc = run_phase(c, k, s))) return rc;
    c->g_rode = k.rode ? B : 0; c->g_pre_real = k.pre_real ? B : 0;
    if (k.pre_real) c->dreal_B = B;
    c->g_fwd_pending = 0;
    c->d_dirty = false;
    c->g_dirty = true;
    c->pending = 2;
    return SIGGAN_OK;
}

extern "C" int siggan_g_apply(siggan_ctx* c, const siggan_hyper* hp, float* metrics_dev, float* metrics_host, void* stream) {
    return apply_common(c, 0, hp, metrics_dev, metrics_host, stream);
}

extern "C" int siggan_g_step(siggan_ctx* c, int32_t batch, const float* z_dev, const siggan_hyper* hp, float* metrics_dev,
                             float* metrics_host, void* stream) {
    int rc = siggan_g_grads(c, batch, z_dev, hp, metrics_dev, stream);
    if (rc) return rc;
    return siggan_g_apply(c, hp, metrics_dev, metrics_host, stream);
}

static bool pow2(int v) { return v > 0 && (v & (v - 1)) == 0; }

extern "C" int siggan_op_conv4x4s2(siggan_ctx* c, int32_t form, const void* in_dev, const float* w_dev, void* out_dev,
                                   int32_t batch, int32_t h_in, int32_t c_in, int32_t c_out, void* stream) {
    if (!c) return fail(SIGGAN_E_INVALID, "null context");
    if (!in_dev || !w_dev || !out_dev) return fail(SIGGAN_E_INVALID, "null tensor");
    if (form != 0 && form != 1) return fail(SIGGAN_E_INVALID, "form must be 0 (down) or 1 (up)");
    if (!pow2(h_in) || !pow2(c_in) || !pow2(c_out) || c_in < 32 || c_out < 32 || c_in > 512 || c_out > 512 || batch < 1)
        return fail(SIGGAN_E_INVALID, "shape not in the model family (pow2 dims, 32 <= C <= 512)");
    if (form == 0 && h_in < 2) return fail(SIGGAN_E_INVALID, "down form needs h_in >= 2");
    DevGuard dg_(c->cfg.device); HIPCHK(dg_.err);
    hipStream_t s = (hipStream_t)stream;
    GConvArgs a = gconv_args(c);
    a.in = in_dev; a.wp = c->op_pack; a.out = out_dev; a.B = batch; a.Hi = h_in; a.Wi = h_in; a.Ci = c_in; a.Co = c_out;
    a.form = form; a.epi = EPI_RAW;
    PrepTable t; t.njobs = 0; t.overflow = 0;
    PrepJob j; memset(&j, 0, sizeof j);
    j.src = w_dev; j.dst = (float*)c->op_pack; j.dt = c->dt;
    if (form == 0) {
        j.type = PREP_PACK_DOWN; j.O = c_out; j.I = c_in;
        a.Ho = a.Wo = h_in / 2; a.lgHr = a.lgWr = ilog2i(h_in / 2); a.M = batch * (h_in / 2) * (h_in / 2);
    } else {
        j.type = PREP_PACK_UP; j.I = c_in; j.O = c_out;
        a.Ho = a.Wo = 2 * h_in; a.lgHr = a.lgWr = ilog2i(h_in); a.M = batch * h_in * h_in;
    }
    prep_add(t, j, (long long)c_in * c_out * 16);
    if (!launch_prepare(t, BN_EPS, s)) return fail(SIGGAN_E_STATE, "prepare table overflow");
    launch_gconv(a, s);
    LAUNCHCHK();
    return SIGGAN_OK;
}

extern "C" int siggan_op_conv4x4s2_wgrad(siggan_ctx* c, const void* small_dev, const void* large_dev, float* dw_dev,
                                         int32_t batch, int32_t h_small, int32_t c_small, int32_t c_large, void* stream) {
    if (!c) return fail(SIGGAN_E_INVALID, "null context");
    if (!small_dev || !large_dev || !dw_dev) return fail(SIGGAN_E_INVALID, "null tensor");
    if (!pow2(h_small) || !pow2(c_small) || !pow2(c_large) || c_small < 32 || c_large < 32 || c_small > 512 || c_large > 512 ||
        batch < 1)
        return fail(SIGGAN_E_INVALID, "shape not in the model family (pow2 dims, 32 <= C <= 512)");
    DevGuard dg_(c->cfg.device); HIPCHK(dg_.err);
    hipStream_t s = (hipStream_t)stream;
    WgradArgs w; memset(&w, 0, sizeof w); w.zeros = c->zeros; w.dt = c->dt;
    w.S = small_dev; w.L = large_dev; w.slab = c->slab; w.dw = dw_dev; w.B = batch; w.Cs = c_small; w.Cl = c_large;
    w.lgHs = w.lgWs = ilog2i(h_small); w.lgCl = ilog2i(c_large); w.K = batch * h_small * h_small;
    const int max_splits = (int)(c->slab_floats / ((int64_t)c_small * (16 * c_large + 1)));
    launch_wgrad(w, max_splits, s);
    LAUNCHCHK();
    return SIGGAN_OK;
}

extern "C" int siggan_op_adam(siggan_ctx* c, float* p, float* g, float* m, float* v, int64_t n, int32_t step,
                              const siggan_hyper* hp, void* stream) {
    if (!c) return fail(SIGGAN_E_INVALID, "null context");
    int rc = check_hyper(hp);
    if (rc) return rc;
    if (!p || !g || !m || !v || n < 1 || step < 1) return fail(SIGGAN_E_INVALID, "bad argument");
    if ((((uintptr_t)p | (uintptr_t)g | (uintptr_t)m | (uintptr_t)v) & 15) != 0) return fail(SIGGAN_E_INVALID, "arenas must be 16-byte aligned");
    DevGuard dg_(c->cfg.device); HIPCHK(dg_.err);
    hipStream_t s = (hipStream_t)stream;
    float* steps = c->partial + ((2 << 20) - 64);
    const float prev = (float)(step - 1);
    HIPCHK(hipMemcpyAsync(steps, &prev, sizeof prev, hipMemcpyHostToDevice, s));
    const bool clip = hp->clip_max_norm > 0.f;
    const float gs = hp->grad_scale > 0.f ? hp->grad_scale : 1.0f;
    if (clip) launch_grad_sumsq(g, n, c->dev, c->partial, s);
    launch_adam_prepare(c->dev, steps, 1, hp->lr, hp->beta1, hp->beta2, gs, hp->clip_max_norm, nullptr, s, 0, nullptr,
                        clip ? c->partial : nullptr);
    launch_adam(p, g, m, v, n, c->dev, hp->beta1, hp->beta2, hp->eps, (clip || gs != 1.0f) ? 1 : 0, s);
    LAUNCHCHK();
    return SIGGAN_OK;
}

extern "C" int siggan_comm_unique_id(void* id_out) {
    if (!id_out) return fail(SIGGAN_E_INVALID, "null argument");
    Rccl* r = rccl();
    if (r->err) return fail(SIGGAN_E_STATE, "%s", r->err);
    ncclUniqueId_t id;
    NCCLCHK(r->GetUniqueId(&id));
    memcpy(id_out, &id, sizeof id);
    return SIGGAN_OK;
}
extern "C" int siggan_comm_init(siggan_ctx* c, int32_t rank, int32_t world, const void* id) {
    ENTER(c);
    if (!id || world < 1 || rank < 0 || rank >= world) return fail(SIGGAN_E_INVALID, "bad rank / world / id");
    if (c->comm) return fail(SIGGAN_E_STATE, "a communicator is already initialised");
    Rccl* r = rccl();
    if (r->err) return fail(SIGGAN_E_STATE, "%s", r->err);
    ncclUniqueId_t uid;
    memcpy(&uid, id, sizeof uid);
    NCCLCHK(r->CommInitRank(&c->comm, world, uid, rank));
    c->comm_rank = rank; c->comm_world = world;
    return SIGGAN_OK;
}
extern "C" int siggan_comm_destroy(siggan_ctx* c) {
    ENTER(c);
    if (!c->comm) return SIGGAN_OK;
    HIPCHK(hipDeviceSynchronize());
    NCCLCHK(rccl()->CommDestroy(c->comm));
    c->comm = nullptr; c->comm_rank = 0; c->comm_world = 1; c->comm_err = 0; c->early_ar = false;
    return SIGGAN_OK;
}
extern "C" int32_t siggan_comm_world(const siggan_ctx* c) { return c ? c->comm_world : -1; }
extern "C" int siggan_comm_broadcast(siggan_ctx* c, void* buf_dev, int64_t bytes, int32_t root, void* stream) {
    ENTER(c);
    if (!buf_dev || bytes < 1 || root < 0 || root >= c->comm_world) return fail(SIGGAN_E_INVALID, "bad argument");
    if (!c->comm) return SIGGAN_OK;
    NCCLCHK(rccl()->Broadcast(buf_dev, buf_dev, (size_t)bytes, NCCL_CHAR, root, c->comm, (hipStream_t)stream));
    return SIGGAN_OK;
}

extern "C" int siggan_device_info(int32_t device, int32_t* compute_units, int32_t* clock_khz, int64_t* hbm_bytes) {
    if (!compute_units || !clock_khz || !hbm_bytes) return fail(SIGGAN_E_INVALID, "null argument");
    hipDeviceProp_t p;
    HIPCHK(hipGetDeviceProperties(&p, device));
    *compute_units = p.multiProcessorCount; *clock_khz = p.clockRate; *hbm_bytes = (int64_t)p.totalGlobalMem;
    return SIGGAN_OK;
}

static Prof g_prof_store;
extern "C" int siggan_prof_enable(siggan_ctx* c, int32_t on) {
    if (!c) return fail(SIGGAN_E_INVALID, "null context");
    DevGuard dg_(c->cfg.device); HIPCHK(dg_.err);
    HIPCHK(hipDeviceSynchronize());
    g_prof_store.clear();
    g_prof = on ? &g_prof_store : nullptr;
    return SIGGAN_OK;
}
extern "C" int32_t siggan_prof_slots(void) { return Prof::NID - 1; }
extern "C" int siggan_prof_read(siggan_ctx* c, int32_t idx, char* name, int32_t name_cap, int64_t* launches, double* ms,
                                double* flops, double* bytes) {
    if (!c || !name || !launches || !ms || !flops || !bytes || idx < 0 || idx >= Prof::NID - 1) return fail(SIGGAN_E_INVALID, "bad argument");
    DevGuard dg_(c->cfg.device); HIPCHK(dg_.err);
    HIPCHK(hipDeviceSynchronize());
    snprintf(name, name_cap, "%s", Prof::name(idx));
    *launches = 0; *ms = 0.0; *flops = 0.0; *bytes = 0.0;
    for (auto& r : g_prof_store.recs) {
        if (r.id != idx) continue;
        float t = 0.f;
        HIPCHK(hipEventElapsedTime(&t, r.e0, r.e1));
        *launches += 1; *ms += t; *flops += r.flops; *bytes += r.bytes;
    }
    return SIGGAN_OK;
}

extern "C" int siggan_debug_tensor(siggan_ctx* c, const char* name, int32_t idx, float* out_dev, int64_t n, void* stream) {
    if (!c || !name || !out_dev || n < 1) return fail(SIGGAN_E_INVALID, "bad argument");
    const void* src = nullptr; int64_t capv = 0;
    const void** ptr = &src; int64_t* cap = &capv;
    bool typed = true;
    const int64_t Bm = c->Bm, Bd = 2 * Bm, SS = (int64_t)c->S * c->S;
    auto gsz = [&](int l) { const int64_t H = 4 << l; return Bm * H * H * c->gC[l]; };
    auto dsz = [&](int l) { const int64_t H = c->S >> l; return Bd * H * H * c->dC[l]; };
    const bool gl = idx >= 0 && idx <= c->Lg, dl = idx >= 1 && idx <= c->Ld;
    if (!strcmp(name, "g_y") && gl) { *ptr = c->g_y[idx]; *cap = gsz(idx); }
    else if (!strcmp(name, "g_a") && gl) { *ptr = c->g_a[idx]; *cap = gsz(idx); }
    else if (!strcmp(name, "g_da") && gl) { *ptr = c->g_da[idx]; *cap = gsz(idx); }
    else if (!strcmp(name, "d_a") && dl) { *ptr = c->d_a[idx]; *cap = dsz(idx); }
    else if (!strcmp(name, "d_dv") && dl) { *ptr = c->d_dv[idx]; *cap = dsz(idx); }
    else if (!strcmp(name, "d_a_g") && dl) {
        const int64_t H = c->S >> idx, off = (int64_t)c->g_r0 * H * H * c->dC[idx];
        *ptr = c->d_a[idx] + (size_t)off * c->es; *cap = dsz(idx) - off;
    }
    else if (!strcmp(name, "z")) { *ptr = c->z; *cap = Bm * c->latent; typed = false; }
    else if (!strcmp(name, "z_g")) { *ptr = c->z_g; *cap = Bm * c->latent; typed = false; }
    else if (!strcmp(name, "img")) { *ptr = c->img; *cap = Bm * SS; typed = false; }
    else if (!strcmp(name, "dpre")) { *ptr = c->dpre; *cap = Bm * SS; typed = false; }
    else if (!strcmp(name, "logits")) { *ptr = c->logits; *cap = Bd; typed = false; }
    else if (!strcmp(name, "probs")) { *ptr = c->probs; *cap = Bd; typed = false; }
    else if (!strcmp(name, "dlogit")) { *ptr = c->dlogit; *cap = Bd; typed = false; }
    else if (!strcmp(name, "d_noise") && dl) { *ptr = c->d_noise[idx]; *cap = Bd * c->dC[idx]; typed = false; }
    else if (!strcmp(name, "rode") || !strcmp(name, "pre_real") || !strcmp(name, "ride_late")) {
        if (n != 1) return fail(SIGGAN_E_INVALID, "debug scalar %s holds 1 float, %lld asked", name, (long long)n);
        DevGuard dg_(c->cfg.device); HIPCHK(dg_.err);
        HIPCHK(hipStreamSynchronize((hipStream_t)stream));
        const float v = !strcmp(name, "rode") ? (float)c->g_rode : !strcmp(name, "pre_real") ? (float)c->g_pre_real
                                                                                               : (float)__atomic_load_n(c->ride_late, __ATOMIC_ACQUIRE);
        HIPCHK(hipMemcpy(out_dev, &v, sizeof v, hipMemcpyHostToDevice));
        return SIGGAN_OK;
    }
    else return fail(SIGGAN_E_INVALID, "unknown debug tensor %s[%d]", name, idx);
    if (n > capv) return fail(SIGGAN_E_INVALID, "debug tensor %s[%d] holds %lld floats, %lld asked", name, idx, (long long)capv, (long long)n);
    DevGuard dg_(c->cfg.device); HIPCHK(dg_.err);
    if (!strcmp(name, "g_a") && idx == c->Lg && c->ga_last_B) {
        const int64_t H = c->S;
        HIPCHK(hipDeviceSynchronize());
        launch_bn_relu(c->dt, c->g_y[idx], c->g_a[idx], (int64_t)c->ga_last_B * H * H, c->gC[idx], c->g_bn[idx], c->cfg.g_leaky_slope,
                       (hipStream_t)stream);
        LAUNCHCHK();
    }
    if (typed && c->dt != DT_F32) { launch_to_f32(c->dt, src, out_dev, n, (hipStream_t)stream); LAUNCHCHK(); }
    else HIPCHK(hipMemcpyAsync(out_dev, src, (size_t)n * sizeof(float), hipMemcpyDeviceToDevice, (hipStream_t)stream));
    return SIGGAN_OK;
}

extern "C" int siggan_augment_batch(int32_t device, const uint8_t* cache_dev, int64_t n_images, const int32_t* index_dev,
                                    const int32_t* params_dev, const int16_t* tables_dev, const float* lut_dev, float* out_dev,
                                    int32_t batch, int32_t size, int32_t augment, int32_t fill, void* stream) {
    if (!cache_dev || !index_dev || !lut_dev || !out_dev) return fail(SIGGAN_E_INVALID, "null tensor");
    if (augment && (!params_dev || !tables_dev)) return fail(SIGGAN_E_INVALID, "augment needs params and tables");
    if (batch < 1 || n_images < 1 || size < 1 || size > 1024) return fail(SIGGAN_E_INVALID, "bad batch / cache / image size");
    if (fill < 0 || fill > 255) return fail(SIGGAN_E_INVALID, "fill must be a byte value");
    DevGuard dg_(device); HIPCHK(dg_.err);
    launch_augment(cache_dev, n_images, index_dev, params_dev, tables_dev, lut_dev, out_dev, batch, size, augment != 0, fill, (hipStream_t)stream);
    LAUNCHCHK();
    return SIGGAN_OK;
}

extern "C" int siggan_op_randn(siggan_ctx* c, float* out_dev, int64_t n, void* stream) {
    if (!c || !out_dev || n < 1) return fail(SIGGAN_E_INVALID, "bad argument");
    DevGuard dg_(c->cfg.device); HIPCHK(dg_.err);
    hipStream_t s = (hipStream_t)stream;
    launch_tick(c->dev, s);
    launch_randn(out_dev, n, c->dev, 3, s);
    LAUNCHCHK();
    return SIGGAN_OK;
}
```

Measured before the change: 45240 images/s.

## Fuse generator BatchNorm activation and BN backward into conv and wgrad operand loads

For f32 generator layers with at most 256 channels, the separate BN+ReLU forward pass and the BN backward apply pass are no longer run as standalone elementwise kernels. Instead the conv and weight-gradient kernels read the raw pre-BN tensor and apply the affine+activation, or the BN backward formula, while staging operands into shared memory. This is meant to remove full-tensor read/write round trips and kernel launches. The cost is extra loads of y and BN parameters inside the GEMM loops, higher register pressure, and recomputing the transform on every reuse.

```diff
diff --git a/signature-gan_amd/csrc/act.h b/signature-gan_amd/csrc/act.h
--- a/signature-gan_amd/csrc/act.h
+++ b/signature-gan_amd/csrc/act.h
@@ -50,6 +50,13 @@
 template <bool LK> __device__ __forceinline__ float g_act(float x, float gs) { return LK ? (x > 0.f ? x : x * gs) : fmaxf(x, 0.f); }
 template <bool LK> __device__ __forceinline__ float g_dact(float x, float g, float gs) { return x > 0.f ? g : (LK ? g * gs : 0.f); }
 
+template <bool LK> __device__ __forceinline__ float g_bn_act(float y, float sc, float sf, float gs) { return g_act<LK>(fmaf(y, sc, sf), gs); }
+template <bool LK>
+__device__ __forceinline__ float g_bn_bwd(float g, float y, float sc, float sf, float mu, float rs, float c1, float c2, float gs) {
+    const float d = g_dact<LK>(fmaf(y, sc, sf), g, gs);
+    return __fmul_rn(sc, __fsub_rn(__fsub_rn(d, c1), __fmul_rn(__fmul_rn(__fsub_rn(y, mu), rs), c2)));
+}
+
 #define SIGGAN_GS_SWITCH(GS, LK, ...)                                                   \
     do {                                                                         \
         if ((GS) != 0.f) { constexpr bool LK = true; __VA_ARGS__; }              \
diff --git a/signature-gan_amd/csrc/gconv.h b/signature-gan_amd/csrc/gconv.h
--- a/signature-gan_amd/csrc/gconv.h
+++ b/signature-gan_amd/csrc/gconv.h
@@ -43,7 +43,12 @@
     int64_t slab_floats;
     size_t slab_stride;
     const float* zeros;
+    int in_tf;
+    const void* in_y;
+    const float* in_bn;
 };
+enum OperandTf : int { TF_NONE = 0, TF_BN_ACT = 1, TF_BN_BWD = 2 };
+static constexpr int TF_MAX_C = 256;
 
 struct BnBwdParams { f32x4 sc, sf, mu, rs; };
 __device__ __forceinline__ BnBwdParams bn_bwd_params(const float* __restrict__ bnp, int Co, int co) {
@@ -63,7 +68,7 @@
     }
 }
 __host__ __device__ inline bool gen_lk(const GConvArgs& a) {
-    return a.gslope != 0.f && (a.epi == EPI_AFFINE_RELU || a.epi == EPI_BN_BWD_STATS);
+    return a.gslope != 0.f && (a.epi == EPI_AFFINE_RELU || a.epi == EPI_BN_BWD_STATS || a.in_tf != TF_NONE);
 }
 
 struct WgradArgs {
@@ -78,6 +83,10 @@
     int K;
     int kchunk;
     const float* zeros;
+    const float* S_bn;
+    const float* L_y;
+    const float* L_bn;
+    float gslope;
 };
 
 struct Prof {
diff --git a/signature-gan_amd/csrc/gconv.hip b/signature-gan_amd/csrc/gconv.hip
--- a/signature-gan_amd/csrc/gconv.hip
+++ b/signature-gan_amd/csrc/gconv.hip
@@ -12,13 +12,19 @@
     return (xcd < r ? xcd * (q + 1) : r * (q + 1) + (xcd - r) * q) + idx;
 }
 
-template <int BM, int BN, int WM, int WN, int BK = 32, int DEEP = 0, int KQ = 1, bool LK = false>
+template <int BM, int BN, int WM, int WN, int BK = 32, int DEEP = 0, int KQ = 1, bool LK = false, int TF = TF_NONE>
 __global__ __launch_bounds__(256 * KQ) void k_gconv(const GConvArgs a) {
     constexpr int TM = BM / (32 * WM), TN = BN / (32 * WN);
     constexpr int PA = BM / 32, PB = BN / 32;
     constexpr int KC = BK / 32;
     constexpr int LD = BK + 4;
-    __shared__ __attribute__((aligned(16))) float smem[KQ * 2 * LD * (BM + BN)];
+    constexpr int NBN = TF == TF_BN_BWD ? 6 : TF == TF_BN_ACT ? 2 : 0;
+    __shared__ __attribute__((aligned(16))) float smem[KQ * 2 * LD * (BM + BN) + NBN * TF_MAX_C];
+    float* const sBN = smem + KQ * 2 * LD * (BM + BN);
+    if (TF != TF_NONE) {
+        for (int i = threadIdx.x; i < NBN * a.Ci; i += 256 * KQ) sBN[i] = a.in_bn[i];
+        __syncthreads();
+    }
     const int quad = KQ > 1 ? (int)(threadIdx.x >> 8) : 0;
     float* const sA = smem + quad * (2 * LD * (BM + BN));
     float* const sB = sA + 2 * LD * BM;
@@ -63,6 +69,8 @@
 
     const float* a_cur[PA];
     int a_step[PA];
+    bool a_ok[PA];
+    const float* const a_y = static_cast<const float*>(a.in_y);
     int l_tap = k_lo >> lgcpt, l_cc = k_lo & ((1 << lgcpt) - 1);
     auto set_tap = [&]() __attribute__((always_inline)) {
         int dh, dw;
@@ -73,17 +81,28 @@
             const bool ok = (unsigned)ih < (unsigned)a.Hi && (unsigned)iw < (unsigned)a.Wi;
             a_cur[p] = ok ? a_base[p] + ((size_t)(ih * a.Wi + iw) * a.Ci + l_cc * BK) : a.zeros;
             a_step[p] = ok ? BK : 0;
+            a_ok[p] = ok;
         }
     };
     constexpr int NSET = DEEP ? 2 : 1;
     f32x4 ra[NSET][PA][KC], rb[NSET][PB][KC];
+    f32x4 ry[TF == TF_BN_BWD ? NSET : 1][PA][KC];
+    bool s_ok[NSET][PA];
+    int s_ch[NSET];
     auto load_tile = [&](int set = 0) __attribute__((always_inline)) {
 #pragma unroll
         for (int p = 0; p < PA; ++p) {
 #pragma unroll
             for (int q = 0; q < KC; ++q) ra[set][p][q] = *reinterpret_cast<const f32x4*>(a_cur[p] + 32 * q);
+            if (TF == TF_BN_BWD) {
+                const float* ys = a_ok[p] ? a_y + (a_cur[p] - a_in) : a.zeros;
+#pragma unroll
+                for (int q = 0; q < KC; ++q) ry[set][p][q] = *reinterpret_cast<const f32x4*>(ys + 32 * q);
+            }
+            if (TF != TF_NONE) s_ok[set][p] = a_ok[p];
             a_cur[p] += a_step[p];
         }
+        if (TF != TF_NONE) s_ch[set] = l_cc * BK + kc * 4;
 #pragma unroll
         for (int p = 0; p < PB; ++p)
 #pragma unroll
@@ -94,10 +113,35 @@
     auto store_tile = [&](int buf, int set = 0) __attribute__((always_inline)) {
         float* dA = sA + buf * LD * BM + rloc * LD + kc * 4;
         float* dB = sB + buf * LD * BN + rloc * LD + kc * 4;
+        if (TF != TF_NONE) {
+#pragma unroll
+            for (int q = 0; q < KC; ++q) {
+                const int ch = s_ch[set] + 32 * q;
+                const f32x4 sc = *reinterpret_cast<const f32x4*>(sBN + ch), sf = *reinterpret_cast<const f32x4*>(sBN + a.Ci + ch);
+                f32x4 mu, rs, c1, c2;
+                if (TF == TF_BN_BWD) {
+                    mu = *reinterpret_cast<const f32x4*>(sBN + 2 * a.Ci + ch); rs = *reinterpret_cast<const f32x4*>(sBN + 3 * a.Ci + ch);
+                    c1 = *reinterpret_cast<const f32x4*>(sBN + 4 * a.Ci + ch); c2 = *reinterpret_cast<const f32x4*>(sBN + 5 * a.Ci + ch);
+                }
+#pragma unroll
+                for (int p = 0; p < PA; ++p) {
+                    f32x4 v = ra[set][p][q];
+#pragma unroll
+                    for (int e = 0; e < 4; ++e) {
+                        const float t = TF == TF_BN_BWD ? g_bn_bwd<LK>(v[e], ry[TF == TF_BN_BWD ? set : 0][p][q][e], sc[e], sf[e], mu[e], rs[e],
+                                                                       c1[e], c2[e], a.gslope)
+                                                        : g_bn_act<LK>(v[e], sc[e], sf[e], a.gslope);
+                        v[e] = s_ok[set][p] ? t : 0.f;
+                    }
+                    *reinterpret_cast<f32x4*>(dA + 32 * p * LD + 32 * q) = v;
+                }
+            }
+        } else {
 #pragma unroll
         for (int p = 0; p < PA; ++p)
 #pragma unroll
             for (int q = 0; q < KC; ++q) *reinterpret_cast<f32x4*>(dA + 32 * p * LD + 32 * q) = ra[set][p][q];
+        }
 #pragma unroll
         for (int p = 0; p < PB; ++p)
 #pragma unroll
@@ -305,7 +349,7 @@
     }
 }
 
-template <int CI, bool LK>
+template <int CI, bool LK, bool TF = false>
 __global__ __launch_bounds__(256) void k_gconv_up4(const GConvArgs a) {
     constexpr int BM = 128, BN = 32, LD = BK + 4, LP = CI + 4, NCC = CI / BK;
     constexpr int PATCH_PIX = 264;
@@ -340,7 +384,16 @@
             const int i = tid + 256 * q;
             if (i < nchunk) {
                 const int pix = i / (CI / 4), ch = i - pix * (CI / 4);
-                *reinterpret_cast<f32x4*>(sP + pix * LP + ch * 4) = v[q];
+                f32x4 w = v[q];
+                if (TF) {
+                    const int pr = pix / Wp, pc = pix - pr * Wp;
+                    const int ih = rh0 - 1 + pr, iw = pc - 1;
+                    const bool ok = (unsigned)ih < (unsigned)a.Hi && (unsigned)iw < (unsigned)a.Wi;
+                    const f32x4 sc = *reinterpret_cast<const f32x4*>(a.in_bn + ch * 4), sf = *reinterpret_cast<const f32x4*>(a.in_bn + CI + ch * 4);
+#pragma unroll
+                    for (int e = 0; e < 4; ++e) w[e] = ok ? g_bn_act<LK>(w[e], sc[e], sf[e], a.gslope) : 0.f;
+                }
+                *reinterpret_cast<f32x4*>(sP + pix * LP + ch * 4) = w;
             }
         }
     }
@@ -561,6 +614,13 @@
     hipEvent_t e0 = g_prof ? g_prof->recs.back().e0 : nullptr, e1 = g_prof ? g_prof->recs.back().e1 : nullptr;
     if (a.dt != DT_F32) {
         launch_gconv16(id, a, grid, st, e0, e1, KQ);
+    } else if (a.in_tf != TF_NONE) {
+        SIGGAN_GS_SWITCH(gen_lk(a) ? 1.f : 0.f, LK, {
+            if (a.in_tf == TF_BN_BWD)
+                hipExtLaunchKernelGGL((k_gconv<BM, BN, WM, WN, BKT, DEEP, KQ, LK, TF_BN_BWD>), grid, dim3(256 * KQ), 0, st, e0, e1, 0, a);
+            else
+                hipExtLaunchKernelGGL((k_gconv<BM, BN, WM, WN, BKT, DEEP, KQ, LK, TF_BN_ACT>), grid, dim3(256 * KQ), 0, st, e0, e1, 0, a);
+        });
     } else if (gen_lk(a)) {
         hipExtLaunchKernelGGL((k_gconv<BM, BN, WM, WN, BKT, DEEP, KQ, true>), grid, dim3(256 * KQ), 0, st, e0, e1, 0, a);
     } else if (g_prof) {
@@ -600,12 +660,18 @@
         return launch_cfg<64, 64, 2, 2, 32, 1>(a, st, 2, ns);
     }
     if (a.dt == DT_F32 && a.form == 1 && a.Co == 32 && (a.epi == EPI_RAW || a.epi == EPI_AFFINE_RELU) && (a.Ci == 32 || a.Ci == 64) &&
+        (a.in_tf == TF_NONE || a.in_tf == TF_BN_ACT) &&
         a.M / 128 >= (a.Ci == 32 ? 384 : 768) && a.M % 128 == 0 &&
         ((1 << (a.lgHr + a.lgWr)) % 128) == 0 && a.lgWr >= 4 && a.lgWr <= 6) {
         dim3 grid(a.M / 128);
         if (g_prof) g_prof->begin(5, 2.0 * a.M * a.Co * (double)(4 * a.Ci) * 4, gconv_bytes(a), st);
         hipEvent_t e0 = g_prof ? g_prof->recs.back().e0 : nullptr, e1 = g_prof ? g_prof->recs.back().e1 : nullptr;
-        if (gen_lk(a)) {
+        if (a.in_tf == TF_BN_ACT) {
+            SIGGAN_GS_SWITCH(a.gslope, LK, {
+                if (a.Ci == 32) hipExtLaunchKernelGGL((k_gconv_up4<32, LK, true>), grid, dim3(256), 0, st, e0, e1, 0, a);
+                else hipExtLaunchKernelGGL((k_gconv_up4<64, LK, true>), grid, dim3(256), 0, st, e0, e1, 0, a);
+            });
+        } else if (gen_lk(a)) {
             if (a.Ci == 32) hipExtLaunchKernelGGL((k_gconv_up4<32, true>), grid, dim3(256), 0, st, e0, e1, 0, a);
             else hipExtLaunchKernelGGL((k_gconv_up4<64, true>), grid, dim3(256), 0, st, e0, e1, 0, a);
         } else {
@@ -618,8 +684,8 @@
     return launch_cfg<128, 32, 4, 1, 32, 1>(a, st, 3, ns);
 }
 
-template <int BM, int BN, int WM, int WN>
-__global__ __launch_bounds__(256) void k_wgrad(const WgradArgs a) {
+template <int BM, int BN, int WM, int WN, bool SBN = false, bool LBN = false, bool LK = false>
+__global__ __launch_bounds__(256) __attribute__((amdgpu_waves_per_eu(SBN || LBN ? 2 : 1))) void k_wgrad(const WgradArgs a) {
     constexpr int TM = BM / (32 * WM), TN = BN / (32 * WN);
     constexpr int LDA = BM + PAD, LDB = BN + PAD;
     constexpr int CA = BM / 4, RA = 256 / CA, PA = BK / RA;
@@ -650,6 +716,15 @@
     const int kh = tap >> 2, kw = tap & 3;
 
     f32x4 ra[2][PA], rb[2][PB];
+    f32x4 ryl[LBN ? 2 : 1][PB];
+    bool oks[2][PA], okl[2][PB];
+    f32x4 s_sc, s_sf, l_sc, l_sf, l_mu, l_rs, l_c1, l_c2;
+    if (SBN) { s_sc = *reinterpret_cast<const f32x4*>(a.S_bn + i0 + ca * 4); s_sf = *reinterpret_cast<const f32x4*>(a.S_bn + a.Cs + i0 + ca * 4); }
+    if (LBN) {
+        l_sc = *reinterpret_cast<const f32x4*>(a.L_bn + lch);          l_sf = *reinterpret_cast<const f32x4*>(a.L_bn + Cl + lch);
+        l_mu = *reinterpret_cast<const f32x4*>(a.L_bn + 2 * Cl + lch); l_rs = *reinterpret_cast<const f32x4*>(a.L_bn + 3 * Cl + lch);
+        l_c1 = *reinterpret_cast<const f32x4*>(a.L_bn + 4 * Cl + lch); l_c2 = *reinterpret_cast<const f32x4*>(a.L_bn + 5 * Cl + lch);
+    }
     size_t a_off[PA];
     int a_pix[PA], b_pix[PB];
 #pragma unroll
@@ -663,6 +738,7 @@
         _Pragma("unroll") for (int p = 0; p < PA; ++p) {                                              \
             const float* src = a_pix[p] < kend ? a_S + a_off[p] : a.zeros;                            \
             ra[SET][p] = *reinterpret_cast<const f32x4*>(src);                                       \
+            if (SBN) oks[SET][p] = a_pix[p] < kend;                                                   \
             a_off[p] += a_adv; a_pix[p] += BK;                                                        \
         }                                                                                             \
         _Pragma("unroll") for (int p = 0; p < PB; ++p) {                                              \
@@ -674,15 +750,32 @@
             const unsigned off = (((unsigned)(2 * y - 1 + kh) << lgWl) + (unsigned)iw) << a.lgCl;     \
             const float* src = ok ? a_L + ((size_t)off + lch) : a.zeros;                              \
             rb[SET][p] = *reinterpret_cast<const f32x4*>(src);                                       \
+            if (LBN) {                                                                                \
+                ryl[LBN ? SET : 0][p] = *reinterpret_cast<const f32x4*>(ok ? a.L_y + ((size_t)off + lch) : a.zeros); \
+                okl[SET][p] = ok;                                                                     \
+            }                                                                                         \
             b_pix[p] += BK;                                                                           \
         }                                                                                             \
     }
 #define WG_STORE_TILE(BUF, SET)                                                                       \
     {                                                                                                 \
-        _Pragma("unroll") for (int p = 0; p < PA; ++p)                                                \
-            *reinterpret_cast<f32x4*>(sA + (BUF) * BK * LDA + (ka + RA * p) * LDA + ca * 4) = ra[SET][p]; \
-        _Pragma("unroll") for (int p = 0; p < PB; ++p)                                                \
-            *reinterpret_cast<f32x4*>(sB + (BUF) * BK * LDB + (kb + RB * p) * LDB + cb * 4) = rb[SET][p]; \
+        _Pragma("unroll") for (int p = 0; p < PA; ++p) {                                              \
+            f32x4 v = ra[SET][p];                                                                     \
+            if (SBN) {                                                                                \
+                _Pragma("unroll") for (int e = 0; e < 4; ++e)                                         \
+                    v[e] = oks[SET][p] ? g_bn_act<LK>(v[e], s_sc[e], s_sf[e], a.gslope) : 0.f;       \
+            }                                                                                         \
+            *reinterpret_cast<f32x4*>(sA + (BUF) * BK * LDA + (ka + RA * p) * LDA + ca * 4) = v;     \
+        }                                                                                             \
+        _Pragma("unroll") for (int p = 0; p < PB; ++p) {                                              \
+            f32x4 v = rb[SET][p];                                                                     \
+            if (LBN) {                                                                                \
+                _Pragma("unroll") for (int e = 0; e < 4; ++e)                                         \
+                    v[e] = okl[SET][p] ? g_bn_bwd<LK>(v[e], ryl[LBN ? SET : 0][p][e], l_sc[e], l_sf[e], l_mu[e], l_rs[e], \
+                                                      l_c1[e], l_c2[e], a.gslope) : 0.f;              \
+            }                                                                                         \
+            *reinterpret_cast<f32x4*>(sB + (BUF) * BK * LDB + (kb + RB * p) * LDB + cb * 4) = v;     \
+        }                                                                                             \
     }
 
     f32x16 acc[TM][TN];
@@ -799,6 +892,15 @@
 
 static void launch_wgrad_reduce(const float* slab, float* dw, float* db, int nsplit, int Cs, int Cl, hipStream_t st);
 
+template <int BM, int BN, int WM, int WN>
+static void launch_wgrad_tf(const WgradArgs& a, dim3 grid, hipStream_t st, hipEvent_t e0, hipEvent_t e1) {
+    SIGGAN_GS_SWITCH(a.gslope, LK, {
+        if (a.S_bn && a.L_y) hipExtLaunchKernelGGL((k_wgrad<BM, BN, WM, WN, true, true, LK>), grid, dim3(256), 0, st, e0, e1, 0, a);
+        else if (a.S_bn) hipExtLaunchKernelGGL((k_wgrad<BM, BN, WM, WN, true, false, LK>), grid, dim3(256), 0, st, e0, e1, 0, a);
+        else hipExtLaunchKernelGGL((k_wgrad<BM, BN, WM, WN, false, true, LK>), grid, dim3(256), 0, st, e0, e1, 0, a);
+    });
+}
+
 int launch_wgrad(WgradArgs a, int max_splits, hipStream_t st) {
     const int N = 16 << a.lgCl;
     const bool small = a.Cs < 64;
@@ -816,6 +918,9 @@
     hipEvent_t e0 = g_prof ? g_prof->recs.back().e0 : nullptr, e1 = g_prof ? g_prof->recs.back().e1 : nullptr;
     if (a.dt != DT_F32) {
         launch_wgrad16(small, a, grid, st, e0, e1);
+    } else if (a.S_bn || a.L_y) {
+        if (small) launch_wgrad_tf<32, 128, 1, 4>(a, grid, st, e0, e1);
+        else launch_wgrad_tf<64, 64, 2, 2>(a, grid, st, e0, e1);
     } else if (g_prof) {
         if (small) hipExtLaunchKernelGGL((k_wgrad<32, 128, 1, 4>), grid, dim3(256), 0, st, e0, e1, 0, a);
         else hipExtLaunchKernelGGL((k_wgrad<64, 64, 2, 2>), grid, dim3(256), 0, st, e0, e1, 0, a);
diff --git a/signature-gan_amd/csrc/ops.h b/signature-gan_amd/csrc/ops.h
--- a/signature-gan_amd/csrc/ops.h
+++ b/signature-gan_amd/csrc/ops.h
@@ -64,6 +64,8 @@
 void launch_bn_relu(int dt, const void* y, void* a, int64_t R, int C, const float* bn, float gslope, hipStream_t s);
 void launch_bn_bwd(int dt, void* da, const void* y, int64_t R, int C, float* bn, float* partial,
                    float* dgamma, float* dbeta, int perm_c0, float gslope, hipStream_t s, int pre_rows = 0, hipEvent_t done = nullptr);
+void launch_bn_bwd_fin_rows(int64_t R, int C, float* bn, const float* partial, int pre_rows, float* dgamma, float* dbeta,
+                            hipStream_t s, hipEvent_t done = nullptr);
 
 void launch_final_fwd(int dt, const void* act, const float* Wt, const float* b, float* img, int B, int S, int C, float gslope,
                       hipStream_t s, const float* bn = nullptr, hipEvent_t done = nullptr);
diff --git a/signature-gan_amd/csrc/ops.hip b/signature-gan_amd/csrc/ops.hip
--- a/signature-gan_amd/csrc/ops.hip
+++ b/signature-gan_amd/csrc/ops.hip
@@ -298,8 +298,8 @@
     if (i >= n4) return;
     const int c = (C4 & (C4 - 1)) == 0 ? (int)(i & (C4 - 1)) : (int)(i % C4);
     const float4 v = f4(ld4<T>(y + i * 4)), sc = bn[c], sh = bn[C4 + c];
-    st4<T>(a + i * 4, f32x4{g_act<LK>(fmaf(v.x, sc.x, sh.x), gs), g_act<LK>(fmaf(v.y, sc.y, sh.y), gs),
-                            g_act<LK>(fmaf(v.z, sc.z, sh.z), gs), g_act<LK>(fmaf(v.w, sc.w, sh.w), gs)});
+    st4<T>(a + i * 4, f32x4{g_bn_act<LK>(v.x, sc.x, sh.x, gs), g_bn_act<LK>(v.y, sc.y, sh.y, gs),
+                            g_bn_act<LK>(v.z, sc.z, sh.z, gs), g_bn_act<LK>(v.w, sc.w, sh.w, gs)});
 }
 void launch_bn_relu(int dt, const void* y, void* a, int64_t R, int C, const float* bn, float gslope, hipStream_t s) {
     const int64_t n4 = R * C / 4;
@@ -338,10 +338,10 @@
     const float4 g = f4(ld4<T>(da + i * 4)), yy = f4(ld4<T>(y + i * 4));
     const float4 sc = bn[c], sf = bn[C4 + c], mu = bn[2 * C4 + c], rs = bn[3 * C4 + c], c1 = bn[4 * C4 + c], c2 = bn[5 * C4 + c];
     float4 o;
-    o.x = sc.x * (g_dact<LK>(fmaf(yy.x, sc.x, sf.x), g.x, gs) - c1.x - (yy.x - mu.x) * rs.x * c2.x);
-    o.y = sc.y * (g_dact<LK>(fmaf(yy.y, sc.y, sf.y), g.y, gs) - c1.y - (yy.y - mu.y) * rs.y * c2.y);
-    o.z = sc.z * (g_dact<LK>(fmaf(yy.z, sc.z, sf.z), g.z, gs) - c1.z - (yy.z - mu.z) * rs.z * c2.z);
-    o.w = sc.w * (g_dact<LK>(fmaf(yy.w, sc.w, sf.w), g.w, gs) - c1.w - (yy.w - mu.w) * rs.w * c2.w);
+    o.x = g_bn_bwd<LK>(g.x, yy.x, sc.x, sf.x, mu.x, rs.x, c1.x, c2.x, gs);
+    o.y = g_bn_bwd<LK>(g.y, yy.y, sc.y, sf.y, mu.y, rs.y, c1.y, c2.y, gs);
+    o.z = g_bn_bwd<LK>(g.z, yy.z, sc.z, sf.z, mu.z, rs.z, c1.z, c2.z, gs);
+    o.w = g_bn_bwd<LK>(g.w, yy.w, sc.w, sf.w, mu.w, rs.w, c1.w, c2.w, gs);
     st4<T>(da + i * 4, f32x4{o.x, o.y, o.z, o.w});
 }
 template <class T, bool LK>
@@ -379,7 +379,7 @@
         f32x4 o;
 #pragma unroll
         for (int e = 0; e < 4; ++e)
-            o[e] = sc[e] * (g_dact<LK>(fmaf(yy[e], sc[e], sf[e]), g[e], gs) - c1[e] - (yy[e] - mu[e]) * rs[e] * c2[e]);
+            o[e] = g_bn_bwd<LK>(g[e], yy[e], sc[e], sf[e], mu[e], rs[e], c1[e], c2[e], gs);
         st4<T>(da + i, o);
     }
 }
@@ -408,6 +408,13 @@
         launch_bn_bwd_fin(p0, p1, nch, R, C, bn, dgamma, dbeta, perm_c0, s);
         SIGGAN_LAUNCH_EV(done, (k_bn_bwd_apply<T, LK>), dim3(cdiv(n4, 256)), dim3(256), 0, s, da, y, n4, C / 4, (const float4*)bn, gslope);
     }));
+}
+
+void launch_bn_bwd_fin_rows(int64_t R, int C, float* bn, const float* partial, int pre_rows, float* dgamma, float* dbeta,
+                            hipStream_t s, hipEvent_t done) {
+    const float* p0 = partial; const float* p1 = partial + (size_t)pre_rows * C;
+    SIGGAN_LAUNCH_EV(done, (k_bn_bwd_fin_apply<float, false>), dim3(C / 32, 1), dim3(256), 0, s, (float*)nullptr, (const float*)nullptr,
+                     R, C, bn, p0, p1, pre_rows, dgamma, dbeta, 0, 0.f);
 }
 
 template <class T, bool LK>
diff --git a/signature-gan_amd/csrc/siggan.hip b/signature-gan_amd/csrc/siggan.hip
--- a/signature-gan_amd/csrc/siggan.hip
+++ b/signature-gan_amd/csrc/siggan.hip
@@ -686,6 +686,10 @@
     return a;
 }
 
+static bool g_bn_on_load(const siggan_ctx* c, int l) {
+    return c->dt == DT_F32 && l >= 1 && l < c->Lg && c->gC[l] <= TF_MAX_C && c->gC[l] % 32 == 0;
+}
+
 static void g_forward_pass(siggan_ctx* c, const float* z, int B, bool training, float* img, hipStream_t s,
                            float* partial = nullptr, float* slab_k = nullptr, uint32_t rng_sid = 0, float* z_out = nullptr,
                            hipEvent_t done = nullptr) {
@@ -710,6 +714,7 @@
         GConvArgs a = gconv_args(c);
         if (slab_k) a.slab = slab_k;
         a.in = A[l - 1]; a.wp = c->g_up[l]; a.B = B; a.Hi = Hi; a.Wi = Hi; a.Ci = Ci; a.Co = Co;
+        if (training && g_bn_on_load(c, l - 1)) { a.in = c->g_y[l - 1]; a.in_tf = TF_BN_ACT; a.in_bn = c->g_bn[l - 1]; }
         a.lgHr = ilog2i(Hi); a.lgWr = a.lgHr; a.Ho = 2 * Hi; a.Wo = 2 * Hi; a.form = 1; a.M = B * Hi * Hi;
         const int C = Co;
         const int64_t off = c->g_bn_off[l];
@@ -720,7 +725,7 @@
             launch_bn_train_stats(c->dt, c->g_y[l], R, C, GP(c, gi_bn_w(l)), GP(c, gi_bn_b(l)), c->st.g_bn_running_mean + off,
                                   c->st.g_bn_running_var + off, c->st.g_bn_batches + l, c->g_bn[l], partial, 0,
                                   BN_MOMENTUM, BN_EPS, s);
-            if (l < c->Lg) launch_bn_relu(c->dt, c->g_y[l], A[l], R, C, c->g_bn[l], gs, s);
+            if (l < c->Lg && !g_bn_on_load(c, l)) launch_bn_relu(c->dt, c->g_y[l], A[l], R, C, c->g_bn[l], gs, s);
         } else {
             a.out = A[l]; a.epi = EPI_AFFINE_RELU; a.scale = c->g_bne[l]; a.shift = c->g_bne[l] + C;
             launch_gconv(a, s);
@@ -840,15 +845,21 @@
         const int Hi = 4 << (l - 1), Ho = 2 * Hi, Ci = c->gC[l - 1], Co = c->gC[l];
         const int64_t R = (int64_t)B * Ho * Ho;
         hipEvent_t const ef = L.fork_event(L.a);
+        const bool tf = l < Lg && pre_rows > 0 && g_bn_on_load(c, l);
         if (l == Lg) {
             launch_final_bwd_reduce(c->dt, c->dpre, c->wfin_t, c->g_y[l], B, S, Co, c->g_bn[l], c->partial, c->partial_b, gs, L.m);
             launch_final_bn_bwd_apply(c->dt, c->dpre, c->wfin_t, c->g_y[l], c->g_da[l], B, S, Co, c->g_bn[l], c->partial, c->partial_b,
                                       GG(c, gi_fin_w(c)), GG(c, gi_fin_b(c)), GG(c, gi_bn_w(l)), GG(c, gi_bn_b(l)), gs, L.m, ef);
-        } else
+        } else if (tf)
+            launch_bn_bwd_fin_rows(R, Co, c->g_bn[l], c->partial, pre_rows, GG(c, gi_bn_w(l)), GG(c, gi_bn_b(l)), L.m, ef);
+        else
             launch_bn_bwd(c->dt, c->g_da[l], c->g_y[l], R, Co, c->g_bn[l], c->partial, GG(c, gi_bn_w(l)), GG(c, gi_bn_b(l)), 0, gs, L.m, pre_rows, ef);
         L.fork_after(L.a, ef);
         WgradArgs w; memset(&w, 0, sizeof w); w.zeros = c->zeros; w.dt = c->dt;
         w.S = c->g_a[l - 1]; w.L = c->g_da[l]; w.slab = c->slab; w.dw = GG(c, gi_up_w(l)); w.B = B; w.Cs = Ci; w.Cl = Co;
+        w.gslope = gs;
+        if (g_bn_on_load(c, l - 1)) { w.S = c->g_y[l - 1]; w.S_bn = c->g_bn[l - 1]; }
+        if (tf) { w.L_y = reinterpret_cast<const float*>(c->g_y[l]); w.L_bn = c->g_bn[l]; }
         w.lgHs = ilog2i(Hi); w.lgWs = w.lgHs; w.lgCl = ilog2i(Co); w.K = B * Hi * Hi;
         const int max_splits = (int)(c->slab_floats / ((int64_t)Ci * (16 * Co + 1)));
         launch_wgrad(w, max_splits, L.a);
@@ -856,6 +867,7 @@
         a.in = c->g_da[l]; a.wp = c->g_dn[l]; a.out = c->g_da[l - 1];
         a.B = B; a.Hi = Ho; a.Wi = Ho; a.Ci = Co; a.Co = Ci;
         a.lgHr = ilog2i(Hi); a.lgWr = a.lgHr; a.Ho = Hi; a.Wo = Hi; a.form = 0; a.M = B * Hi * Hi; a.epi = EPI_RAW;
+        if (tf) { a.in_tf = TF_BN_BWD; a.in_y = c->g_y[l]; a.in_bn = c->g_bn[l]; }
         if (l >= 2) {
             a.epi = EPI_BN_BWD_STATS; a.aref = c->g_y[l - 1]; a.bnp = c->g_bn[l - 1]; a.stat0 = c->partial; a.stat_cap = PARTIAL_FLOATS;
         }
@@ -1568,8 +1580,8 @@
     else return fail(SIGGAN_E_INVALID, "unknown debug tensor %s[%d]", name, idx);
     if (n > capv) return fail(SIGGAN_E_INVALID, "debug tensor %s[%d] holds %lld floats, %lld asked", name, idx, (long long)capv, (long long)n);
     DevGuard dg_(c->cfg.device); HIPCHK(dg_.err);
-    if (!strcmp(name, "g_a") && idx == c->Lg && c->ga_last_B) {
-        const int64_t H = c->S;
+    if (!strcmp(name, "g_a") && (idx == c->Lg || g_bn_on_load(c, idx)) && c->ga_last_B) {
+        const int64_t H = 4 << idx;
         HIPCHK(hipDeviceSynchronize());
         launch_bn_relu(c->dt, c->g_y[idx], c->g_a[idx], (int64_t)c->ga_last_B * H * H, c->gC[idx], c->g_bn[idx], c->cfg.g_leaky_slope,
                        (hipStream_t)stream);
```

Measured after the change: 44450 images/s (median of 2 runs). 1.7% lower.
